# puzzlepaint/camera_calibration

Hardware: NVIDIA H100
Metric: LM iterations/sec (higher is better)
Workload: dtype f64

## Files before the change

### camera_calibration_b200/cabi.py

```python
from __future__ import annotations

import ctypes as C
import os
from dataclasses import dataclass, field
from typing import List, Optional, Sequence

import numpy as np

MODEL_CENTRAL_GENERIC = 0
MODEL_NONCENTRAL_GENERIC = 1
MODEL_CENTRAL_THIN_PRISM_FISHEYE = 2
MODEL_CENTRAL_OPENCV = 3
MODEL_CENTRAL_RADIAL = 4

SCHUR_DENSE = 0
SCHUR_DENSE_CUDA = 1
SCHUR_DENSE_ONTHEFLY = 2
SCHUR_SPARSE = 3
SCHUR_SPARSE_ONTHEFLY = 4

JACOBIAN_NUMERIC = 0
JACOBIAN_ANALYTIC = 1

MAX_TRACE = 128
# ... 347 lines not shown
            p = Problem()
            p.n_cameras = len(self.cameras)
            p.cameras = C.cast(self._cam_array, C.POINTER(Camera))
            p.n_imagesets = self.n_imagesets
            p.n_points = self.n_points
            p.n_obs = self.n_obs
            p.obs_imageset = _ptr(self.obs_imageset, C.c_uint32)
            p.obs_camera = _ptr(self.obs_camera, C.c_uint32)
            p.obs_point = _ptr(self.obs_point, C.c_uint32)
            p.obs_xy = _ptr(self.obs_xy, C.c_float)
            self._c = p
        return self._c

    def shard(self, rank: int, world: int) -> "FlatProblem":
        keep = (self.obs_imageset % np.uint32(world)) == np.uint32(rank)
        return FlatProblem(self.cameras, self.n_imagesets, self.n_points, self.obs_imageset[keep],
                           self.obs_camera[keep], self.obs_point[keep], self.obs_xy[keep])

    def shard_indices(self, rank: int, world: int) -> np.ndarray:
        return np.nonzero((self.obs_imageset % np.uint32(world)) == np.uint32(rank))[0]


@dataclass
class FlatState:

    points: np.ndarray
    rig_tr_global: np.ndarray
    camera_tr_rig: np.ndarray
    intrinsics: List[np.ndarray]
    last_projection: Optional[np.ndarray] = None
    _iptr: object = field(default=None, repr=False)

    def __post_init__(self):
        self.points = np.ascontiguousarray(self.points, dtype=np.float64).reshape(-1, 3)
        self.rig_tr_global = np.ascontiguousarray(self.rig_tr_global, dtype=np.float64).reshape(-1, 7)
        self.camera_tr_rig = np.ascontiguousarray(self.camera_tr_rig, dtype=np.float64).reshape(-1, 7)
        self.intrinsics = [np.ascontiguousarray(a, dtype=np.float64).reshape(-1) for a in self.intrinsics]
        if self.last_projection is not None:
            self.last_projection = np.ascontiguousarray(self.last_projection, dtype=np.float64).reshape(-1, 2)

    def copy(self) -> "FlatState":
        return FlatState(self.points.copy(), self.rig_tr_global.copy(), self.camera_tr_rig.copy(),
                         [a.copy() for a in self.intrinsics],
                         None if self.last_projection is None else self.last_projection.copy())

    def c_struct(self) -> State:
        s = State()
        s.points = _ptr(self.points, C.c_double)
        s.rig_tr_global = _ptr(self.rig_tr_global, C.c_double)
        s.camera_tr_rig = _ptr(self.camera_tr_rig, C.c_double)
        arr = (C.POINTER(C.c_double) * len(self.intrinsics))(*[_ptr(a, C.c_double) for a in self.intrinsics])
        self._iptr = arr
        s.intrinsics = C.cast(arr, C.POINTER(C.POINTER(C.c_double)))
        if self.last_projection is not None:
            s.last_projection = _ptr(self.last_projection, C.c_double)
        else:
            s.last_projection = None
        return s

    def check(self, problem: FlatProblem):
        if self.points.shape != (problem.n_points, 3):
            raise ValueError("points shape")
        if self.rig_tr_global.shape != (problem.n_imagesets, 7):
            raise ValueError("rig_tr_global shape")
        if self.camera_tr_rig.shape != (problem.n_cameras, 7):
            raise ValueError("camera_tr_rig shape")
        for cam, a in zip(problem.cameras, self.intrinsics):
            if a.size != cam.intrinsics_size():
                raise ValueError("intrinsics size")
        if self.last_projection is not None and self.last_projection.shape != (problem.n_obs, 2):
            raise ValueError("last_projection shape")


_LIB = None
LIB_PATH = os.path.join(os.path.dirname(os.path.abspath(__file__)), "csrc", "libb200ba.so")

_D = C.POINTER(C.c_double)
_I32 = C.POINTER(C.c_int32)

SYMBOLS = {
    "b200ba_intrinsics_size": (C.c_int64, [C.POINTER(Camera)]),
    "b200ba_update_parameter_count": (C.c_int32, [C.POINTER(Camera)]),
    "b200ba_default_options": (None, [C.POINTER(Options)]),
    "b200ba_create": (C.c_int, [C.POINTER(Problem), C.c_int, C.POINTER(C.c_void_p)]),
    "b200ba_destroy": (None, [C.c_void_p]),
    "b200ba_last_error": (C.c_char_p, [C.c_void_p]),
    "b200ba_set_state": (C.c_int, [C.c_void_p, C.POINTER(State)]),
    "b200ba_get_state": (C.c_int, [C.c_void_p, C.POINTER(State)]),
    "b200ba_optimize": (C.c_int, [C.c_void_p, C.POINTER(Options), C.POINTER(Report)]),
    "b200ba_optimize_host": (C.c_int, [C.c_void_p, C.POINTER(State), C.POINTER(Options), C.POINTER(Report)]),
    "b200ba_evaluate": (C.c_int, [C.c_void_p, C.POINTER(Options), C.c_int, _D, _D, _D]),
    "b200ba_get_jacobians": (C.c_int, [C.c_void_p, _D, _D, _D, _D, _I32, C.c_int32]),
    "b200ba_build_system": (C.c_int, [C.c_void_p, C.POINTER(Options), C.c_int32, _D, _D, _D]),
    "b200ba_degrees_of_freedom": (C.c_int32, [C.c_void_p, C.POINTER(Options)]),
    "b200ba_schur_solve": (C.c_int, [C.c_int, C.c_int32, C.c_int32, C.c_int32, _D, _D, _D, _D, _D, _D]),
    "b200ba_project": (C.c_int, [C.c_int, C.POINTER(Camera), _D, C.c_int64, _D, _D, _I32]),
    "b200ba_unproject": (C.c_int, [C.c_int, C.POINTER(Camera), _D, C.c_int64, _D, _D, _D, _I32]),
    "b200ba_fit_directions": (C.c_int, [C.c_int, C.c_int32, C.c_int32, _D, C.c_int64, _D, _D, C.c_int32,
                                        C.POINTER(FitReport)]),
    "b200ba_compare_models": (C.c_int, [C.c_int, C.POINTER(Camera), _D, C.POINTER(Camera), _D, C.POINTER(FittingReport),
                                        _D, _D, _D]),
    "b200ba_fitting_images": (C.c_int, [C.c_int, C.POINTER(Camera), _D, C.POINTER(Camera), _D, C.POINTER(FittingReport),
                                        C.POINTER(C.c_uint8), C.POINTER(C.c_uint8), C.POINTER(C.c_uint8),
                                        C.POINTER(C.c_uint8), C.POINTER(C.c_uint8), _D]),
    "b200ba_line_offsets": (C.c_int, [C.c_int, C.POINTER(Camera), _D, C.POINTER(LineOffsetsReport), C.POINTER(C.c_uint8),
                                      _D, C.c_int32, _D, C.POINTER(C.c_int64), _D]),
    "b200ba_localization_accuracy": (C.c_int, [C.c_int, C.POINTER(Camera), _D, C.POINTER(Camera), _D, C.c_int64,
                                               C.c_uint64, C.POINTER(LocalizationReport), C.POINTER(C.c_float), _D,
                                               C.POINTER(C.c_float), _D]),
    "b200ba_compare_reconstructions": (C.c_int, [C.c_int, C.POINTER(Camera), _D, C.POINTER(Camera), _D, C.c_int32, _D,
                                                 _D, _D, _D, C.c_int32, C.POINTER(ReconstructionComparison), _D]),
    "b200ba_reconstruction_directions": (C.c_int, [C.c_int, C.POINTER(Camera), _D, C.POINTER(Camera), _D, C.c_int32,
                                                   C.POINTER(C.c_int32), _D]),
    "b200ba_reconstruction_alignment": (C.c_int, [C.c_int64, _D, C.c_int32, _D, _D, _D, _D,
                                                  C.POINTER(ReconstructionComparison)]),
    "b200ba_nccl_unique_id": (C.c_int, [C.POINTER(C.c_uint8)]),
    "b200ba_comm_init": (C.c_int, [C.c_void_p, C.POINTER(C.c_uint8), C.c_int, C.c_int]),
    "b200ba_get_timings": (C.c_int, [C.c_void_p, C.POINTER(Timings)]),
    "b200ba_dense_cholesky_solve": (C.c_int, [C.c_int, C.c_int32, C.c_int32, C.POINTER(C.c_double), C.POINTER(C.c_double),
                                             C.POINTER(C.c_double), C.POINTER(C.c_double), C.POINTER(C.c_double)]),
    "b200ba_run_bundle_adjustment": (C.c_int, [C.c_void_p, C.POINTER(Options), C.c_int32, C.c_double, C.POINTER(BAReport),
                                              ON_ITERATION, C.c_void_p]),
    "b200ba_calibration_report": (C.c_int, [C.c_void_p, C.POINTER(CameraReport), _D, _D]),
    "b200ba_report_images": (C.c_int, [C.c_void_p, C.c_int32, C.POINTER(C.c_uint8), C.POINTER(C.c_uint8),
                                       C.POINTER(C.c_uint8), C.POINTER(C.c_int64), _D]),
    "b200ba_delete_outliers": (C.c_int, [C.c_void_p, C.c_int32, C.c_float, C.POINTER(C.c_uint8), C.POINTER(C.c_uint8),
                                         C.POINTER(C.c_uint8), C.POINTER(OutlierReport), _D]),
    "b200ba_render_voronoi": (C.c_int, [C.c_int, C.c_int32, C.c_int32, C.c_int64, _I32, C.POINTER(C.c_float),
                                        C.POINTER(C.c_uint8), _D]),
    "b200ba_visualize_camera": (C.c_int, [C.c_int, C.c_int32, C.c_int32, _D, C.POINTER(C.c_uint8), _D, _D, _D]),
    "b200ba_intersect_features": (C.c_int, [C.c_int, C.c_int32, C.c_int64, C.POINTER(C.c_int64), C.POINTER(C.c_float),
                                            C.c_double, C.POINTER(C.c_uint8), C.POINTER(IntersectionReport), _D]),
    "b200ba_synthetic_poses": (C.c_int, [C.POINTER(Pattern), C.c_int32, C.c_int32, C.c_int32, C.c_int32,
                                         C.POINTER(C.c_float), C.c_int64, C.c_uint64, _D, C.POINTER(C.c_int64)]),
    "b200ba_render_pattern_images": (C.c_int, [C.c_int, C.POINTER(Pattern), C.POINTER(C.c_uint8), C.c_int32,
                                               C.c_int32, C.c_int32, C.c_int32, C.POINTER(C.c_float), C.c_int64, _D,
                                               C.POINTER(C.c_uint8), _D]),
    "b200ba_feature_samples": (C.c_int, [C.c_int32, C.c_int32, C.POINTER(C.c_float)]),
    "b200ba_refine_features": (C.c_int, [C.c_int, C.POINTER(Pattern), C.POINTER(C.c_uint8), C.c_int32, C.c_int32,
                                         C.c_int64, C.POINTER(C.c_float), C.c_int32, C.c_int32, C.c_int32, C.c_int64,
                                         C.POINTER(FeaturePrediction), C.POINTER(C.c_float), C.POINTER(C.c_float),
                                         C.POINTER(C.c_int32), _D]),
    "b200ba_snapshot_state": (C.c_int, [C.c_void_p]),
    "b200ba_restore_state": (C.c_int, [C.c_void_p]),
    "b200ba_version": (C.c_char_p, []),
    "b200ba_debug_set_eval_budget": (None, [C.c_int]),
    "b200ba_debug_eval_counts": (C.c_int, [C.c_void_p, C.POINTER(C.c_uint16)]),
    "b200ba_debug_solve_step": (C.c_int, [C.c_void_p, C.POINTER(Options), C.c_double, C.c_int32, _D, _D, _D, _D, _D, _D,
                                          _I32]),
    "b200ba_debug_apply_update": (C.c_int, [C.c_void_p, C.POINTER(Options), _D, C.c_int32, C.POINTER(State)]),
    "b200ba_debug_cost_compare": (C.c_int, [C.c_int, C.c_int64, _D, _D, _D, _D]),
    "b200ba_debug_nice_orientation": (C.c_int, [C.c_void_p, _D]),
    "b200ba_debug_lm_events": (C.c_int32, [C.c_void_p, _I32, C.c_int32]),
}

LM_ACCEPTED, LM_REJECTED_COST, LM_REFUSED_PIVOT = 1, 2, 3


class LibraryMissing(RuntimeError):
    pass


def load_library(path: Optional[str] = None):
    global _LIB
    if _LIB is not None and path is None:
        return _LIB
    p = path or LIB_PATH
    if not os.path.exists(p):
        raise LibraryMissing(
            f"{p} not found: build the CUDA extension first (python -c 'import __graft_entry__ as g; g.build()'). "
            "There is no CPU fallback for this path.")
    lib = C.CDLL(p, mode=C.RTLD_GLOBAL)
    for name, (res, args) in SYMBOLS.items():
        fn = getattr(lib, name)
        fn.restype = res
        fn.argtypes = args
    if path is None:
        _LIB = lib
    return lib
```

### camera_calibration_b200/csrc/ba_common.h

```cpp
#pragma once

#include <cuda_runtime.h>
#include <stdint.h>
#include <string.h>

#include "../../include/b200ba.h"

namespace b200ba {

constexpr int kMaxCameras = 8;
constexpr int kMaxK = 80;

struct CamDev {
  int model_type;
  int width, height;
  int min_x, min_y, max_x, max_y;
  int gw, gh;
  double gmul_x, gmul_y;
  double sx, sy;
  double center_x, center_y;
  int K;
  int dof_per_point;
  int64_t intr_off;
  int64_t tan_off;
  int upd_off;
  int upd_count;
};

struct Layout {
  int n_points, n_imagesets, n_cameras;
  int rig_in_state;
  int localize_only;
  int eliminate_points;
  int dof;
  int bs;
  int nblocks;
  int dsz;
  int nbd;
  int nd;
  int g_point, g_pose, g_rig, g_intr;
  int n_jcols;
  int Kmax;
  int jc_point, jc_pose, jc_rig, jc_intr;
};

struct ProblemDev {
  int64_t n_obs;
  const uint32_t* obs_imageset;
  const uint32_t* obs_camera;
  const uint32_t* obs_point;
  const float2* obs_xy;
  CamDev cams[kMaxCameras];
};

struct StateDev {
  double* points;
  double* rig_tr_global;
  double* camera_tr_rig;
  double* intrinsics;
  double* image_tr_global;
  double* tangents;
};

struct ObsOut {
  double* residual;
  double* cost;
  double* jac;
  double* cjac;
  int compact;
  int32_t* cell;
  uint8_t* has_jac;
  uint16_t* evals;
};

struct SystemDev {
  double* base;
  int64_t total;
  double* Dblk;
  double* bp;
  double* B;
  double* C;
  double* bd;
  double* scalars;
};

constexpr int kReportBiasCells = 50;
struct ReportCam {
  long long count;
  double sum, max, median;
  double biasedness;
  int biasedness_cells;
  double hfov, vfov;
  unsigned long long select_prefix;
  long long select_rank;
};
struct ReportDev {
  double2* err;
  double* mag;
  int64_t* cam_off;
  int* cell_off;
  uint32_t* cell_order;
  double* Q;
  double* partial;
  unsigned int* select_hist;
  int* hist;
  double* kl;
  ReportCam* cams;
};

struct OutlierDev {
  int64_t* range;
  double* mag;
  double* partial;
  unsigned int* select_hist;
  ReportCam* stats;
  uint8_t* used;
  int* kept;
  unsigned long long* counts;
  uint8_t* remove;
  uint32_t* owner;
  uint8_t* image;
};

struct CompareDev {
  double* mag;
  double* dir_err;
  double* rep_err;
  unsigned long long* dir_max;
  int64_t* range;
  double* partial;
  unsigned int* select_hist;
  ReportCam* stats;
  uint8_t* angles;
  uint8_t* magnitudes;
  uint8_t* directions;
  uint8_t* rep_magnitudes;
  uint8_t* reprojections;
};

constexpr int kLocPoints = 15;
constexpr int kLocMaxDraws = 4096;
struct LocalizationDev {
  double* p;
  double* f;
  float* samples;
  double* poses;
  double* mag;
  unsigned long long* counts;
  int* capped;
  int64_t* range;
  double* partial;
  unsigned int* select_hist;
  ReportCam* stats;
};

constexpr int kSweepSums = 10;

constexpr int kLineSums = 10;
struct LineOffsetsDev {
  double* lines;
  double* partial;
  double* sums;
  double* mag;
  unsigned long long* extent;
  int64_t* range;
  double* stat_partial;
  unsigned int* select_hist;
  ReportCam* stats;
  double* offsets;
  uint8_t* image;
  double* obj;
};

constexpr int kVoronoiNoSite = INT32_MIN;
struct VoronoiGrid {
  int x0, y0;
  int bs;
  int nx, ny;
  int* off;
  int* count;
  int* idx;
  int* scan_sums;
};
constexpr int kVoronoiScanChunk = 4096;
constexpr int kVoronoiScanMax = 4096;
constexpr int64_t kVoronoiMaxBuckets = int64_t(kVoronoiScanChunk) * kVoronoiScanMax - 1;

struct FixedRanges {
  int n;
  int lo[4], hi[4];
  __host__ __device__ bool has(int g) const {
    for (int i = 0; i < n; ++i)
      if (g >= lo[i] && g < hi[i]) return true;
    return false;
  }
};

__host__ __device__ __forceinline__ uint64_t loc_splitmix64(uint64_t z) {
  z += 0x9E3779B97F4A7C15ull;
  z = (z ^ (z >> 30)) * 0xBF58476D1CE4E5B9ull;
  z = (z ^ (z >> 27)) * 0x94D049BB133111EBull;
  return z ^ (z >> 31);
}

__host__ __device__ __forceinline__ float rf_add(float a, float b) {
#ifdef __CUDA_ARCH__
  return __fadd_rn(a, b);
#else
  return a + b;
#endif
}
__host__ __device__ __forceinline__ float rf_sub(float a, float b) {
#ifdef __CUDA_ARCH__
  return __fsub_rn(a, b);
#else
  return a - b;
#endif
}
__host__ __device__ __forceinline__ float rf_mul(float a, float b) {
#ifdef __CUDA_ARCH__
  return __fmul_rn(a, b);
#else
  return a * b;
#endif
}
// ... 141 lines not shown
```

### camera_calibration_b200/csrc/ba_host.cu

```cuda

#include <cublas_v2.h>
#include <cusolverDn.h>
#include <dlfcn.h>

#include <algorithm>
#include <cmath>
#include <cstdarg>
#include <cstdio>
#include <cstring>
#include <limits>
#include <string>
#include <vector>

#include "ba_kernels.h"

using namespace b200ba;

namespace {

std::string g_create_error;

struct NcclUniqueId {
  char internal[128];
};
struct NcclApi {
  void* lib = nullptr;
  int (*GetUniqueId)(void*) = nullptr;
  int (*CommInitRank)(void**, int, NcclUniqueId, int) = nullptr;
  int (*AllReduce)(const void*, void*, size_t, int, int, void*, cudaStream_t) = nullptr;
  int (*Broadcast)(const void*, void*, size_t, int, int, void*, cudaStream_t) = nullptr;
  int (*ReduceScatter)(const void*, void*, size_t, int, int, void*, cudaStream_t) = nullptr;
  int (*CommDestroy)(void*) = nullptr;
  const char* (*GetErrorString)(int) = nullptr;
};
constexpr int kNcclDouble = 8;
constexpr int kNcclInt32 = 2;
constexpr int kNcclSum = 0;
constexpr int kNcclMax = 2;

NcclApi g_nccl;
bool load_nccl(std::string* err) {
  if (g_nccl.lib) return true;
  const char* names[] = {"libnccl.so.2", "libnccl.so"};
  void* lib = nullptr;
  for (const char* n : names) {
    lib = dlopen(n, RTLD_NOW | RTLD_GLOBAL);
    if (lib) break;
  }
  if (!lib) {
    *err = std::string("cannot load libnccl: ") + dlerror();
    return false;
  }
  g_nccl.lib = lib;
  *reinterpret_cast<void**>(&g_nccl.GetUniqueId) = dlsym(lib, "ncclGetUniqueId");
  *reinterpret_cast<void**>(&g_nccl.CommInitRank) = dlsym(lib, "ncclCommInitRank");
  *reinterpret_cast<void**>(&g_nccl.AllReduce) = dlsym(lib, "ncclAllReduce");
  *reinterpret_cast<void**>(&g_nccl.Broadcast) = dlsym(lib, "ncclBroadcast");
  *reinterpret_cast<void**>(&g_nccl.ReduceScatter) = dlsym(lib, "ncclReduceScatter");
  *reinterpret_cast<void**>(&g_nccl.CommDestroy) = dlsym(lib, "ncclCommDestroy");
  *reinterpret_cast<void**>(&g_nccl.GetErrorString) = dlsym(lib, "ncclGetErrorString");
  if (!g_nccl.GetUniqueId || !g_nccl.CommInitRank || !g_nccl.AllReduce || !g_nccl.Broadcast || !g_nccl.ReduceScatter ||
      !g_nccl.CommDestroy) {
    *err = "libnccl lacks a required symbol";
    g_nccl.lib = nullptr;
    return false;
  }
  return true;
}

enum Phase { PH_JAC = 0, PH_ACC, PH_SCHUR, PH_FACTOR, PH_TRIAL, PH_UPDATE, PH_ALLREDUCE, PH_STRAGGLER, PH_SOLVE, PH_COUNT };

}

struct b200ba_handle {
  int device = 0;
  cudaStream_t stream = nullptr;
  cudaStream_t side_stream = nullptr;
  cudaEvent_t straggler_done = nullptr;
  cublasHandle_t cublas = nullptr;
  cusolverDnHandle_t cusolver = nullptr;
  std::string error;

  std::vector<b200ba_camera> cams_host;
  ProblemDev pb{};
  int n_cameras = 0, n_imagesets = 0, n_points = 0;
  int64_t n_obs = 0;
  int uniform_model = -1;
  int64_t n_control_total = 0, n_param_total = 0, intr_total = 0, tan_total = 0;
  uint32_t *d_obs_imageset = nullptr, *d_obs_camera = nullptr, *d_obs_point = nullptr;
  float2* d_obs_xy = nullptr;

  StateDev st[2]{};
  int cur = 0;
  double2* d_last_projection = nullptr;
  bool have_state = false;
  StateDev snap{};
  double2* d_snap_lp = nullptr;
  bool have_snapshot = false;

  Layout L{};
  bool have_layout = false;
  ObsOut out{};
  ObsOut out_trial{};
  SystemDev sys{};
  double *d_W = nullptr, *d_S = nullptr, *d_Linv = nullptr, *d_v = nullptr, *d_y = nullptr, *d_x = nullptr;
  double trace_H = 0;
  int64_t reduce_count = 0;
  double* d_potrf_work = nullptr;
  int potrf_lwork = 0;
  int *d_info = nullptr, *d_fail = nullptr;
  std::vector<uint32_t> perm;
  uint32_t* d_perm = nullptr;
  double2* d_lp_stage = nullptr;
  uint32_t* d_straggler_list = nullptr;
  int* d_straggler_count = nullptr;
  double *d_partial = nullptr, *d_scal = nullptr;
  double* d_rot = nullptr;
  double* h_scal = nullptr;
  int* h_flags = nullptr;

  std::vector<uint32_t> h_obs_imageset, h_obs_camera, h_obs_point;
  std::vector<float> h_obs_xy;
  int group_blocks_n = 0;
  int n_groups = 0;
  std::vector<int> group_start;
  std::vector<int> group_count;
  int* d_group_of_block = nullptr;
  int* d_group_blocks = nullptr;
  uint8_t* d_flags = nullptr;
  int* d_cols = nullptr;
  int* d_count = nullptr;
  int* h_count = nullptr;
  double* d_Wc = nullptr;
  double* d_P = nullptr;
  size_t wc_stride = 0, p_stride = 0;
  cudaEvent_t ev_syrk[2] = {nullptr, nullptr}, ev_scatter[2] = {nullptr, nullptr}, ev_s_ready = nullptr;
  double* d_u = nullptr;
  bool use_grouped = false;
  double* capture_S = nullptr;
  double* capture_rhs = nullptr;
  std::vector<int32_t> lm_events;
  std::vector<double> grp_sums;
  int force_grouped = -1;

  ReportDev rep{};
  double2* d_rep_stage = nullptr;
  bool have_report = false;
  std::vector<int64_t> img_cam_groups;
  int* d_img_group_off = nullptr;
  uint32_t* d_img_group_obs = nullptr;
  bool have_images = false;

  void* comm = nullptr;
  int rank = 0, n_ranks = 1;

  bool own_dense = true;
  DenseCtx dn;
  int dense_planned_ranks = 0, dense_planned_n = -1;
  int dense_nb = 0;
  cudaStream_t panel_stream = nullptr;
  cudaStream_t aux_stream = nullptr;
  int* d_ident_cols = nullptr;
  double* d_gemv_partial = nullptr;

  b200ba_timings timings{};
  struct Pending {
    int phase;
    cudaEvent_t a, b;
    bool own_a = true;
  };
  std::vector<Pending> pending;
  std::vector<cudaEvent_t> event_pool;
};

namespace {

#define CUDA_TRY(h, expr)                                                                      \
  do {                                                                                         \
    cudaError_t _e = (expr);                                                                   \
    if (_e != cudaSuccess) {                                                                   \
      (h)->error = std::string(#expr) + ": " + cudaGetErrorString(_e);                         \
      return 1;                                                                                \
    }                                                                                          \
  } while (0)
#define CUBLAS_TRY(h, expr)                                                                    \
  do {                                                                                         \
    cublasStatus_t _s = (expr);                                                                \
    if (_s != CUBLAS_STATUS_SUCCESS) {                                                         \
      (h)->error = std::string(#expr) + ": cuBLAS status " + std::to_string(static_cast<int>(_s)); \
      return 1;                                                                                \
    }                                                                                          \
  } while (0)
#define CUSOLVER_TRY(h, expr)                                                                  \
  do {                                                                                         \
    cusolverStatus_t _s = (expr);                                                              \
    if (_s != CUSOLVER_STATUS_SUCCESS) {                                                       \
      (h)->error = std::string(#expr) + ": cuSOLVER status " + std::to_string(static_cast<int>(_s)); \
      return 1;                                                                                \
    }                                                                                          \
  } while (0)

template <class T>
int dev_alloc(b200ba_handle* h, T** p, size_t count) {
  if (*p) {
    cudaFree(*p);
    *p = nullptr;
  }
  if (count == 0) count = 1;
  CUDA_TRY(h, cudaMalloc(reinterpret_cast<void**>(p), count * sizeof(T)));
  return 0;
}

int64_t intrinsics_size(const b200ba_camera& c) {
  const int64_t G = static_cast<int64_t>(c.grid_width) * c.grid_height;
  switch (c.model_type) {
    case B200BA_MODEL_CENTRAL_GENERIC: return 3 * G;
    case B200BA_MODEL_NONCENTRAL_GENERIC: return 6 * G;
    default: return 12;
  }
}
int update_parameter_count(const b200ba_camera& c) {
  const int G = c.grid_width * c.grid_height;
  switch (c.model_type) {
    case B200BA_MODEL_CENTRAL_GENERIC: return 2 * G;
    case B200BA_MODEL_NONCENTRAL_GENERIC: return 5 * G;
    default: return 12;
  }
}
int jacobian_size(const b200ba_camera& c) {
  switch (c.model_type) {
    case B200BA_MODEL_CENTRAL_GENERIC: return 32;
    case B200BA_MODEL_NONCENTRAL_GENERIC: return 80;
    default: return 12;
  }
}

void fill_camdev(const b200ba_camera& c, CamDev* d) {
  d->model_type = c.model_type;
  d->width = c.width;
  d->height = c.height;
  d->min_x = c.calibration_min_x;
  d->min_y = c.calibration_min_y;
  d->max_x = c.calibration_max_x;
  d->max_y = c.calibration_max_y;
  d->gw = c.grid_width;
  d->gh = c.grid_height;
  const int aw = c.calibration_max_x + 1 - c.calibration_min_x;
  const int ah = c.calibration_max_y + 1 - c.calibration_min_y;
  d->gmul_x = (c.grid_width > 0) ? static_cast<double>(c.grid_width - 3) / aw : 0.0;
  d->gmul_y = (c.grid_height > 0) ? static_cast<double>(c.grid_height - 3) / ah : 0.0;
  d->sx = (c.grid_width > 0) ? static_cast<double>((c.grid_width - 3.f) / aw) : 0.0;
  d->sy = (c.grid_height > 0) ? static_cast<double>((c.grid_height - 3.f) / ah) : 0.0;
  d->center_x = 0.5f * static_cast<float>(c.calibration_min_x + c.calibration_max_x + 1);
  d->center_y = 0.5f * static_cast<float>(c.calibration_min_y + c.calibration_max_y + 1);
  d->K = jacobian_size(c);
  d->dof_per_point = c.model_type == B200BA_MODEL_CENTRAL_GENERIC ? 2 : (c.model_type == B200BA_MODEL_NONCENTRAL_GENERIC ? 5 : 0);
  d->upd_count = update_parameter_count(c);
}

int64_t align32(int64_t n) { return (n + 31) / 32 * 32; }

cudaEvent_t get_event(b200ba_handle* h) {
  if (!h->event_pool.empty()) {
    cudaEvent_t e = h->event_pool.back();
    h->event_pool.pop_back();
    return e;
  }
  cudaEvent_t e;
  cudaEventCreate(&e);
  return e;
}
struct ScopedPhase {
  b200ba_handle* h;
  int phase;
  cudaEvent_t a;
  ScopedPhase(b200ba_handle* h_, int p) : h(h_), phase(p) {
    a = get_event(h);
    cudaEventRecord(a, h->stream);
  }
  ~ScopedPhase() {
    cudaEvent_t b = get_event(h);
    cudaEventRecord(b, h->stream);
    h->pending.push_back({phase, a, b, true});
  }
};
void resolve_timings(b200ba_handle* h) {
  for (auto& p : h->pending) {
    float ms = 0;
    if (cudaEventElapsedTime(&ms, p.a, p.b) == cudaSuccess) {
      switch (p.phase) {
        case PH_JAC: h->timings.jacobian_kernel_ms += ms; h->timings.jacobian_kernel_launches++; break;
        case PH_ACC: h->timings.accumulate_ms += ms; break;
        case PH_SCHUR: h->timings.schur_ms += ms; break;
        case PH_FACTOR: h->timings.factor_ms += ms; break;
        case PH_TRIAL: h->timings.trial_cost_ms += ms; break;
        case PH_UPDATE: h->timings.update_ms += ms; break;
        case PH_ALLREDUCE: h->timings.allreduce_ms += ms; break;
        case PH_STRAGGLER: h->timings.straggler_ms += ms; break;
        case PH_SOLVE: h->timings.solve_ms += ms; h->timings.factor_ms += ms; break;
      }
    }
    if (p.own_a) h->event_pool.push_back(p.a);
    h->event_pool.push_back(p.b);
  }
  h->pending.clear();
}
int reduce_group_sums(b200ba_handle* h) {
  if (h->n_ranks <= 1 || !h->comm || h->grp_sums.empty()) return 0;
  const size_t n = h->grp_sums.size();
  double* d = nullptr;
  CUDA_TRY(h, cudaMalloc(reinterpret_cast<void**>(&d), n * sizeof(double)));
  cudaMemcpy(d, h->grp_sums.data(), n * sizeof(double), cudaMemcpyHostToDevice);
  const int rc = g_nccl.AllReduce(d, d, n, kNcclDouble, kNcclSum, h->comm, h->stream);
  const cudaError_t ce = cudaStreamSynchronize(h->stream);
  if (rc == 0 && ce == cudaSuccess) cudaMemcpy(h->grp_sums.data(), d, n * sizeof(double), cudaMemcpyDeviceToHost);
  cudaFree(d);
  if (rc != 0 || ce != cudaSuccess) {
    h->error = "all-reduce of the group centroids failed";
    return 1;
  }
  return 0;
}

int build_groups(b200ba_handle* h, bool allocate) {
  const Layout& L = h->L;
  const int nb = L.nblocks;
  int gb = (L.bs == 3) ? 96 : 48;
  if (const char* e = getenv("B200BA_GROUP_BLOCKS")) gb = std::max(1, atoi(e));
  h->group_blocks_n = gb;
  std::vector<int> order(nb);
  for (int i = 0; i < nb; ++i) order[i] = i;
  if (L.eliminate_points && nb > 0) {
    const double* sx = h->grp_sums.data();
    const double* sy = sx + nb;
    const double* cnt = sy + nb;
    const double qx = std::max(1.0, h->cams_host[0].width / 64.0), qy = std::max(1.0, h->cams_host[0].height / 64.0);
    std::vector<uint32_t> zkey(nb, 0);
    for (int p = 0; p < nb; ++p) {
      if (cnt[p] <= 0) continue;
      uint32_t ux = static_cast<uint32_t>(std::min(1023.0, std::max(0.0, sx[p] / cnt[p] / qx)));
      uint32_t uy = static_cast<uint32_t>(std::min(1023.0, std::max(0.0, sy[p] / cnt[p] / qy)));
      uint32_t z = 0;
      for (int b = 0; b < 10; ++b) z |= ((ux >> b) & 1u) << (2 * b) | ((uy >> b) & 1u) << (2 * b + 1);
      zkey[p] = z;
    }
    std::stable_sort(order.begin(), order.end(), [&](int a, int b) { return zkey[a] < zkey[b]; });
  }
  h->n_groups = (nb + gb - 1) / gb;
  h->group_start.assign(h->n_groups + 1, 0);
  std::vector<int> gob(std::max(1, nb), 0);
  for (int g = 0; g < h->n_groups; ++g) {
    h->group_start[g] = g * gb;
    for (int i = g * gb; i < std::min(nb, (g + 1) * gb); ++i) gob[order[i]] = g;
  }
  h->group_start[h->n_groups] = nb;
  h->group_count.assign(std::max(1, h->n_groups), 0);
  if (allocate) {
    if (dev_alloc(h, &h->d_group_of_block, std::max(1, nb))) return 1;
    if (dev_alloc(h, &h->d_group_blocks, std::max(1, nb))) return 1;
    if (dev_alloc(h, &h->d_flags, static_cast<size_t>(std::max(1, h->n_groups)) * std::max(1, L.nd))) return 1;
    if (dev_alloc(h, &h->d_cols, static_cast<size_t>(std::max(1, h->n_groups)) * std::max(1, L.nd))) return 1;
    if (dev_alloc(h, &h->d_count, std::max(1, h->n_groups))) return 1;
    if (h->h_count) cudaFreeHost(h->h_count);
    CUDA_TRY(h, cudaMallocHost(reinterpret_cast<void**>(&h->h_count), std::max(1, h->n_groups) * sizeof(int)));
    h->wc_stride = static_cast<size_t>(gb) * L.bs * (std::max(1, L.nd) + 1);
    h->p_stride = static_cast<size_t>(std::max(1, L.nd)) * std::max(1, L.nd);
    if (dev_alloc(h, &h->d_Wc, 2 * h->wc_stride)) return 1;
    if (!h->own_dense && dev_alloc(h, &h->d_P, 2 * h->p_stride)) return 1;
    for (int i = 0; i < 2; ++i) {
      if (!h->ev_syrk[i]) CUDA_TRY(h, cudaEventCreateWithFlags(&h->ev_syrk[i], cudaEventDisableTiming));
      if (!h->ev_scatter[i]) CUDA_TRY(h, cudaEventCreateWithFlags(&h->ev_scatter[i], cudaEventDisableTiming));
    }
    if (!h->ev_s_ready) CUDA_TRY(h, cudaEventCreateWithFlags(&h->ev_s_ready, cudaEventDisableTiming));
    if (dev_alloc(h, &h->d_u, std::max(1, L.nbd))) return 1;
  }
  CUDA_TRY(h, cudaMemcpy(h->d_group_of_block, gob.data(), std::max(1, nb) * sizeof(int), cudaMemcpyHostToDevice));
  if (nb > 0) CUDA_TRY(h, cudaMemcpy(h->d_group_blocks, order.data(), nb * sizeof(int), cudaMemcpyHostToDevice));
  return 0;
}

int nccl_bcast_cb(double* buf, size_t count, int root, cudaStream_t s, void* user) {
  b200ba_handle* h = static_cast<b200ba_handle*>(user);
  const int rc = g_nccl.Broadcast(buf, buf, count, kNcclDouble, root, h->comm, s);
  if (rc != 0) {
    h->error = std::string("ncclBroadcast: ") + (g_nccl.GetErrorString ? g_nccl.GetErrorString(rc) : "error");
    return 1;
  }
  return 0;
}

cudaError_t dense_create(DenseCtx* d, bool own_streams) {
  cudaError_t e = cudaSuccess;
  if (own_streams) {
    int lo = 0, hi = 0;
    cudaDeviceGetStreamPriorityRange(&lo, &hi);
    e = cudaStreamCreateWithFlags(&d->s_main, cudaStreamNonBlocking);
    if (e == cudaSuccess) e = cudaStreamCreateWithPriority(&d->s_panel, cudaStreamNonBlocking, hi);
    if (e == cudaSuccess) e = cudaStreamCreateWithPriority(&d->s_aux, cudaStreamNonBlocking, hi);
  }
  for (cudaEvent_t* ev : {&d->ev_ready[0], &d->ev_ready[1], &d->ev_main[0], &d->ev_main[1], &d->ev_half2[0],
                          &d->ev_half2[1], &d->ev_misc})
    if (e == cudaSuccess && !*ev) e = cudaEventCreateWithFlags(ev, cudaEventDisableTiming);
  return e;
}
void dense_release(DenseCtx* d, bool own_streams) {
  for (cudaEvent_t ev : {d->ev_ready[0], d->ev_ready[1], d->ev_main[0], d->ev_main[1], d->ev_half2[0], d->ev_half2[1],
                         d->ev_misc})
    if (ev) cudaEventDestroy(ev);
  if (own_streams)
    for (cudaStream_t s : {d->s_main, d->s_panel, d->s_aux})
      if (s) cudaStreamDestroy(s);
}

int plan_dense(b200ba_handle* h) {
// ... 56 lines not shown
  }
  const int rig_dof = L.rig_in_state ? 6 * h->n_cameras : 0;
  if (L.eliminate_points) {
    L.bs = 3;
    L.nblocks = h->n_points;
    L.g_point = 0;
    L.g_pose = 3 * h->n_points;
    L.g_rig = L.g_pose + 6 * h->n_imagesets;
    L.g_intr = L.g_rig + rig_dof;
  } else {
    L.bs = 6;
    L.nblocks = h->n_imagesets;
    L.g_pose = 0;
    L.g_rig = 6 * h->n_imagesets;
    L.g_point = L.g_rig + rig_dof;
    L.g_intr = L.g_point + 3 * h->n_points;
  }
  L.dsz = L.bs * (L.bs + 1) / 2;
  L.nbd = L.bs * L.nblocks;
  L.dof = 3 * h->n_points + 6 * h->n_imagesets + rig_dof + n_intr;
  L.nd = L.dof - L.nbd;
  L.Kmax = kmax;
  L.jc_point = 0;
  L.jc_pose = 3;
  L.jc_rig = 9;
  L.jc_intr = 9 + (L.rig_in_state ? 6 : 0);
  L.n_jcols = L.jc_intr + kmax;
  const bool same = h->have_layout && memcmp(&L, &h->L, sizeof(Layout)) == 0;
  if (same) return plan_dense(h);
  h->L = L;
  h->have_layout = true;
  h->dense_planned_n = -1;

  const int64_t n = h->n_obs;
  if (dev_alloc(h, &h->out.residual, 2 * n)) return 1;
  if (dev_alloc(h, &h->out.cost, n)) return 1;
  h->out.compact = (h->uniform_model == B200BA_MODEL_CENTRAL_GENERIC) ? 1 : 0;
  if (h->out.compact) {
    if (h->out.jac) cudaFree(h->out.jac);
    h->out.jac = nullptr;
    if (dev_alloc(h, &h->out.cjac, 14 * static_cast<size_t>(n))) return 1;
  } else {
    if (dev_alloc(h, &h->out.jac, 2 * static_cast<size_t>(L.n_jcols) * n)) return 1;
  }
  if (dev_alloc(h, &h->out.cell, n)) return 1;
  if (dev_alloc(h, &h->out.has_jac, n)) return 1;
  if (dev_alloc(h, &h->out.evals, n)) return 1;
  h->out_trial.evals = nullptr;
  if (dev_alloc(h, &h->out_trial.residual, 2 * n)) return 1;
  if (dev_alloc(h, &h->out_trial.cost, n)) return 1;
  h->out_trial.jac = nullptr;
  h->out_trial.cjac = nullptr;
  h->out_trial.compact = 0;
  h->out_trial.cell = nullptr;
  h->out_trial.has_jac = nullptr;

  SystemDev& s = h->sys;
  const int64_t oD = 0;
  const int64_t obp = oD + align32(static_cast<int64_t>(L.dsz) * L.nblocks);
  const int64_t oB = obp + align32(L.nbd);
  const int64_t obd = oB + align32(static_cast<int64_t>(L.nbd) * L.nd);
  const int64_t osc = obd + align32(L.nd);
  const int64_t oC = osc + 32;
  s.total = oC + align32(static_cast<int64_t>(L.nd) * L.nd);
  h->reduce_count = oC;
  if (dev_alloc(h, &s.base, s.total)) return 1;
  s.Dblk = s.base + oD;
  s.bp = s.base + obp;
  s.B = s.base + oB;
  s.C = s.base + oC;
  s.bd = s.base + obd;
  s.scalars = s.base + osc;
  if (dev_alloc(h, &h->d_W, static_cast<size_t>(L.nbd) * L.nd)) return 1;
  if (!h->own_dense) {
    if (dev_alloc(h, &h->d_S, static_cast<size_t>(L.nd) * L.nd + L.nd)) return 1;
  } else if (plan_dense(h)) {
    return 1;
  }
  if (dev_alloc(h, &h->d_Linv, static_cast<size_t>(L.dsz) * L.nblocks)) return 1;
  if (dev_alloc(h, &h->d_v, L.nbd)) return 1;
  if (dev_alloc(h, &h->d_y, L.nbd)) return 1;
  if (dev_alloc(h, &h->d_x, L.dof)) return 1;
  int lwork = 0;
  CUSOLVER_TRY(h, cusolverDnDpotrf_bufferSize(h->cusolver, CUBLAS_FILL_MODE_LOWER, L.nd, h->d_S, std::max(1, L.nd), &lwork));
  h->potrf_lwork = lwork;
  if (dev_alloc(h, &h->d_potrf_work, std::max(1, lwork))) return 1;

  {
    const int nb = L.nblocks;
    h->grp_sums.assign(3 * static_cast<size_t>(std::max(1, nb)), 0.0);
    if (L.eliminate_points) {
      for (int64_t o = 0; o < h->n_obs; ++o) {
        const int p = static_cast<int>(h->h_obs_point[o]);
        h->grp_sums[p] += h->h_obs_xy[2 * o];
        h->grp_sums[nb + p] += h->h_obs_xy[2 * o + 1];
        h->grp_sums[2 * nb + p] += 1.0;
      }
    }
    if (reduce_group_sums(h)) return 1;
    if (build_groups(h, true)) return 1;
  }
  return 0;
}

int sync_stream(b200ba_handle* h) {
  CUDA_TRY(h, cudaStreamSynchronize(h->stream));
  resolve_timings(h);
  return 0;
}

int all_reduce(b200ba_handle* h, double* buf, size_t count) {
  if (h->n_ranks <= 1 || !h->comm) return 0;
  ScopedPhase ph(h, PH_ALLREDUCE);
  int rc = g_nccl.AllReduce(buf, buf, count, kNcclDouble, kNcclSum, h->comm, h->stream);
  if (rc != 0) {
    h->error = std::string("ncclAllReduce: ") + (g_nccl.GetErrorString ? g_nccl.GetErrorString(rc) : "error");
    return 1;
  }
  return 0;
}

int evaluate_state(b200ba_handle* h, int which, bool jac, const ObsOut& out, double huber, int phase,
                   bool overlap_stragglers = false) {
  launch_prepare_state(h->pb, h->L, h->st[which], h->n_control_total, h->stream);
  h->timings.kernel_launches += 1;
  {
    cudaEvent_t a = get_event(h), mid = get_event(h);
    cudaEventRecord(a, h->stream);
    launch_residual_jacobian(h->uniform_model, jac, h->pb, h->L, h->st[which], h->d_last_projection, out, huber,
                             h->d_straggler_list, h->d_straggler_count, h->stream, mid);
    if (h->n_obs == 0) cudaEventRecord(mid, h->stream);
    h->pending.push_back({phase, a, mid, true});
    cudaStream_t ss = overlap_stragglers ? h->side_stream : h->stream;
    if (overlap_stragglers) CUDA_TRY(h, cudaStreamWaitEvent(h->side_stream, mid, 0));
    cudaEvent_t s0 = get_event(h), s1 = get_event(h);
    cudaEventRecord(s0, ss);
    launch_straggler_pass(h->uniform_model, jac, h->pb, h->L, h->st[which], h->d_last_projection, out, huber,
                          h->d_straggler_list, h->d_straggler_count, ss);
    cudaEventRecord(s1, ss);
    h->pending.push_back({PH_STRAGGLER, s0, s1, true});
    h->straggler_done = s1;
    h->timings.kernel_launches += 2 * (h->n_obs > 0);
  }
  CUDA_TRY(h, cudaGetLastError());
  return 0;
}

int build_system(b200ba_handle* h, double huber, double* cost, double* n_valid, const b200ba_options* fix = nullptr) {
  if (evaluate_state(h, h->cur, true, h->out, huber, PH_JAC, true)) return 1;
  {
    ScopedPhase ph(h, PH_ACC);
    CUDA_TRY(h, cudaMemsetAsync(h->sys.base, 0, h->sys.total * sizeof(double), h->stream));
    launch_accumulate_scatter(h->pb, h->L, h->st[h->cur], h->out, h->sys, huber, h->stream);
    if (!h->L.localize_only || h->L.rig_in_state) {
      launch_accumulate_cells(h->pb, h->L, h->st[h->cur], h->out, h->sys, huber, h->stream);
      h->timings.kernel_launches += 1;
    }
    CUDA_TRY(h, cudaStreamWaitEvent(h->stream, h->straggler_done, 0));
    launch_accumulate_list(h->pb, h->L, h->st[h->cur], h->out, h->sys, huber, h->d_straggler_list, h->d_straggler_count, h->stream);
    h->timings.kernel_launches += 2;
    launch_cost_reduce(h->n_obs, h->out.cost, nullptr, h->out.residual, h->d_partial, h->sys.scalars, h->stream);
    launch_trace(h->L.nblocks, h->L.bs, h->sys.Dblk, h->L.nd, h->sys.C, h->sys.scalars + 8, h->stream);
    h->timings.kernel_launches += 3;
  }
  CUDA_TRY(h, cudaGetLastError());
  if (all_reduce(h, h->sys.base, static_cast<size_t>(h->reduce_count))) return 1;
  if (fix) {
    const Layout& L = h->L;
    FixedRanges fr{};
    auto add = [&](int g0, int count) {
      if (count > 0 && fr.n < 4) {
        fr.lo[fr.n] = g0;
        fr.hi[fr.n] = g0 + count;
        fr.n++;
      }
    };
    int n_intr = 0;
    for (int c = 0; c < h->n_cameras; ++c) n_intr += update_parameter_count(h->cams_host[c]);
    if (fix->debug_fix_points) add(L.g_point, 3 * L.n_points);
    if (fix->debug_fix_poses) add(L.g_pose, 6 * L.n_imagesets);
    if (fix->debug_fix_rig_poses && L.rig_in_state) add(L.g_rig, 6 * L.n_cameras);
    if (fix->debug_fix_intrinsics && !L.localize_only) add(L.g_intr, n_intr);
    launch_mask_fixed(L, h->sys, fr, h->rank == 0 ? 1.0 : 0.0, h->stream);
    h->timings.kernel_launches += 3;
  }
  CUDA_TRY(h, cudaMemcpyAsync(h->h_scal, h->sys.scalars, 9 * sizeof(double), cudaMemcpyDeviceToHost, h->stream));
  if (h->n_groups > 0 && h->L.nd > 0 && h->force_grouped != 0) {
    ScopedPhase ph(h, PH_SCHUR);
    CUDA_TRY(h, cudaMemsetAsync(h->d_flags, 0, static_cast<size_t>(h->n_groups) * h->L.nd, h->stream));
    launch_group_support(h->L.bs, h->L.nblocks, h->L.nd, h->sys.B, h->d_group_of_block, h->d_flags, h->stream);
    launch_compact_columns(h->n_groups, h->L.nd, h->d_flags, h->d_cols, h->d_count, h->stream);
    CUDA_TRY(h, cudaMemcpyAsync(h->h_count, h->d_count, h->n_groups * sizeof(int), cudaMemcpyDeviceToHost, h->stream));
    h->timings.kernel_launches += 2;
  }
  if (sync_stream(h)) return 1;
  *cost = h->h_scal[3];
  *n_valid = h->h_scal[4];
  h->trace_H = h->h_scal[8];
  h->use_grouped = false;
  if (h->n_groups > 0 && h->L.nd > 0 && h->force_grouped != 0) {
    double grouped = 0;
    for (int g = 0; g < h->n_groups; ++g) {
      const double kg = static_cast<double>(h->group_start[g + 1] - h->group_start[g]) * h->L.bs;
      const double mg = h->h_count[g];
      h->group_count[g] = h->h_count[g];
      grouped += mg * mg * (kg + 24.0);
    }
    const double dense = static_cast<double>(h->L.nd) * h->L.nd * h->L.nbd;
    h->use_grouped = (h->force_grouped == 1) || grouped < 0.6 * dense;
  }
  return 0;
}

int factor_dense(b200ba_handle* h) {
  const int nd = h->L.nd;
  CUSOLVER_TRY(h, cusolverDnDpotrf(h->cusolver, CUBLAS_FILL_MODE_LOWER, nd, h->d_S, nd, h->d_potrf_work, h->potrf_lwork,
                                   h->d_info));
  return 0;
}

int capture_reduced_system(b200ba_handle* h) {
  const Layout& L = h->L;
  const int nd = L.nd;
  if (nd > 0) {
    if (h->own_dense) {
      const DenseCtx& d = h->dn;
      for (int j = 0; j < d.nblk; ++j) {
        const int c0 = j * d.NB, w = std::min(d.NB, nd - c0);
        CUDA_TRY(h, cudaMemcpy2DAsync(h->capture_S + static_cast<size_t>(c0) * nd, static_cast<size_t>(nd) * sizeof(double),
                                      h->d_S + d.map.col_offset(c0), d.map.ld * sizeof(double),
                                      static_cast<size_t>(nd) * sizeof(double), w, cudaMemcpyDeviceToHost, h->stream));
      }
    } else {
      CUDA_TRY(h, cudaMemcpyAsync(h->capture_S, h->d_S, static_cast<size_t>(nd) * nd * sizeof(double), cudaMemcpyDeviceToHost,
                                  h->stream));
    }
    CUDA_TRY(h, cudaMemcpyAsync(h->capture_rhs, h->d_x + L.nbd, static_cast<size_t>(nd) * sizeof(double),
                                cudaMemcpyDeviceToHost, h->stream));
  }
  return sync_stream(h);
}

int solve_system_own(b200ba_handle* h, double lambda, int* spd);

int solve_system(b200ba_handle* h, double lambda, int* spd) {
  if (h->own_dense) return solve_system_own(h, lambda, spd);
  const Layout& L = h->L;
  const double one = 1.0, minus_one = -1.0;
  bool grouped_done = false;
  if (h->use_grouped) {
    ScopedPhase ph(h, PH_SCHUR);
    const double zero = 0.0;
    CUDA_TRY(h, cudaMemsetAsync(h->d_fail, 0, sizeof(int), h->stream));
    launch_schur_blocks(L.bs, L.nblocks, h->sys.Dblk, h->sys.bp, lambda, h->d_Linv, h->d_v, h->d_fail, h->stream);
    CUDA_TRY(h, cudaEventRecord(h->ev_s_ready, h->stream));
    CUDA_TRY(h, cudaStreamWaitEvent(h->side_stream, h->ev_s_ready, 0));
    CUDA_TRY(h, cudaMemcpyAsync(h->d_S, h->sys.C, static_cast<size_t>(L.nd) * L.nd * sizeof(double),
                                cudaMemcpyDeviceToDevice, h->side_stream));
    CUDA_TRY(h, cudaEventRecord(h->ev_s_ready, h->side_stream));
    launch_block_solve_t(L.bs, L.nblocks, h->d_Linv, h->d_v, h->d_u, h->stream);
    h->timings.kernel_launches += 2;
    int it = 0;
    for (int g = h->rank; g < h->n_groups; g += h->n_ranks) {
      const int nblk = h->group_start[g + 1] - h->group_start[g];
      const int kg = nblk * L.bs, mg = h->group_count[g];
      if (mg == 0 || kg == 0) continue;
      h->timings.contraction_flops += static_cast<double>(mg) * mg * kg;
      const int b = it & 1;
      double* Wc = h->d_Wc + b * h->wc_stride;
      double* P = h->d_P + b * h->p_stride;
      const int* cols = h->d_cols + static_cast<size_t>(g) * L.nd;
      if (it >= 2) CUDA_TRY(h, cudaStreamWaitEvent(h->stream, h->ev_scatter[b], 0));
      launch_gather_scale(L.bs, nblk, L.nd, mg, mg, h->sys.B, h->d_Linv, h->d_group_blocks + h->group_start[g], cols, Wc,
                          h->stream);
      CUBLAS_TRY(h, cublasDsyrk(h->cublas, CUBLAS_FILL_MODE_LOWER, CUBLAS_OP_N, mg, kg, &one, Wc, mg, &zero, P, mg));
      CUDA_TRY(h, cudaEventRecord(h->ev_syrk[b], h->stream));
      CUDA_TRY(h, cudaStreamWaitEvent(h->side_stream, h->ev_syrk[b], 0));
      launch_scatter_sub(L.nd, mg, cols, P, h->d_S, h->side_stream);
      CUDA_TRY(h, cudaEventRecord(h->ev_scatter[b], h->side_stream));
      h->timings.kernel_launches += 2;
      ++it;
    }
    CUDA_TRY(h, cudaStreamWaitEvent(h->stream, h->ev_s_ready, 0));
    for (int b = 0; b < 2 && b < it; ++b) CUDA_TRY(h, cudaStreamWaitEvent(h->stream, h->ev_scatter[b], 0));
    grouped_done = true;
  }
  if (grouped_done) {
    if (h->n_ranks > 1) {
      if (all_reduce(h, h->d_S, static_cast<size_t>(L.nd) * L.nd)) return 1;
    }
    ScopedPhase ph(h, PH_SCHUR);
    launch_add_diagonal(L.nd, h->d_S, L.nd, lambda, h->stream);
    CUDA_TRY(h, cudaMemcpyAsync(h->d_x + L.nbd, h->sys.bd, L.nd * sizeof(double), cudaMemcpyDeviceToDevice, h->stream));
    if (L.nbd > 0 && L.nd > 0)
      CUBLAS_TRY(h, cublasDgemv(h->cublas, CUBLAS_OP_N, L.nd, L.nbd, &minus_one, h->sys.B, L.nd, h->d_u, 1, &one,
                                h->d_x + L.nbd, 1));
    h->timings.kernel_launches += 1;
  } else {
    const int p0 = static_cast<int>(static_cast<int64_t>(L.nblocks) * h->rank / h->n_ranks);
    const int p1 = static_cast<int>(static_cast<int64_t>(L.nblocks) * (h->rank + 1) / h->n_ranks);
    const int k_rows = L.bs * (p1 - p0);
    double* rhs_tail = h->d_S + static_cast<size_t>(L.nd) * L.nd;
    {
      ScopedPhase ph(h, PH_SCHUR);
      CUDA_TRY(h, cudaMemsetAsync(h->d_fail, 0, sizeof(int), h->stream));
      launch_schur_blocks(L.bs, L.nblocks, h->sys.Dblk, h->sys.bp, lambda, h->d_Linv, h->d_v, h->d_fail, h->stream);
// ... 86 lines not shown
    launch_block_solve_t(L.bs, L.nblocks, h->d_Linv, h->d_v, h->d_u, h->stream);
    h->timings.kernel_launches += 2;
    bool joined = false;
    auto join_copy = [&]() {
      if (!joined) cudaStreamWaitEvent(h->stream, h->ev_s_ready, 0);
      joined = true;
    };
    if (h->use_grouped) {
      int it = 0;
      for (int g = h->rank; g < h->n_groups; g += R) {
        const int nblk = h->group_start[g + 1] - h->group_start[g];
        const int kg = nblk * L.bs, mg = h->group_count[g];
        if (mg == 0 || kg == 0) continue;
        const int ldw = (mg + 1) / 2 * 2;
        double* Wc = h->d_Wc + (it & 1) * h->wc_stride;
        const int* cols = h->d_cols + static_cast<size_t>(g) * nd;
        launch_gather_scale(L.bs, nblk, nd, mg, ldw, h->sys.B, h->d_Linv, h->d_group_blocks + h->group_start[g], cols, Wc,
                            h->stream);
        join_copy();
        GemmArgs ga{};
        ga.M = ga.N = mg;
        ga.K = kg;
        ga.A = ga.B = Wc;
        ga.lda = ga.ldb = ldw;
        ga.C = h->d_S;
        ga.alpha = -1.0;
        ga.beta = 1.0;
        ga.a_aligned = ga.b_aligned = gemm_operand_aligned(Wc, ldw);
        ga.cols = cols;
        ga.map = d.map;
        if (launch_dgemm_nt(ga, true, true, h->stream)) {
          h->error = "dgemm_nt (contraction) launch failed";
          return 1;
        }
        h->timings.contraction_flops += static_cast<double>(mg) * mg * kg;
        h->timings.kernel_launches += 2;
        ++it;
      }
    } else if (L.nbd > 0 && nd > 0) {
      const int p0 = static_cast<int>(static_cast<int64_t>(L.nblocks) * h->rank / R);
      const int p1 = static_cast<int>(static_cast<int64_t>(L.nblocks) * (h->rank + 1) / R);
      const int k_rows = L.bs * (p1 - p0);
      launch_schur_scale_rows(L.bs, L.nblocks, nd, h->sys.B, h->d_Linv, h->d_W, h->stream);
      h->timings.kernel_launches += 1;
      if (k_rows > 0) {
        const double* Wr = h->d_W + static_cast<size_t>(L.bs) * p0 * nd;
        join_copy();
        GemmArgs ga{};
        ga.M = ga.N = nd;
        ga.K = k_rows;
        ga.A = ga.B = Wr;
        ga.lda = ga.ldb = nd;
        ga.C = h->d_S;
        ga.ldc = d.map.ld;
        ga.alpha = -1.0;
        ga.beta = 1.0;
        ga.a_aligned = ga.b_aligned = gemm_operand_aligned(Wr, nd);
        ga.cols = h->d_ident_cols;
        ga.map = d.map;
        if (launch_dgemm_nt(ga, true, R > 1, h->stream)) {
          h->error = "dgemm_nt (contraction) launch failed";
          return 1;
        }
        h->timings.contraction_flops += static_cast<double>(nd) * nd * k_rows;
        h->timings.kernel_launches += 1;
      }
    }
    join_copy();
    if (h->rank == 0) launch_add_diagonal_map(nd, h->d_S, d.map, lambda, h->stream);
    CUDA_TRY(h, cudaMemcpyAsync(h->d_x + L.nbd, h->sys.bd, nd * sizeof(double), cudaMemcpyDeviceToDevice, h->stream));
    if (L.nbd > 0 && nd > 0) launch_gemv_t(L.nbd, nd, nd, h->sys.B, h->d_u, -1.0, h->d_x + L.nbd, h->d_gemv_partial, h->stream);
    h->timings.kernel_launches += 4;
  }
  if (h->capture_S && capture_reduced_system(h)) return 1;
  if (R > 1 && nd > 0) {
    ScopedPhase ph(h, PH_ALLREDUCE);
    const int rc = g_nccl.ReduceScatter(h->d_S, h->d_S + static_cast<size_t>(h->rank) * d.chunk, static_cast<size_t>(d.chunk),
                                        kNcclDouble, kNcclSum, h->comm, h->stream);
    if (rc != 0) {
      h->error = std::string("ncclReduceScatter: ") + (g_nccl.GetErrorString ? g_nccl.GetErrorString(rc) : "error");
      return 1;
    }
  }
  {
    ScopedPhase ph(h, PH_FACTOR);
    if (dense_factor(&d)) {
      if (h->error.empty()) h->error = "dense_factor: launch failed";
      return 1;
    }
    h->timings.factor_flops += static_cast<double>(nd) * nd * nd / 3.0;
    if (R > 1) {
      const int rc = g_nccl.AllReduce(h->d_info, h->d_info, 1, kNcclInt32, kNcclMax, h->comm, h->stream);
      if (rc != 0) {
        h->error = "ncclAllReduce (factorisation status) failed";
        return 1;
      }
    }
  }
  {
    ScopedPhase ph(h, PH_SOLVE);
    if (dense_solve(&d, h->d_x + L.nbd)) {
      h->error = "dense_solve: launch failed";
      return 1;
    }
    h->timings.kernel_launches += 4 * d.ntiles;
  }
  {
    ScopedPhase ph(h, PH_SCHUR);
    if (L.nbd > 0 && nd > 0)
      launch_gemv_n(L.nbd, nd, nd, h->sys.B, h->d_x + L.nbd, h->d_y, h->stream);
    else if (L.nbd > 0)
      CUDA_TRY(h, cudaMemsetAsync(h->d_y, 0, L.nbd * sizeof(double), h->stream));
    launch_block_backsub2(L.bs, L.nblocks, h->d_Linv, h->d_u, h->d_y, h->d_x, h->stream);
    h->timings.kernel_launches += 1;
  }
  CUDA_TRY(h, cudaMemcpyAsync(h->h_flags, h->d_info, sizeof(int), cudaMemcpyDeviceToHost, h->stream));
  CUDA_TRY(h, cudaMemcpyAsync(h->h_flags + 1, h->d_fail, sizeof(int), cudaMemcpyDeviceToHost, h->stream));
  if (sync_stream(h)) return 1;
  *spd = (h->h_flags[0] == 0 && h->h_flags[1] == 0) ? 1 : 0;
  return 0;
}

int check_ready(b200ba_handle* h, const b200ba_options* opt) {
  if (!h) return 1;
  if (!opt) {
    h->error = "options are NULL";
    return 2;
  }
  if (!h->have_state) {
    h->error = "no state: call b200ba_set_state first";
    return 2;
  }
  CUDA_TRY(h, cudaSetDevice(h->device));
  return make_layout(h, opt);
}

void free_handle_buffers(b200ba_handle* h) {
  auto F = [](auto*& p) {
    if (p) cudaFree(p);
    p = nullptr;
  };
  F(h->d_obs_imageset); F(h->d_obs_camera); F(h->d_obs_point); F(h->d_obs_xy);
  for (int i = 0; i < 2; ++i) {
    F(h->st[i].points); F(h->st[i].rig_tr_global); F(h->st[i].camera_tr_rig); F(h->st[i].intrinsics);
    F(h->st[i].image_tr_global); F(h->st[i].tangents);
  }
  F(h->d_last_projection);
  F(h->snap.points); F(h->snap.rig_tr_global); F(h->snap.camera_tr_rig); F(h->snap.intrinsics); F(h->d_snap_lp);
  h->have_snapshot = false;
  F(h->out.residual); F(h->out.cost); F(h->out.jac); F(h->out.cjac); F(h->out.cell); F(h->out.has_jac); F(h->out.evals);
  F(h->out_trial.residual); F(h->out_trial.cost);
  F(h->sys.base); F(h->d_W); F(h->d_S); F(h->d_Linv); F(h->d_v); F(h->d_y); F(h->d_x); F(h->d_potrf_work);
  F(h->d_info); F(h->d_fail); F(h->d_straggler_list); F(h->d_straggler_count); F(h->d_perm); F(h->d_lp_stage);
  F(h->d_group_of_block); F(h->d_group_blocks); F(h->d_flags); F(h->d_cols); F(h->d_count); F(h->d_Wc); F(h->d_P); F(h->d_u);
  if (h->h_count) cudaFreeHost(h->h_count);
  h->h_count = nullptr;
  F(h->d_partial); F(h->d_scal); F(h->d_rot);
  F(h->rep.err); F(h->rep.mag); F(h->rep.cam_off); F(h->rep.cell_off); F(h->rep.cell_order); F(h->rep.Q);
  F(h->rep.partial); F(h->rep.select_hist); F(h->rep.hist); F(h->rep.kl); F(h->rep.cams); F(h->d_rep_stage);
  h->have_report = false;
  F(h->d_img_group_off); F(h->d_img_group_obs);
  h->have_images = false;
  F(h->dn.Lpack); F(h->dn.tmp); F(h->dn.d_panel_off); F(h->dn.d_panel_h); F(h->d_ident_cols); F(h->d_gemv_partial);
  h->dn.S = nullptr;
  h->dense_planned_n = -1;
  if (h->h_scal) cudaFreeHost(h->h_scal);
  if (h->h_flags) cudaFreeHost(h->h_flags);
  h->h_scal = nullptr;
  h->h_flags = nullptr;
}

int setup_report(b200ba_handle* h) {
  if (h->have_report) return 0;
  const int64_t n = h->n_obs;
  const int nc = h->n_cameras;
  constexpr int kCells = kReportBiasCells * kReportBiasCells;
  std::vector<int64_t> cam_off(nc + 1, 0);
  for (int64_t o = 0; o < n; ++o) ++cam_off[h->h_obs_camera[o] + 1];
  for (int c = 0; c < nc; ++c) cam_off[c + 1] += cam_off[c];
  std::vector<uint32_t> key(n);
  std::vector<int> cell_off(static_cast<size_t>(nc) * kCells + 1, 0);
  for (int64_t o = 0; o < n; ++o) {
    const uint32_t cam = h->h_obs_camera[o];
    const b200ba_camera& c = h->cams_host[cam];
    const double step_u = static_cast<double>(c.calibration_max_x - c.calibration_min_x) / kReportBiasCells + 1e-7;
    const double step_v = static_cast<double>(c.calibration_max_y - c.calibration_min_y) / kReportBiasCells + 1e-7;
    const float dx = h->h_obs_xy[2 * o] - static_cast<float>(c.calibration_min_x);
    const float dy = h->h_obs_xy[2 * o + 1] - static_cast<float>(c.calibration_min_y);
    const int cx = std::min(kReportBiasCells - 1, std::max(0, static_cast<int>(dx / step_u)));
    const int cy = std::min(kReportBiasCells - 1, std::max(0, static_cast<int>(dy / step_v)));
    key[o] = cam * kCells + cy * kReportBiasCells + cx;
    ++cell_off[key[o] + 1];
  }
  for (size_t k = 0; k + 1 < cell_off.size(); ++k) cell_off[k + 1] += cell_off[k];
  std::vector<uint32_t> pos(n), order(n);
  for (int64_t i = 0; i < n; ++i) pos[h->perm[i]] = static_cast<uint32_t>(i);
  {
    std::vector<int> fill(cell_off.begin(), cell_off.end() - 1);
    for (int64_t o = 0; o < n; ++o) order[fill[key[o]]++] = pos[o];
  }
  double Q[64], q_sum = 0;
  for (int y = 0; y < 8; ++y)
    for (int x = 0; x < 8; ++x) {
      const double dx = (2.5 / (0.5 * 8)) * (0.5 * 8 - (x + 0.5));
      const double dy = (2.5 / (0.5 * 8)) * (0.5 * 8 - (y + 0.5));
      const double p = std::exp(-0.5 * (dx * dx + dy * dy));
      Q[y * 8 + x] = p;
      q_sum += p;
    }
  for (double& q : Q) q /= q_sum;
  ReportDev& r = h->rep;
  if (dev_alloc(h, &r.err, n) || dev_alloc(h, &r.mag, n) || dev_alloc(h, &r.cam_off, nc + 1) ||
      dev_alloc(h, &r.cell_off, cell_off.size()) || dev_alloc(h, &r.cell_order, n) || dev_alloc(h, &r.Q, 64) ||
      dev_alloc(h, &r.partial, report_partial_size(nc)) || dev_alloc(h, &r.select_hist, 256 * nc) ||
      dev_alloc(h, &r.hist, static_cast<size_t>(nc) * B200BA_REPORT_HIST * B200BA_REPORT_HIST) ||
      dev_alloc(h, &r.kl, static_cast<size_t>(nc) * kCells) || dev_alloc(h, &r.cams, nc) || dev_alloc(h, &h->d_rep_stage, n))
    return 1;
  CUDA_TRY(h, cudaMemcpy(r.cam_off, cam_off.data(), cam_off.size() * sizeof(int64_t), cudaMemcpyHostToDevice));
  CUDA_TRY(h, cudaMemcpy(r.cell_off, cell_off.data(), cell_off.size() * sizeof(int), cudaMemcpyHostToDevice));
  if (n > 0) CUDA_TRY(h, cudaMemcpy(r.cell_order, order.data(), n * sizeof(uint32_t), cudaMemcpyHostToDevice));
  CUDA_TRY(h, cudaMemcpy(r.Q, Q, sizeof(Q), cudaMemcpyHostToDevice));
  h->have_report = true;
  return 0;
}

int setup_images(b200ba_handle* h) {
  if (h->have_images) return 0;
  const int64_t n = h->n_obs;
  const int nc = h->n_cameras;
  std::vector<uint32_t> pos(n);
  for (int64_t i = 0; i < n; ++i) pos[h->perm[i]] = static_cast<uint32_t>(i);
  std::vector<std::pair<int64_t, uint32_t>> keyed;
  keyed.reserve(n);
  for (int64_t o = 0; o < n; ++o) {
    const b200ba_camera& c = h->cams_host[h->h_obs_camera[o]];
    const float x = h->h_obs_xy[2 * o], y = h->h_obs_xy[2 * o + 1];
    if (!(x > -1.f && y > -1.f && x < 4.f * c.width && y < 4.f * c.height)) continue;
    const int64_t ix = static_cast<int>(x), iy = static_cast<int>(y);
    if (ix >= 4 * static_cast<int64_t>(c.width) || iy >= 4 * static_cast<int64_t>(c.height)) continue;
    const int64_t key = (static_cast<int64_t>(h->h_obs_camera[o]) << 40) | (iy * 4 * c.width + ix);
    keyed.emplace_back(key, static_cast<uint32_t>(o));
  }
  std::stable_sort(keyed.begin(), keyed.end(),
                   [](const std::pair<int64_t, uint32_t>& a, const std::pair<int64_t, uint32_t>& b) { return a.first < b.first; });
  std::vector<int> group_off;
  std::vector<uint32_t> group_obs(keyed.size());
  h->img_cam_groups.assign(nc + 1, 0);
  for (size_t k = 0; k < keyed.size(); ++k) {
    if (k == 0 || keyed[k].first != keyed[k - 1].first) {
      group_off.push_back(static_cast<int>(k));
      ++h->img_cam_groups[(keyed[k].first >> 40) + 1];
    }
    group_obs[k] = pos[keyed[k].second];
  }
  group_off.push_back(static_cast<int>(keyed.size()));
  for (int c = 0; c < nc; ++c) h->img_cam_groups[c + 1] += h->img_cam_groups[c];
  if (dev_alloc(h, &h->d_img_group_off, group_off.size()) || dev_alloc(h, &h->d_img_group_obs, group_obs.size())) return 1;
  CUDA_TRY(h, cudaMemcpy(h->d_img_group_off, group_off.data(), group_off.size() * sizeof(int), cudaMemcpyHostToDevice));
  if (!group_obs.empty())
    CUDA_TRY(h, cudaMemcpy(h->d_img_group_obs, group_obs.data(), group_obs.size() * sizeof(uint32_t), cudaMemcpyHostToDevice));
  h->have_images = true;
  return 0;
}

struct CallScope {
  std::string* error;
  int rc = 0;
  std::vector<void*> buffers;
  cudaEvent_t events[3] = {};
  cublasHandle_t cublas = nullptr;
  cusolverDnHandle_t cusolver = nullptr;

  explicit CallScope(std::string* error_sink) : error(error_sink) {}
  CallScope(const CallScope&) = delete;
  CallScope& operator=(const CallScope&) = delete;
  ~CallScope() {
    for (void* p : buffers) cudaFree(p);
    for (cudaEvent_t e : events)
      if (e) cudaEventDestroy(e);
    if (cublas) cublasDestroy(cublas);
    if (cusolver) cusolverDnDestroy(cusolver);
  }
  int use_device(int device) {
    int ndev = 0;
    if (cudaGetDeviceCount(&ndev) != cudaSuccess || ndev == 0) {
      g_create_error = "no CUDA device available (this library has no CPU fallback)";
      return 3;
    }
    if (device >= 0) cudaSetDevice(device);
    return 0;
  }
  void fail(const char* message) {
    if (rc == 0) {
      *error = message;
      rc = 1;
    }
  }
  bool ok(cudaError_t e) {
    if (e != cudaSuccess) fail(cudaGetErrorString(e));
    return e == cudaSuccess;
  }
  template <class T>
  void alloc(T** p, size_t count) {
    if (ok(cudaMalloc(p, sizeof(T) * count))) buffers.push_back(*p);
  }
  void record(int k, cudaStream_t s) {
    for (cudaEvent_t& e : events)
      if (!e) ok(cudaEventCreate(&e));
    cudaEventRecord(events[k], s);
  }
  float elapsed_ms(int from, int to) {
    float ms = 0;
    ok(cudaEventElapsedTime(&ms, events[from], events[to]));
    return ms;
  }
  bool create_solvers() {
    if (rc == 0 && (cublasCreate(&cublas) != CUBLAS_STATUS_SUCCESS || cusolverDnCreate(&cusolver) != CUSOLVER_STATUS_SUCCESS))
      fail("cuBLAS / cuSOLVER initialisation failed");
    return rc == 0;
  }
};

struct VoronoiRun {
  VoronoiGrid g{};
  int64_t nb = 0;
  void alloc(CallScope& cs, int64_t n, int64_t lo_x, int64_t lo_y, int64_t hi_x, int64_t hi_y) {
    g = voronoi_grid_geometry(lo_x, lo_y, hi_x, hi_y);
    nb = static_cast<int64_t>(g.nx) * g.ny;
    cs.alloc(&g.off, nb + 1);
    cs.alloc(&g.count, nb);
    cs.alloc(&g.idx, std::max<int64_t>(1, n));
    cs.alloc(&g.scan_sums, kVoronoiScanMax);
  }
  cudaError_t n_valid(int64_t* out) {
    int v = 0;
    const cudaError_t e = cudaMemcpy(&v, g.off + nb, sizeof(int), cudaMemcpyDeviceToHost);
    *out = v;
    return e;
  }
};

void alloc_range_statistics(CallScope& cs, int64_t n, int64_t** range, double** partial, unsigned int** select_hist,
                            ReportCam** stats) {
  cs.alloc(range, 2);
  cs.alloc(partial, report_partial_size(1));
  cs.alloc(select_hist, 256);
  cs.alloc(stats, 1);
  const int64_t r[2] = {0, n};
  if (cs.rc == 0) cs.ok(cudaMemcpy(*range, r, sizeof(r), cudaMemcpyHostToDevice));
}

struct LmResult {
  int iterations = 0, attempts = 0;
  double initial_cost = 0, final_cost = 0, lambda = 0;
};
template <class System, class InitLambda, class Solve, class TrialCost, class Accept>
LmResult small_lm(const int& rc, int max_iterations, System system, InitLambda init_lambda, Solve solve,
                  TrialCost trial_cost, Accept accept) {
  LmResult r;
  for (int iteration = 0; rc == 0 && iteration < max_iterations; ++iteration) {
    r.final_cost = system(iteration);
    if (rc) break;
    if (iteration == 0) r.initial_cost = r.final_cost;
    if (r.final_cost == 0) break;
    if (iteration == 0) {
      r.lambda = init_lambda(static_cast<double>(0.001f));
      if (rc) break;
    }
    bool applied = false;
    for (int attempt = 0; rc == 0 && attempt < 10; ++attempt) {
      r.attempts++;
      const bool solved = solve(r.lambda);
      if (rc) break;
      if (!solved) {
        r.lambda = 2.f * r.lambda;
        continue;
      }
      const double test_cost = trial_cost();
      if (rc) break;
      if (test_cost < r.final_cost) {
        accept();
        r.lambda = 0.5f * r.lambda;
        applied = true;
        r.iterations += 1;
        r.final_cost = test_cost;
        break;
      }
      r.lambda = 2.f * r.lambda;
    }
    if (!applied || r.final_cost == 0) break;
  }
  return r;
}

int download_system(b200ba_handle* h, double* H, double* b) {
  const Layout& L = h->L;
  const int n = L.dof;
  std::vector<double> D(static_cast<size_t>(L.dsz) * L.nblocks), bp(L.nbd), B(static_cast<size_t>(L.nbd) * L.nd),
      C(static_cast<size_t>(L.nd) * L.nd), bd(L.nd);
  CUDA_TRY(h, cudaMemcpy(D.data(), h->sys.Dblk, D.size() * sizeof(double), cudaMemcpyDeviceToHost));
  CUDA_TRY(h, cudaMemcpy(bp.data(), h->sys.bp, bp.size() * sizeof(double), cudaMemcpyDeviceToHost));
  CUDA_TRY(h, cudaMemcpy(B.data(), h->sys.B, B.size() * sizeof(double), cudaMemcpyDeviceToHost));
  CUDA_TRY(h, cudaMemcpy(C.data(), h->sys.C, C.size() * sizeof(double), cudaMemcpyDeviceToHost));
  CUDA_TRY(h, cudaMemcpy(bd.data(), h->sys.bd, bd.size() * sizeof(double), cudaMemcpyDeviceToHost));
  std::fill(H, H + static_cast<size_t>(n) * n, 0.0);
  for (int p = 0; p < L.nblocks; ++p) {
    const double* d = &D[static_cast<size_t>(L.dsz) * p];
    const int o = L.bs * p;
    for (int a2 = 0; a2 < L.bs; ++a2)
      for (int b2 = a2; b2 < L.bs; ++b2)
        H[static_cast<size_t>(o + a2) * n + o + b2] = d[a2 * L.bs - (a2 * (a2 - 1)) / 2 + (b2 - a2)];
  }
  for (int i = 0; i < L.nbd; ++i)
    for (int k = 0; k < L.nd; ++k) H[static_cast<size_t>(i) * n + L.nbd + k] = B[static_cast<size_t>(i) * L.nd + k];
  for (int i = 0; i < L.nd; ++i)
    for (int k = i; k < L.nd; ++k) H[static_cast<size_t>(L.nbd + i) * n + L.nbd + k] = C[static_cast<size_t>(i) * L.nd + k];
  for (int i = 0; i < L.nbd; ++i) b[i] = bp[i];
  for (int i = 0; i < L.nd; ++i) b[L.nbd + i] = bd[i];
  return 0;
}

}

extern "C" {

const char* b200ba_version(void) { return "b200ba 0.1.0 (sm_90a, FP64)"; }

int64_t b200ba_intrinsics_size(const b200ba_camera* cam) { return cam ? intrinsics_size(*cam) : 0; }
int32_t b200ba_update_parameter_count(const b200ba_camera* cam) { return cam ? update_parameter_count(*cam) : 0; }

void b200ba_default_options(b200ba_options* o) {
  if (!o) return;
  o->max_iteration_count = 1;
  o->init_lambda = -1.0;
  o->numerical_diff_delta = 1e-4;
  o->regularization_weight = 0.0;
  o->localize_only = 0;
  o->eliminate_points = 1;
  o->schur_mode = B200BA_SCHUR_DENSE;
  o->max_lm_attempts = 50;
  o->init_lambda_factor = 1e-5;
  o->huber_parameter = 1.0;
  o->jacobian_mode = B200BA_JACOBIAN_ANALYTIC;
  o->print_progress = 0;
  o->debug_verify_cost = 0;
  o->debug_fix_points = o->debug_fix_poses = o->debug_fix_rig_poses = o->debug_fix_intrinsics = 0;
}

const char* b200ba_last_error(const b200ba_handle* h) { return h ? h->error.c_str() : g_create_error.c_str(); }

int b200ba_create(const b200ba_problem* p, int device, b200ba_handle** out) {
  if (!p || !out) {
    g_create_error = "NULL argument";
    return 2;
  }
  *out = nullptr;
  int ndev = 0;
  if (cudaGetDeviceCount(&ndev) != cudaSuccess || ndev == 0) {
    g_create_error = "no CUDA device available (this library has no CPU fallback)";
    return 3;
  }
  if (p->n_cameras < 1 || p->n_cameras > kMaxCameras) {
    g_create_error = "n_cameras out of range (1..8)";
    return 2;
  }
  for (int c = 0; c < p->n_cameras; ++c) {
    const int t = p->cameras[c].model_type;
    if (t != B200BA_MODEL_CENTRAL_GENERIC && t != B200BA_MODEL_NONCENTRAL_GENERIC && t != B200BA_MODEL_CENTRAL_OPENCV) {
      g_create_error = "camera model not on the accelerated path (central-generic, noncentral-generic, central-opencv)";
      return 2;
    }
    if (t != B200BA_MODEL_CENTRAL_OPENCV && (p->cameras[c].grid_width < 4 || p->cameras[c].grid_height < 4)) {
      g_create_error = "generic models need a grid of at least 4x4 control points";
      return 2;
    }
  }
  if (p->n_obs >= (1LL << 31)) {
    g_create_error = "n_obs must be < 2^31";
    return 2;
  }
  for (int64_t o = 0; o < p->n_obs; ++o) {
    if (p->obs_imageset[o] >= static_cast<uint32_t>(p->n_imagesets) || p->obs_point[o] >= static_cast<uint32_t>(p->n_points) ||
        p->obs_camera[o] >= static_cast<uint32_t>(p->n_cameras)) {
      g_create_error = "observation index out of range";
      return 2;
    }
  }
  b200ba_handle* h = new b200ba_handle();
  auto fail = [&](int rc) {
    g_create_error = h->error;
    free_handle_buffers(h);
    if (h->cublas) cublasDestroy(h->cublas);
    if (h->cusolver) cusolverDnDestroy(h->cusolver);
    if (h->stream) cudaStreamDestroy(h->stream);
    if (h->side_stream) cudaStreamDestroy(h->side_stream);
    delete h;
    return rc;
  };
  if (device < 0) {
    if (cudaGetDevice(&device) != cudaSuccess) device = 0;
  }
  h->device = device;
#define TRYC(expr) \
  if ((expr) != 0) return fail(1)
  auto cuda_ok = [&](cudaError_t e, const char* what) {
    if (e != cudaSuccess) {
      h->error = std::string(what) + ": " + cudaGetErrorString(e);
      return 1;
    }
    return 0;
  };
  TRYC(cuda_ok(cudaSetDevice(device), "cudaSetDevice"));
  TRYC(cuda_ok(cudaStreamCreateWithFlags(&h->stream, cudaStreamNonBlocking), "cudaStreamCreate"));
  TRYC(cuda_ok(cudaStreamCreateWithFlags(&h->side_stream, cudaStreamNonBlocking), "cudaStreamCreate"));
  if (cublasCreate(&h->cublas) != CUBLAS_STATUS_SUCCESS) {
    h->error = "cublasCreate failed";
    return fail(1);
  }
  cublasSetStream(h->cublas, h->stream);
  if (cusolverDnCreate(&h->cusolver) != CUSOLVER_STATUS_SUCCESS) {
    h->error = "cusolverDnCreate failed";
    return fail(1);
  }
  cusolverDnSetStream(h->cusolver, h->stream);

  h->n_cameras = p->n_cameras;
  h->n_imagesets = p->n_imagesets;
  h->n_points = p->n_points;
  h->n_obs = p->n_obs;
  h->cams_host.assign(p->cameras, p->cameras + p->n_cameras);
  h->uniform_model = h->cams_host[0].model_type;
  int upd = 0;
  for (int c = 0; c < p->n_cameras; ++c) {
    CamDev& d = h->pb.cams[c];
    fill_camdev(h->cams_host[c], &d);
    d.intr_off = h->intr_total;
    d.tan_off = h->tan_total;
    d.upd_off = upd;
    upd += d.upd_count;
    h->intr_total += intrinsics_size(h->cams_host[c]);
    const int64_t G = static_cast<int64_t>(d.gw) * d.gh;
    h->tan_total += 6 * G;
    h->n_control_total += G;
    if (d.gw == 0) h->n_param_total += 12;
    if (h->cams_host[c].model_type != h->uniform_model) h->uniform_model = -1;
  }
  const int64_t n = p->n_obs;
  TRYC(dev_alloc(h, &h->d_obs_imageset, n));
  TRYC(dev_alloc(h, &h->d_obs_camera, n));
  TRYC(dev_alloc(h, &h->d_obs_point, n));
  TRYC(dev_alloc(h, &h->d_obs_xy, n));
  if (n > 0) {
    std::vector<uint32_t> key(n);
    for (int64_t o = 0; o < n; ++o) {
      const uint32_t cam = p->obs_camera[o];
      const CamDev& cd = h->pb.cams[cam];
      uint32_t cell = 0;
      if (cd.gw > 0) {
        const double gx = 1.0 + cd.gmul_x * (static_cast<double>(p->obs_xy[2 * o]) - cd.min_x);
        const double gy = 1.0 + cd.gmul_y * (static_cast<double>(p->obs_xy[2 * o + 1]) - cd.min_y);
        const int x0 = std::min(std::max(static_cast<int>(std::floor(gx)) - 1, 0), cd.gw - 4);
        const int y0 = std::min(std::max(static_cast<int>(std::floor(gy)) - 1, 0), cd.gh - 4);
        cell = static_cast<uint32_t>(x0 + y0 * cd.gw);
      }
      key[o] = (cam << 24) | cell;
    }
    h->perm.resize(n);
    for (int64_t o = 0; o < n; ++o) h->perm[o] = static_cast<uint32_t>(o);
    std::stable_sort(h->perm.begin(), h->perm.end(), [&](uint32_t a, uint32_t b) { return key[a] < key[b]; });
    std::vector<uint32_t> t32(n);
    std::vector<float> txy(2 * n);
    for (int64_t i = 0; i < n; ++i) t32[i] = p->obs_imageset[h->perm[i]];
    TRYC(cuda_ok(cudaMemcpy(h->d_obs_imageset, t32.data(), n * sizeof(uint32_t), cudaMemcpyHostToDevice), "H2D"));
    for (int64_t i = 0; i < n; ++i) t32[i] = p->obs_camera[h->perm[i]];
    TRYC(cuda_ok(cudaMemcpy(h->d_obs_camera, t32.data(), n * sizeof(uint32_t), cudaMemcpyHostToDevice), "H2D"));
    for (int64_t i = 0; i < n; ++i) t32[i] = p->obs_point[h->perm[i]];
    TRYC(cuda_ok(cudaMemcpy(h->d_obs_point, t32.data(), n * sizeof(uint32_t), cudaMemcpyHostToDevice), "H2D"));
    for (int64_t i = 0; i < n; ++i) {
      txy[2 * i] = p->obs_xy[2 * h->perm[i]];
      txy[2 * i + 1] = p->obs_xy[2 * h->perm[i] + 1];
    }
    TRYC(cuda_ok(cudaMemcpy(h->d_obs_xy, txy.data(), n * sizeof(float2), cudaMemcpyHostToDevice), "H2D"));
    TRYC(dev_alloc(h, &h->d_perm, n));
    TRYC(cuda_ok(cudaMemcpy(h->d_perm, h->perm.data(), n * sizeof(uint32_t), cudaMemcpyHostToDevice), "H2D"));
  }
  TRYC(dev_alloc(h, &h->d_lp_stage, n));
  if (n > 0) {
    h->h_obs_imageset.assign(p->obs_imageset, p->obs_imageset + n);
    h->h_obs_camera.assign(p->obs_camera, p->obs_camera + n);
    h->h_obs_point.assign(p->obs_point, p->obs_point + n);
    h->h_obs_xy.assign(p->obs_xy, p->obs_xy + 2 * n);
  }
  if (const char* e = getenv("B200BA_DENSE")) h->own_dense = !(strcmp(e, "lib") == 0 || strcmp(e, "0") == 0);
  if (const char* e = getenv("B200BA_DENSE_NB")) h->dense_nb = std::max(128, atoi(e) / 128 * 128);
  {
    int lo = 0, hi = 0;
    cudaDeviceGetStreamPriorityRange(&lo, &hi);
    TRYC(cuda_ok(cudaStreamCreateWithPriority(&h->panel_stream, cudaStreamNonBlocking, hi), "cudaStreamCreate"));
    TRYC(cuda_ok(cudaStreamCreateWithPriority(&h->aux_stream, cudaStreamNonBlocking, hi), "cudaStreamCreate"));
  }
  if (const char* e = getenv("B200BA_GROUPED")) h->force_grouped = atoi(e);
  h->pb.n_obs = n;
  h->pb.obs_imageset = h->d_obs_imageset;
  h->pb.obs_camera = h->d_obs_camera;
  h->pb.obs_point = h->d_obs_point;
  h->pb.obs_xy = h->d_obs_xy;
  for (int i = 0; i < 2; ++i) {
    TRYC(dev_alloc(h, &h->st[i].points, 3 * static_cast<size_t>(h->n_points)));
    TRYC(dev_alloc(h, &h->st[i].rig_tr_global, 7 * static_cast<size_t>(h->n_imagesets)));
    TRYC(dev_alloc(h, &h->st[i].camera_tr_rig, 7 * static_cast<size_t>(h->n_cameras)));
    TRYC(dev_alloc(h, &h->st[i].intrinsics, h->intr_total));
    TRYC(dev_alloc(h, &h->st[i].image_tr_global, 12 * static_cast<size_t>(h->n_imagesets) * h->n_cameras));
    TRYC(dev_alloc(h, &h->st[i].tangents, h->tan_total));
  }
  TRYC(dev_alloc(h, &h->d_last_projection, n));
  TRYC(cuda_ok(cudaMemset(h->d_last_projection, 0, std::max<int64_t>(1, n) * sizeof(double2)), "memset"));
  TRYC(dev_alloc(h, &h->d_straggler_list, n));
  TRYC(dev_alloc(h, &h->d_straggler_count, 1));
  TRYC(dev_alloc(h, &h->d_info, 2));
  TRYC(dev_alloc(h, &h->d_fail, 1));
  TRYC(dev_alloc(h, &h->d_partial, cost_reduce_partial_size()));
  TRYC(dev_alloc(h, &h->d_scal, 16));
  TRYC(cuda_ok(cudaMallocHost(reinterpret_cast<void**>(&h->h_scal), 16 * sizeof(double)), "cudaMallocHost"));
  TRYC(cuda_ok(cudaMallocHost(reinterpret_cast<void**>(&h->h_flags), 4 * sizeof(int)), "cudaMallocHost"));
#undef TRYC
  *out = h;
  return 0;
}

void b200ba_destroy(b200ba_handle* h) {
  if (!h) return;
  cudaSetDevice(h->device);
  if (h->stream) cudaStreamSynchronize(h->stream);
  if (h->comm && g_nccl.CommDestroy) g_nccl.CommDestroy(h->comm);
  resolve_timings(h);
  for (auto e : h->event_pool) cudaEventDestroy(e);
  for (int i = 0; i < 2; ++i) {
    if (h->ev_syrk[i]) cudaEventDestroy(h->ev_syrk[i]);
    if (h->ev_scatter[i]) cudaEventDestroy(h->ev_scatter[i]);
  }
  if (h->ev_s_ready) cudaEventDestroy(h->ev_s_ready);
  free_handle_buffers(h);
  if (h->cublas) cublasDestroy(h->cublas);
  if (h->cusolver) cusolverDnDestroy(h->cusolver);
  if (h->stream) cudaStreamDestroy(h->stream);
  if (h->side_stream) cudaStreamDestroy(h->side_stream);
  if (h->panel_stream) cudaStreamDestroy(h->panel_stream);
  if (h->aux_stream) cudaStreamDestroy(h->aux_stream);
  dense_release(&h->dn, false);
  delete h;
}

int b200ba_set_state(b200ba_handle* h, const b200ba_state* s) {
  if (!h) return 1;
  if (!s || !s->points || !s->rig_tr_global || !s->camera_tr_rig || !s->intrinsics) {
    h->error = "NULL state array";
    return 2;
  }
  CUDA_TRY(h, cudaSetDevice(h->device));
  StateDev& d = h->st[h->cur];
  CUDA_TRY(h, cudaMemcpyAsync(d.points, s->points, 3 * sizeof(double) * h->n_points, cudaMemcpyHostToDevice, h->stream));
  CUDA_TRY(h, cudaMemcpyAsync(d.rig_tr_global, s->rig_tr_global, 7 * sizeof(double) * h->n_imagesets, cudaMemcpyHostToDevice, h->stream));
  CUDA_TRY(h, cudaMemcpyAsync(d.camera_tr_rig, s->camera_tr_rig, 7 * sizeof(double) * h->n_cameras, cudaMemcpyHostToDevice, h->stream));
  for (int c = 0; c < h->n_cameras; ++c)
    CUDA_TRY(h, cudaMemcpyAsync(d.intrinsics + h->pb.cams[c].intr_off, s->intrinsics[c],
                                sizeof(double) * intrinsics_size(h->cams_host[c]), cudaMemcpyHostToDevice, h->stream));
  if (s->last_projection) {
    CUDA_TRY(h, cudaMemcpyAsync(h->d_lp_stage, s->last_projection, 2 * sizeof(double) * h->n_obs, cudaMemcpyHostToDevice, h->stream));
    launch_permute_double2(h->n_obs, h->d_perm, h->d_lp_stage, h->d_last_projection, false, h->stream);
  } else
    CUDA_TRY(h, cudaMemsetAsync(h->d_last_projection, 0, std::max<int64_t>(1, h->n_obs) * sizeof(double2), h->stream));
  CUDA_TRY(h, cudaStreamSynchronize(h->stream));
  h->have_state = true;
  return 0;
}

int b200ba_get_state(b200ba_handle* h, b200ba_state* s) {
  if (!h) return 1;
  if (!s || !h->have_state) {
    h->error = "no state";
    return 2;
  }
  CUDA_TRY(h, cudaSetDevice(h->device));
  const StateDev& d = h->st[h->cur];
  if (s->points) CUDA_TRY(h, cudaMemcpyAsync(s->points, d.points, 3 * sizeof(double) * h->n_points, cudaMemcpyDeviceToHost, h->stream));
  if (s->rig_tr_global) CUDA_TRY(h, cudaMemcpyAsync(s->rig_tr_global, d.rig_tr_global, 7 * sizeof(double) * h->n_imagesets, cudaMemcpyDeviceToHost, h->stream));
  if (s->camera_tr_rig) CUDA_TRY(h, cudaMemcpyAsync(s->camera_tr_rig, d.camera_tr_rig, 7 * sizeof(double) * h->n_cameras, cudaMemcpyDeviceToHost, h->stream));
  if (s->intrinsics)
    for (int c = 0; c < h->n_cameras; ++c)
      CUDA_TRY(h, cudaMemcpyAsync(s->intrinsics[c], d.intrinsics + h->pb.cams[c].intr_off,
                                  sizeof(double) * intrinsics_size(h->cams_host[c]), cudaMemcpyDeviceToHost, h->stream));
  if (s->last_projection) {
    launch_permute_double2(h->n_obs, h->d_perm, h->d_last_projection, h->d_lp_stage, true, h->stream);
    CUDA_TRY(h, cudaMemcpyAsync(s->last_projection, h->d_lp_stage, 2 * sizeof(double) * h->n_obs, cudaMemcpyDeviceToHost, h->stream));
  }
  CUDA_TRY(h, cudaStreamSynchronize(h->stream));
  return 0;
}

static int copy_state_dev(b200ba_handle* h, const StateDev& src, const double2* src_lp, StateDev& dst, double2* dst_lp) {
  CUDA_TRY(h, cudaMemcpyAsync(dst.points, src.points, 3 * sizeof(double) * h->n_points, cudaMemcpyDeviceToDevice, h->stream));
  CUDA_TRY(h, cudaMemcpyAsync(dst.rig_tr_global, src.rig_tr_global, 7 * sizeof(double) * h->n_imagesets, cudaMemcpyDeviceToDevice, h->stream));
  CUDA_TRY(h, cudaMemcpyAsync(dst.camera_tr_rig, src.camera_tr_rig, 7 * sizeof(double) * h->n_cameras, cudaMemcpyDeviceToDevice, h->stream));
  CUDA_TRY(h, cudaMemcpyAsync(dst.intrinsics, src.intrinsics, sizeof(double) * h->intr_total, cudaMemcpyDeviceToDevice, h->stream));
  CUDA_TRY(h, cudaMemcpyAsync(dst_lp, src_lp, sizeof(double2) * std::max<int64_t>(1, h->n_obs), cudaMemcpyDeviceToDevice, h->stream));
  CUDA_TRY(h, cudaStreamSynchronize(h->stream));
  return 0;
}

int b200ba_snapshot_state(b200ba_handle* h) {
  if (!h) return 1;
  if (!h->have_state) {
    h->error = "no state";
    return 2;
  }
  CUDA_TRY(h, cudaSetDevice(h->device));
  if (!h->snap.points) {
    if (dev_alloc(h, &h->snap.points, 3 * static_cast<size_t>(h->n_points))) return 1;
    if (dev_alloc(h, &h->snap.rig_tr_global, 7 * static_cast<size_t>(h->n_imagesets))) return 1;
    if (dev_alloc(h, &h->snap.camera_tr_rig, 7 * static_cast<size_t>(h->n_cameras))) return 1;
    if (dev_alloc(h, &h->snap.intrinsics, h->intr_total)) return 1;
    if (dev_alloc(h, &h->d_snap_lp, h->n_obs)) return 1;
  }
  if (copy_state_dev(h, h->st[h->cur], h->d_last_projection, h->snap, h->d_snap_lp)) return 1;
  h->have_snapshot = true;
  return 0;
}

int b200ba_restore_state(b200ba_handle* h) {
  if (!h) return 1;
// ... 470 lines not shown
    if (e == cudaSuccess) e = cudaMemcpy(jac.data(), tmp, jac.size() * sizeof(double), cudaMemcpyDeviceToHost);
    cudaFree(tmp);
    CUDA_TRY(h, e);
  } else
    CUDA_TRY(h, cudaMemcpy(jac.data(), h->out.jac, jac.size() * sizeof(double), cudaMemcpyDeviceToHost));
  CUDA_TRY(h, cudaMemcpy(cell.data(), h->out.cell, n * sizeof(int32_t), cudaMemcpyDeviceToHost));
  CUDA_TRY(h, cudaMemcpy(has.data(), h->out.has_jac, n, cudaMemcpyDeviceToHost));
  std::vector<uint32_t> cams(n);
  CUDA_TRY(h, cudaMemcpy(cams.data(), h->d_obs_camera, n * sizeof(uint32_t), cudaMemcpyDeviceToHost));
  auto J = [&](int col, int r, int64_t i) { return jac[(2 * static_cast<size_t>(col) + r) * n + i]; };
  for (int64_t i = 0; i < n; ++i) {
    const int64_t o = h->perm[i];
    const bool v = has[i] == 1 || has[i] == 3;
    for (int r = 0; r < 2; ++r) {
      if (j_point) for (int j = 0; j < 3; ++j) j_point[(o * 2 + r) * 3 + j] = v ? J(L.jc_point + j, r, i) : 0.0;
      if (j_pose) for (int j = 0; j < 6; ++j) j_pose[(o * 2 + r) * 6 + j] = v ? J(L.jc_pose + j, r, i) : 0.0;
      if (j_rig) for (int j = 0; j < 6; ++j) j_rig[(o * 2 + r) * 6 + j] = (v && L.rig_in_state) ? J(L.jc_rig + j, r, i) : 0.0;
    }
    const CamDev& c = h->pb.cams[cams[i]];
    for (int k = 0; k < K; ++k) {
      const bool vk = v && !L.localize_only && k < c.K;
      if (j_intr) {
        j_intr[(o * 2 + 0) * K + k] = vk ? J(L.jc_intr + k, 0, i) : 0.0;
        j_intr[(o * 2 + 1) * K + k] = vk ? J(L.jc_intr + k, 1, i) : 0.0;
      }
      if (intr_index) {
        int idx = -1;
        if (vk) {
          int local;
          if (c.model_type == B200BA_MODEL_CENTRAL_GENERIC) {
            const int cp = k >> 1;
            local = 2 * (cell[i] + (cp & 3) + (cp >> 2) * c.gw) + (k & 1);
          } else if (c.model_type == B200BA_MODEL_NONCENTRAL_GENERIC) {
            const int cp = k / 5;
            local = 5 * (cell[i] + (cp & 3) + (cp >> 2) * c.gw) + (k - 5 * cp);
          } else {
            local = k;
          }
          idx = L.g_intr + c.upd_off + local;
        }
        intr_index[o * K + k] = idx;
      }
    }
  }
  return 0;
}

int b200ba_build_system(b200ba_handle* h, const b200ba_options* opt, int32_t n, double* H, double* b, double* cost) {
  if (int rc = check_ready(h, opt)) return rc;
  const Layout& L = h->L;
  if (n != L.dof) {
    h->error = "n does not equal the number of unknowns";
    return 2;
  }
  double c = 0, nv = 0;
  if (build_system(h, opt->huber_parameter, &c, &nv)) return 1;
  if (cost) *cost = c;
  return download_system(h, H, b);
}

int b200ba_debug_solve_step(b200ba_handle* h, const b200ba_options* opt, double lambda, int32_t n, double* H, double* b,
                            double* S, double* rhs, double* x, double* lambda_used, int32_t info[8]) {
  if (int rc = check_ready(h, opt)) return rc;
  const Layout& L = h->L;
  if (h->n_ranks > 1) {
    h->error = "b200ba_debug_solve_step: the handle is joined to a communicator";
    return 2;
  }
  if (n != L.dof || !S || !rhs || !x || !info) {
    h->error = "b200ba_debug_solve_step: n does not equal the number of unknowns, or a required output is NULL";
    return 2;
  }
  const bool any_fixed = opt->debug_fix_points || opt->debug_fix_poses || opt->debug_fix_rig_poses || opt->debug_fix_intrinsics;
  double cost = 0, n_valid = 0;
  if (build_system(h, opt->huber_parameter, &cost, &n_valid, any_fixed ? opt : nullptr)) return 1;
  if (H && b && download_system(h, H, b)) return 1;
  if (lambda < 0) lambda = opt->init_lambda_factor * h->trace_H / L.dof;
  int spd = 1;
  h->capture_S = S;
  h->capture_rhs = rhs;
  const int rc = solve_system(h, lambda, &spd);
  h->capture_S = h->capture_rhs = nullptr;
  if (rc) return rc;
  CUDA_TRY(h, cudaMemcpy(x, h->d_x, static_cast<size_t>(L.dof) * sizeof(double), cudaMemcpyDeviceToHost));
  if (lambda_used) *lambda_used = lambda;
  info[0] = spd;
  info[1] = h->use_grouped ? 1 : 0;
  info[2] = h->n_groups;
  info[3] = info[4] = info[5] = info[6] = 0;
  info[7] = h->own_dense ? h->dn.NB : 0;
  return 0;
}

int b200ba_debug_apply_update(b200ba_handle* h, const b200ba_options* opt, const double* x, int32_t n,
                              b200ba_state* out) {
  if (int rc = check_ready(h, opt)) return rc;
  const Layout& L = h->L;
  if (n != L.dof || !x || !out) {
    h->error = "b200ba_debug_apply_update: n does not equal the number of unknowns, or an argument is NULL";
    return 2;
  }
  CUDA_TRY(h, cudaMemcpyAsync(h->d_x, x, static_cast<size_t>(n) * sizeof(double), cudaMemcpyHostToDevice, h->stream));
  launch_update_state(h->pb, L, h->st[h->cur], h->st[1 - h->cur], h->d_x, h->n_control_total, h->n_param_total,
                      h->stream);
  CUDA_TRY(h, cudaGetLastError());
  b200ba_state o = *out;
  o.last_projection = nullptr;
  h->cur = 1 - h->cur;
  const int rc = b200ba_get_state(h, &o);
  h->cur = 1 - h->cur;
  return rc;
}

int b200ba_debug_cost_compare(int device, int64_t n, const double* trial, const double* base, const double* residual,
                              double out[6]) {
  if (n < 0 || (n > 0 && !trial) || !out) {
    g_create_error = "b200ba_debug_cost_compare: bad argument";
    return 2;
  }
  CallScope cs(&g_create_error);
  if (int rc = cs.use_device(device)) return rc;
  const size_t m = static_cast<size_t>(std::max<int64_t>(1, n));
  double *d_t = nullptr, *d_b = nullptr, *d_r = nullptr, *d_partial = nullptr, *d_out = nullptr;
  cs.alloc(&d_t, m);
  if (base) cs.alloc(&d_b, m);
  if (residual) cs.alloc(&d_r, 2 * m);
  cs.alloc(&d_partial, cost_reduce_partial_size());
  cs.alloc(&d_out, 6);
  if (cs.rc == 0 && n > 0) {
    cs.ok(cudaMemcpy(d_t, trial, n * sizeof(double), cudaMemcpyHostToDevice));
    if (base) cs.ok(cudaMemcpy(d_b, base, n * sizeof(double), cudaMemcpyHostToDevice));
    if (residual) cs.ok(cudaMemcpy(d_r, residual, 2 * n * sizeof(double), cudaMemcpyHostToDevice));
  }
  if (cs.rc == 0) {
    launch_cost_reduce(n, d_t, d_b, d_r, d_partial, d_out, 0);
    cs.ok(cudaGetLastError());
    cs.ok(cudaMemcpy(out, d_out, 6 * sizeof(double), cudaMemcpyDeviceToHost));
  }
  return cs.rc;
}

int b200ba_debug_nice_orientation(b200ba_handle* h, double* rot) {
  if (!h) return 1;
  if (!rot || !h->have_state) {
    h->error = "b200ba_debug_nice_orientation: rot is NULL, or no state";
    return 2;
  }
  CUDA_TRY(h, cudaSetDevice(h->device));
  if (!h->d_rot && dev_alloc(h, &h->d_rot, 9 * static_cast<size_t>(h->n_cameras))) return 1;
  launch_nice_orientation(h->pb, h->st[h->cur], h->n_cameras, h->d_rot, h->stream);
  CUDA_TRY(h, cudaGetLastError());
  CUDA_TRY(h, cudaMemcpyAsync(rot, h->d_rot, 9 * sizeof(double) * h->n_cameras, cudaMemcpyDeviceToHost, h->stream));
  CUDA_TRY(h, cudaStreamSynchronize(h->stream));
  return 0;
}

int32_t b200ba_debug_lm_events(const b200ba_handle* h, int32_t* codes, int32_t cap) {
  if (!h) return -1;
  const int32_t n = static_cast<int32_t>(h->lm_events.size());
  for (int32_t i = 0; i < n && i < cap && codes; ++i) codes[i] = h->lm_events[i];
  return n;
}

B200BA_API void b200ba_debug_set_eval_budget(int budget) { set_main_eval_budget(budget); }

B200BA_API int b200ba_debug_eval_counts(b200ba_handle* h, uint16_t* counts) {
  if (!h || !counts || !h->have_layout) return 1;
  std::vector<uint16_t> tmp(h->n_obs);
  CUDA_TRY(h, cudaMemcpy(tmp.data(), h->out.evals, h->n_obs * sizeof(uint16_t), cudaMemcpyDeviceToHost));
  for (int64_t i = 0; i < h->n_obs; ++i) counts[h->perm[i]] = tmp[i];
  return 0;
}

int b200ba_get_timings(const b200ba_handle* h, b200ba_timings* t) {
  if (!h || !t) return 1;
  *t = h->timings;
  return 0;
}

int b200ba_dense_cholesky_solve(int device, int32_t n, int32_t nb, const double* A, const double* b, double* x,
                                double* factor_ms, double* solve_ms) {
  if (n < 1 || nb < 128 || nb % 128 != 0 || !A || !b || !x) {
    g_create_error = "b200ba_dense_cholesky_solve: bad argument";
    return 2;
  }
  CallScope cs(&g_create_error);
  if (int rc = cs.use_device(device)) return rc;
  DenseCtx d;
  dense_plan(&d, n, nb, 0, 1);
  double* dA = nullptr;
  double* db = nullptr;
  cs.ok(dense_create(&d, true));
  cs.alloc(&dA, static_cast<size_t>(n) * n);
  cs.alloc(&d.S, static_cast<size_t>(d.chunk));
  cs.alloc(&d.Lpack, static_cast<size_t>(d.panel_off[d.nblk]));
  cs.alloc(&d.tmp, static_cast<size_t>(n));
  cs.alloc(&d.d_panel_off, d.panel_off.size());
  cs.alloc(&d.d_panel_h, d.panel_h.size());
  cs.alloc(&db, static_cast<size_t>(n));
  cs.alloc(&d.info, 1);
  if (cs.rc == 0) {
    cs.ok(cudaMemcpy(dA, A, static_cast<size_t>(n) * n * sizeof(double), cudaMemcpyHostToDevice));
    cs.ok(cudaMemcpy(db, b, static_cast<size_t>(n) * sizeof(double), cudaMemcpyHostToDevice));
    cs.ok(cudaMemcpy(d.d_panel_off, d.panel_off.data(), d.panel_off.size() * sizeof(int64_t), cudaMemcpyHostToDevice));
    cs.ok(cudaMemcpy(d.d_panel_h, d.panel_h.data(), d.panel_h.size() * sizeof(int), cudaMemcpyHostToDevice));
    cs.ok(cudaMemset(d.S, 0, static_cast<size_t>(d.chunk) * sizeof(double)));
    cs.ok(cudaMemset(d.info, 0, sizeof(int)));
    cs.ok(cudaMemcpy2D(d.S, d.map.ld * sizeof(double), dA, static_cast<size_t>(n) * sizeof(double),
                       static_cast<size_t>(n) * sizeof(double), n, cudaMemcpyDeviceToDevice));
    cs.ok(cudaDeviceSynchronize());
  }
  if (cs.rc == 0) {
    cs.record(0, d.s_main);
    if (dense_factor(&d)) cs.fail("b200ba_dense_cholesky_solve: kernel launch failed");
    cs.record(1, d.s_main);
    if (cs.rc == 0 && dense_solve(&d, db)) cs.fail("b200ba_dense_cholesky_solve: kernel launch failed");
    cs.record(2, d.s_main);
    cs.ok(cudaStreamSynchronize(d.s_main));
    cs.ok(cudaStreamSynchronize(d.s_panel));
  }
  if (cs.rc == 0) {
    if (factor_ms) *factor_ms = cs.elapsed_ms(0, 1);
    if (solve_ms) *solve_ms = cs.elapsed_ms(1, 2);
    int info = 0;
    cs.ok(cudaMemcpy(&info, d.info, sizeof(int), cudaMemcpyDeviceToHost));
    cs.ok(cudaMemcpy(x, db, static_cast<size_t>(n) * sizeof(double), cudaMemcpyDeviceToHost));
    if (cs.rc == 0 && info != 0) {
      g_create_error = "b200ba_dense_cholesky_solve: the matrix is not positive definite";
      cs.rc = 4;
    }
  }
  dense_release(&d, true);
  return cs.rc;
}

int b200ba_schur_solve(int device, int32_t bs, int32_t nb, int32_t nd, const double* D, const double* B,
                       const double* C, const double* b1, const double* b2, double* x) {
  if (bs < 1 || bs > 6 || nb < 0 || nd < 1 || !D || !B || !C || !b1 || !b2 || !x) {
    g_create_error = "b200ba_schur_solve: bad argument";
    return 2;
  }
  CallScope cs(&g_create_error);
  if (int rc = cs.use_device(device)) return rc;
  const int nbd = bs * nb;
  double *dD = nullptr, *dB = nullptr, *dC = nullptr, *db1 = nullptr, *db2 = nullptr, *dDinvB = nullptr, *dDinvb = nullptr,
         *dwork = nullptr;
  int *dipiv = nullptr, *dinfo = nullptr;
  cs.alloc(&dD, std::max(1, nb * bs * bs));
  cs.alloc(&dB, std::max<size_t>(1, static_cast<size_t>(nbd) * nd));
  cs.alloc(&dC, static_cast<size_t>(nd) * nd);
  cs.alloc(&db1, std::max(1, nbd));
  cs.alloc(&db2, nd);
  cs.alloc(&dDinvB, std::max<size_t>(1, static_cast<size_t>(nbd) * nd));
  cs.alloc(&dDinvb, std::max(1, nbd));
  cs.alloc(&dipiv, nd);
  cs.alloc(&dinfo, 1);
  if (cs.rc == 0) {
    cs.ok(cudaMemcpy(dD, D, sizeof(double) * nb * bs * bs, cudaMemcpyHostToDevice));
    cs.ok(cudaMemcpy(dB, B, sizeof(double) * static_cast<size_t>(nbd) * nd, cudaMemcpyHostToDevice));
    cs.ok(cudaMemcpy(dC, C, sizeof(double) * static_cast<size_t>(nd) * nd, cudaMemcpyHostToDevice));
    cs.ok(cudaMemcpy(db1, b1, sizeof(double) * nbd, cudaMemcpyHostToDevice));
    cs.ok(cudaMemcpy(db2, b2, sizeof(double) * nd, cudaMemcpyHostToDevice));
  }
  if (cs.create_solvers()) {
    const double one = 1.0, m1 = -1.0;
    launch_symmetrize(nd, dC, 0);
    launch_generic_block_inverse(bs, nb, nd, dD, dB, db1, dDinvB, dDinvb, 0);
    if (nbd > 0) {
      cublasDgemm(cs.cublas, CUBLAS_OP_N, CUBLAS_OP_T, nd, nd, nbd, &m1, dB, nd, dDinvB, nd, &one, dC, nd);
      cublasDgemv(cs.cublas, CUBLAS_OP_N, nd, nbd, &m1, dB, nd, dDinvb, 1, &one, db2, 1);
    }
    int lwork = 0;
    cusolverDnDgetrf_bufferSize(cs.cusolver, nd, nd, dC, nd, &lwork);
    cs.alloc(&dwork, std::max(1, lwork));
    cusolverDnDgetrf(cs.cusolver, nd, nd, dC, nd, dwork, dipiv, dinfo);
    cusolverDnDgetrs(cs.cusolver, CUBLAS_OP_N, nd, 1, dC, nd, dipiv, db2, nd, dinfo);
    if (nbd > 0) cublasDgemv(cs.cublas, CUBLAS_OP_T, nd, nbd, &m1, dDinvB, nd, db2, 1, &one, dDinvb, 1);
    cs.ok(cudaDeviceSynchronize());
    if (nbd > 0) cs.ok(cudaMemcpy(x, dDinvb, sizeof(double) * nbd, cudaMemcpyDeviceToHost));
    cs.ok(cudaMemcpy(x + nbd, db2, sizeof(double) * nd, cudaMemcpyDeviceToHost));
  }
  return cs.rc;
}

static int model_io(int device, const b200ba_camera* cam, const double* intrinsics, int64_t n, const double* in,
                    int in_w, double* io_pixels, double* dirs, double* origins, int32_t* ok_out, bool project) {
  if (!cam || !intrinsics || n < 0) {
    g_create_error = "bad argument";
    return 2;
  }
  CallScope cs(&g_create_error);
  if (int rc = cs.use_device(device)) return rc;
  CamDev c{};
  fill_camdev(*cam, &c);
  const int64_t ni = intrinsics_size(*cam);
  double *dintr = nullptr, *din = nullptr, *dpx = nullptr, *ddir = nullptr, *dorg = nullptr;
  int32_t* dok = nullptr;
  const size_t nn = std::max<int64_t>(1, n);
  cs.alloc(&dintr, ni);
  cs.alloc(&din, in_w * nn);
  cs.alloc(&dpx, 2 * nn);
  cs.alloc(&ddir, 3 * nn);
  cs.alloc(&dorg, 3 * nn);
  cs.alloc(&dok, nn);
  if (cs.rc == 0) {
    cs.ok(cudaMemcpy(dintr, intrinsics, sizeof(double) * ni, cudaMemcpyHostToDevice));
// ... 1507 lines not shown
```

### camera_calibration_b200/csrc/ba_kernels.cu

```cuda

#include <algorithm>
#include <cstdlib>

#include "ba_device.cuh"
#include "ba_kernels.h"

namespace b200ba {

__device__ __forceinline__ int intr_col(const CamDev& c, int cell, int k);

__device__ __forceinline__ void add_H(const Layout& L, const SystemDev& sys, int gi, int gj, double v) {
  if (gi > gj) {
    const int t = gi;
    gi = gj;
    gj = t;
  }
  if (gj < L.nbd) {
    const int blk = gi / L.bs;
    const int a = gi - blk * L.bs, b = gj - blk * L.bs;
    atomicAdd(&sys.Dblk[static_cast<int64_t>(blk) * L.dsz + a * L.bs - (a * (a - 1)) / 2 + (b - a)], v);
  } else if (gi < L.nbd) {
    atomicAdd(&sys.B[static_cast<int64_t>(gi) * L.nd + (gj - L.nbd)], v);
  } else {
    atomicAdd(&sys.C[static_cast<int64_t>(gi - L.nbd) * L.nd + (gj - L.nbd)], v);
// ... 534 lines not shown
                              uint32_t* straggler_list, int* straggler_count, cudaStream_t s,
                              cudaEvent_t main_done) {
  if (jac)
    launch_rj<true>(uniform_model, pb, L, st, last_projection, out, huber, straggler_list, straggler_count, s, main_done);
  else
    launch_rj<false>(uniform_model, pb, L, st, last_projection, out, huber, straggler_list, straggler_count, s, main_done);
}

void launch_straggler_pass(int uniform_model, bool jac, const ProblemDev& pb, const Layout& L, const StateDev& st,
                           double2* last_projection, const ObsOut& out, double huber, uint32_t* straggler_list,
                           int* straggler_count, cudaStream_t s) {
  if (jac)
    launch_stragglers<true>(uniform_model, pb, L, st, last_projection, out, huber, straggler_list, straggler_count, s);
  else
    launch_stragglers<false>(uniform_model, pb, L, st, last_projection, out, huber, straggler_list, straggler_count, s);
}

__global__ void expand_jacobian_kernel(ProblemDev pb, Layout L, StateDev st, ObsOut out, double* __restrict__ jac) {
  const int64_t o = blockIdx.x * static_cast<int64_t>(blockDim.x) + threadIdx.x;
  const int col = blockIdx.y;
  if (o >= pb.n_obs) return;
  double jx = 0.0, jy = 0.0;
  if (out.has_jac[o] == kJacValid || out.has_jac[o] == kJacLate) load_jcol(pb, L, st, out, o, col, jx, jy);
  jac[(2 * static_cast<int64_t>(col)) * pb.n_obs + o] = jx;
  jac[(2 * static_cast<int64_t>(col) + 1) * pb.n_obs + o] = jy;
}
void launch_expand_jacobian(const ProblemDev& pb, const Layout& L, const StateDev& st, const ObsOut& out, double* jac,
                            cudaStream_t s) {
  if (pb.n_obs == 0 || L.n_jcols == 0) return;
  dim3 grid(static_cast<unsigned>((pb.n_obs + 127) / 128), L.n_jcols);
  expand_jacobian_kernel<<<grid, 128, 0, s>>>(pb, L, st, out, jac);
}

__global__ void accumulate_list_kernel(ProblemDev pb, Layout L, StateDev st, ObsOut out, SystemDev sys, double huber,
                                       const uint32_t* __restrict__ list, const int* __restrict__ count) {
  const int lane = threadIdx.x & 31;
  const int64_t warp = (blockIdx.x * static_cast<int64_t>(blockDim.x) + threadIdx.x) >> 5;
  const int64_t n_warps = (static_cast<int64_t>(gridDim.x) * blockDim.x) >> 5;
  const int64_t n = pb.n_obs;
  for (int64_t li = warp; li < *count; li += n_warps) {
    const int64_t o = list[li];
    if (out.has_jac[o] != kJacLate) continue;
    const int cam = static_cast<int>(pb.obs_camera[o]);
    const int iset = static_cast<int>(pb.obs_imageset[o]);
    const int pidx = static_cast<int>(pb.obs_point[o]);
    const CamDev& c = pb.cams[cam];
    const int cell = out.cell[o];
    const double rx = out.residual[o], ry = out.residual[n + o];
    const double w = huber_weight_sq(huber, rx * rx + ry * ry);
    const int K = L.localize_only ? 0 : c.K;
    const int nc = 9 + (L.rig_in_state ? 6 : 0) + K;
    auto jcol = [&](int e) -> int {
      if (e < 9) return e;
      if (L.rig_in_state && e < 15) return L.jc_rig + (e - 9);
      return L.jc_intr + (e - (L.rig_in_state ? 15 : 9));
    };
    auto gidx = [&](int e) -> int {
      if (e < 3) return L.g_point + 3 * pidx + e;
      if (e < 9) return L.g_pose + 6 * iset + (e - 3);
      if (L.rig_in_state && e < 15) return L.g_rig + 6 * cam + (e - 9);
      return L.g_intr + intr_col(c, cell, e - (L.rig_in_state ? 15 : 9));
    };
    for (int p = lane; p < nc * nc; p += 32) {
      const int i = p / nc, j = p - i * nc;
      if (j < i) continue;
      const int ci = jcol(i), cj = jcol(j);
      double ax, ay, bx, by;
      load_jcol(pb, L, st, out, o, ci, ax, ay);
      load_jcol(pb, L, st, out, o, cj, bx, by);
      const double v = w * (ax * bx + ay * by);
      add_H(L, sys, gidx(i), gidx(j), v);
    }
    for (int i = lane; i < nc; i += 32) {
      const int ci = jcol(i);
      double ax, ay;
      load_jcol(pb, L, st, out, o, ci, ax, ay);
      const double v = w * (ax * rx + ay * ry);
      add_b(L, sys, gidx(i), v);
    }
    __syncwarp();
    if (lane == 0) out.has_jac[o] = kJacValid;
  }
}
void launch_accumulate_list(const ProblemDev& pb, const Layout& L, const StateDev& st, const ObsOut& out,
                            const SystemDev& sys, double huber, const uint32_t* list, const int* count, cudaStream_t s) {
  if (pb.n_obs == 0) return;
  accumulate_list_kernel<<<296, 128, 0, s>>>(pb, L, st, out, sys, huber, list, count);
}

__device__ __forceinline__ int intr_col(const CamDev& c, int cell, int k) {
  if (c.model_type == B200BA_MODEL_CENTRAL_GENERIC) {
    const int cp = k >> 1;
    return c.upd_off + 2 * (cell + (cp & 3) + (cp >> 2) * c.gw) + (k & 1);
  } else if (c.model_type == B200BA_MODEL_NONCENTRAL_GENERIC) {
    const int cp = k / 5;
    return c.upd_off + 5 * (cell + (cp & 3) + (cp >> 2) * c.gw) + (k - 5 * cp);
  }
  return c.upd_off + k;
}

__device__ __forceinline__ double warp_sum(double v) {
#pragma unroll
  for (int off = 16; off > 0; off >>= 1) v += __shfl_xor_sync(0xffffffffu, v, off);
  return v;
}

__global__ void __launch_bounds__(128)
    accumulate_scatter_kernel(ProblemDev pb, Layout L, StateDev st, ObsOut out, SystemDev sys, double huber) {
  const int64_t o = blockIdx.x * static_cast<int64_t>(blockDim.x) + threadIdx.x;
  const int64_t n = pb.n_obs;
  if (o >= n || out.has_jac[o] != kJacValid) return;
  const int iset = static_cast<int>(pb.obs_imageset[o]);
  const int cam = static_cast<int>(pb.obs_camera[o]);
  const int pidx = static_cast<int>(pb.obs_point[o]);
  const double rx = out.residual[o], ry = out.residual[n + o];
  const double w = huber_weight_sq(huber, rx * rx + ry * ry);
  double jpx[3], jpy[3], jox[6], joy[6], jrx6[6], jry6[6];
  if (out.compact) {
    double jp[2][3], jo[2][6], jr[2][6];
    compact_small_blocks(pb, L, st, out, o, jp, jo, jr);
#pragma unroll
    for (int a = 0; a < 3; ++a) {
      jpx[a] = jp[0][a];
      jpy[a] = jp[1][a];
    }
#pragma unroll
    for (int a = 0; a < 6; ++a) {
      jox[a] = jo[0][a];
      joy[a] = jo[1][a];
      jrx6[a] = jr[0][a];
      jry6[a] = jr[1][a];
    }
  } else {
#pragma unroll
    for (int a = 0; a < 3; ++a) {
      jpx[a] = out.jac[(2 * static_cast<int64_t>(L.jc_point + a)) * n + o];
      jpy[a] = out.jac[(2 * static_cast<int64_t>(L.jc_point + a) + 1) * n + o];
    }
#pragma unroll
    for (int a = 0; a < 6; ++a) {
      jox[a] = out.jac[(2 * static_cast<int64_t>(L.jc_pose + a)) * n + o];
      joy[a] = out.jac[(2 * static_cast<int64_t>(L.jc_pose + a) + 1) * n + o];
      if (L.rig_in_state) {
        jrx6[a] = out.jac[(2 * static_cast<int64_t>(L.jc_rig + a)) * n + o];
        jry6[a] = out.jac[(2 * static_cast<int64_t>(L.jc_rig + a) + 1) * n + o];
      }
    }
  }
  const int gp = L.g_point + 3 * pidx, go = L.g_pose + 6 * iset;
#pragma unroll
  for (int a = 0; a < 3; ++a) {
    const double wx_ = w * jpx[a], wy_ = w * jpy[a];
#pragma unroll
    for (int b = a; b < 3; ++b) add_H(L, sys, gp + a, gp + b, wx_ * jpx[b] + wy_ * jpy[b]);
#pragma unroll
    for (int b = 0; b < 6; ++b) add_H(L, sys, gp + a, go + b, wx_ * jox[b] + wy_ * joy[b]);
    add_b(L, sys, gp + a, wx_ * rx + wy_ * ry);
  }
#pragma unroll
  for (int a = 0; a < 6; ++a) {
    const double wx_ = w * jox[a], wy_ = w * joy[a];
#pragma unroll
    for (int b = a; b < 6; ++b) add_H(L, sys, go + a, go + b, wx_ * jox[b] + wy_ * joy[b]);
    add_b(L, sys, go + a, wx_ * rx + wy_ * ry);
  }
  if (L.rig_in_state) {
    const int gr = L.g_rig + 6 * cam;
#pragma unroll
    for (int b = 0; b < 6; ++b) {
      const double wx_ = w * jrx6[b], wy_ = w * jry6[b];
#pragma unroll
      for (int a = 0; a < 3; ++a) add_H(L, sys, gp + a, gr + b, wx_ * jpx[a] + wy_ * jpy[a]);
#pragma unroll
      for (int a = 0; a < 6; ++a) add_H(L, sys, go + a, gr + b, wx_ * jox[a] + wy_ * joy[a]);
    }
  }
}

void launch_accumulate_scatter(const ProblemDev& pb, const Layout& L, const StateDev& st, const ObsOut& out,
                               const SystemDev& sys, double huber, cudaStream_t s) {
  const int threads = 128;
  const unsigned blocks = static_cast<unsigned>((pb.n_obs + threads - 1) / threads);
  if (blocks == 0) return;
  accumulate_scatter_kernel<<<blocks, threads, 0, s>>>(pb, L, st, out, sys, huber);
}

constexpr int kCellChunk = 128;
constexpr int kCellTile = 32;
constexpr int kCellThreads = 256;
constexpr uint32_t kInvalidKey = 0xffffffffu;

__device__ __forceinline__ uint32_t cell_key(const ProblemDev& pb, const ObsOut& out, int64_t pos) {
  if (out.has_jac[pos] != kJacValid) return kInvalidKey;
  return (pb.obs_camera[pos] << 24) | static_cast<uint32_t>(out.cell[pos]);
}

template <int MAXPAIRS>
__global__ void __launch_bounds__(kCellThreads)
    accumulate_cells_kernel(ProblemDev pb, Layout L, StateDev st, ObsOut out, SystemDev sys, double huber) {
  extern __shared__ double smem[];
  static_assert(kCellTile == 32, "one lane per observation of a tile");
  const int64_t n = pb.n_obs;
  const int64_t begin = static_cast<int64_t>(blockIdx.x) * kCellChunk;
  const int64_t end = min(n, begin + kCellChunk);
  const int rigE = L.rig_in_state ? 6 : 0;
  const int Emax = rigE + L.Kmax;
  const int S = Emax | 1;
  double* sJx = smem;
  double* sJy = sJx + kCellTile * S;
  double* sR = sJy + kCellTile * S;
  double* sPx = sR + 2 * kCellTile;
  double* sPy = sPx + 9 * kCellTile;
  __shared__ double sObs[kCellTile * 16];
  __shared__ double sTan[96];
  __shared__ uint32_t sKey[kCellTile];
  __shared__ int sPoint[kCellTile];
  __shared__ int sIset[kCellTile];
  const int warp = threadIdx.x >> 5, lane = threadIdx.x & 31;
  constexpr int kWarps = kCellThreads / 32;
  constexpr int kSlots = (kMaxK + 31) / 32;

  double acc[MAXPAIRS];
  double accb = 0;
  int pi[MAXPAIRS], pj[MAXPAIRS];

  int64_t pos = begin;
  while (pos < end) {
    const uint32_t key = cell_key(pb, out, pos);
    if (key == kInvalidKey) {
      ++pos;
      continue;
    }
    const int cam = static_cast<int>(key >> 24);
    const int cell = static_cast<int>(key & 0xffffffu);
    const CamDev& c = pb.cams[cam];
    const int K = L.localize_only ? 0 : c.K;
    const int E = rigE + K;
    const int npairs = E * (E + 1) / 2;
#pragma unroll
    for (int q = 0; q < MAXPAIRS; ++q) {
      acc[q] = 0;
      const int p = threadIdx.x + q * kCellThreads;
      int i = 0, j = 0;
      if (p < npairs) {
        int lo = 0, hi = E - 1;
        while (lo < hi) {
          const int mid = (lo + hi + 1) >> 1;
          if (mid * E - mid * (mid - 1) / 2 <= p) lo = mid; else hi = mid - 1;
        }
        i = lo;
        j = i + (p - (i * E - i * (i - 1) / 2));
      }
      pi[q] = i;
      pj[q] = j;
    }
    accb = 0;
    int gck[kSlots];
#pragma unroll
    for (int s = 0; s < kSlots; ++s) {
      const int kk = lane + 32 * s;
      gck[s] = (kk < K) ? (L.g_intr + intr_col(c, cell, kk) - L.nbd) : -1;
    }
    bool run_done = false;
    while (!run_done && pos < end) {
      const int tile_n = static_cast<int>(min(static_cast<int64_t>(kCellTile), end - pos));
      __syncthreads();
      if (threadIdx.x < tile_n) sKey[threadIdx.x] = cell_key(pb, out, pos + threadIdx.x);
      __syncthreads();
      int run_n = 0;
      while (run_n < tile_n && sKey[run_n] == key) ++run_n;
      if (run_n < tile_n) run_done = true;
      if (out.compact) {
        if (warp == 0 && lane < run_n) {
          const int64_t o = pos + lane;
          const double rx = out.residual[o], ry = out.residual[n + o];
          const double sw = sqrt(huber_weight_sq(huber, rx * rx + ry * ry));
          double wx[4], dwx[4], wy[4], dwy[4];
          bspline_basis(out.cjac[12 * n + o], wx, dwx);
          bspline_basis(out.cjac[13 * n + o], wy, dwy);
          double* so = sObs + lane * 16;
          so[0] = sw;
#pragma unroll
          for (int q = 0; q < 4; ++q) {
            so[1 + q] = wx[q];
            so[5 + q] = wy[q];
          }
#pragma unroll
          for (int q = 0; q < 6; ++q) so[9 + q] = out.cjac[static_cast<int64_t>(6 + q) * n + o];
          sR[2 * lane] = sw * rx;
          sR[2 * lane + 1] = sw * ry;
          sPoint[lane] = static_cast<int>(pb.obs_point[o]);
          sIset[lane] = static_cast<int>(pb.obs_imageset[o]);
        }
        if (warp == 1 && lane < run_n) {
          const int64_t o = pos + lane;
          const double rx = out.residual[o], ry = out.residual[n + o];
          const double sw = sqrt(huber_weight_sq(huber, rx * rx + ry * ry));
          double jp[2][3], jo[2][6], jr[2][6];
          compact_small_blocks(pb, L, st, out, o, jp, jo, jr);
#pragma unroll
          for (int q = 0; q < 3; ++q) {
            sPx[lane * 9 + q] = sw * jp[0][q];
            sPy[lane * 9 + q] = sw * jp[1][q];
          }
#pragma unroll
          for (int q = 0; q < 6; ++q) {
            sPx[lane * 9 + 3 + q] = sw * jo[0][q];
            sPy[lane * 9 + 3 + q] = sw * jo[1][q];
            if (rigE) {
              sJx[lane * S + q] = sw * jr[0][q];
              sJy[lane * S + q] = sw * jr[1][q];
            }
          }
        }
        if (threadIdx.x >= 64 && threadIdx.x < 64 + 96 && K > 0) {
          const int q = threadIdx.x - 64, cp = q / 6;
          sTan[q] = st.tangents[c.tan_off + 6 * (static_cast<int64_t>(cell) + (cp & 3) + static_cast<int64_t>(cp >> 2) * c.gw) + (q - 6 * cp)];
        }
        __syncthreads();
        if (lane < run_n) {
          const double* so = sObs + lane * 16;
          for (int k = warp; k < K; k += kWarps) {
            const int cp = k >> 1;
            const double wk = so[0] * so[1 + (cp & 3)] * so[5 + (cp >> 2)];
            const double* t = sTan + 6 * cp + 3 * (k & 1);
            sJx[lane * S + rigE + k] = wk * (so[9] * t[0] + so[10] * t[1] + so[11] * t[2]);
            sJy[lane * S + rigE + k] = wk * (so[12] * t[0] + so[13] * t[1] + so[14] * t[2]);
          }
        }
      } else if (lane < run_n) {
        const int64_t o = pos + lane;
        const double rx = out.residual[o], ry = out.residual[n + o];
        const double sw = sqrt(huber_weight_sq(huber, rx * rx + ry * ry));
        for (int e = warp; e < E; e += kWarps) {
          const int col = (e < rigE) ? (L.jc_rig + e) : (L.jc_intr + (e - rigE));
          sJx[lane * S + e] = sw * out.jac[(2 * static_cast<int64_t>(col)) * n + o];
          sJy[lane * S + e] = sw * out.jac[(2 * static_cast<int64_t>(col) + 1) * n + o];
        }
        for (int r9 = warp; r9 < 9; r9 += kWarps) {
          const int col = (r9 < 3) ? (L.jc_point + r9) : (L.jc_pose + (r9 - 3));
          sPx[lane * 9 + r9] = sw * out.jac[(2 * static_cast<int64_t>(col)) * n + o];
          sPy[lane * 9 + r9] = sw * out.jac[(2 * static_cast<int64_t>(col) + 1) * n + o];
        }
        if (warp == 0) {
          sR[2 * lane] = sw * rx;
          sR[2 * lane + 1] = sw * ry;
          sPoint[lane] = static_cast<int>(pb.obs_point[o]);
          sIset[lane] = static_cast<int>(pb.obs_imageset[o]);
        }
      }
      __syncthreads();
      if (K > 0) {
        for (int q = warp; q < run_n * 9; q += kWarps) {
          const int t = q / 9, r9 = q - 9 * t;
          const double px = sPx[t * 9 + r9], py = sPy[t * 9 + r9];
          const int grow = (r9 < 3) ? (L.g_point + 3 * sPoint[t] + r9) : (L.g_pose + 6 * sIset[t] + (r9 - 3));
          double* rowp = (grow < L.nbd) ? (sys.B + static_cast<int64_t>(grow) * L.nd)
                                        : (sys.C + static_cast<int64_t>(grow - L.nbd) * L.nd);
          const double* jx = sJx + t * S + rigE;
          const double* jy = sJy + t * S + rigE;
#pragma unroll
          for (int s = 0; s < kSlots; ++s) {
            const int kk = lane + 32 * s;
            if (kk < K) atomicAdd(rowp + gck[s], fma(px, jx[kk], py * jy[kk]));
          }
        }
      }
#pragma unroll
      for (int q = 0; q < MAXPAIRS; ++q) {
        if (threadIdx.x + q * kCellThreads < npairs) {
          double a = acc[q];
          const double* xi = sJx + pi[q];
          const double* xj = sJx + pj[q];
          const double* yi = sJy + pi[q];
          const double* yj = sJy + pj[q];
          for (int t = 0; t < run_n; ++t) a = fma(xi[t * S], xj[t * S], fma(yi[t * S], yj[t * S], a));
          acc[q] = a;
        }
      }
      if (threadIdx.x < E) {
        double a = accb;
        for (int t = 0; t < run_n; ++t)
          a = fma(sJx[t * S + threadIdx.x], sR[2 * t], fma(sJy[t * S + threadIdx.x], sR[2 * t + 1], a));
        accb = a;
      }
      pos += run_n;
    }
    auto gcol = [&](int e) -> int {
      return (e < rigE) ? (L.g_rig + 6 * cam + e) : (L.g_intr + intr_col(c, cell, e - rigE));
    };
#pragma unroll
    for (int q = 0; q < MAXPAIRS; ++q) {
      if (threadIdx.x + q * kCellThreads < npairs) {
        const int gi = gcol(pi[q]) - L.nbd, gj = gcol(pj[q]) - L.nbd;
        atomicAdd(&sys.C[static_cast<int64_t>(gi) * L.nd + gj], acc[q]);
      }
    }
    if (threadIdx.x < E) atomicAdd(&sys.bd[gcol(threadIdx.x) - L.nbd], accb);
  }
}

void launch_accumulate_cells(const ProblemDev& pb, const Layout& L, const StateDev& st, const ObsOut& out,
                             const SystemDev& sys, double huber, cudaStream_t s) {
  if (pb.n_obs == 0) return;
  const int rigE = L.rig_in_state ? 6 : 0;
  const int Emax = rigE + L.Kmax;
  if (Emax == 0) return;
  const int npairs = Emax * (Emax + 1) / 2;
  const int per_thread = (npairs + kCellThreads - 1) / kCellThreads;
  const size_t smem = (2 * static_cast<size_t>(kCellTile) * (Emax | 1) + 2 * kCellTile + 18 * kCellTile) * sizeof(double);
  const unsigned blocks = static_cast<unsigned>((pb.n_obs + kCellChunk - 1) / kCellChunk);
#define B200BA_LAUNCH_CELLS(MP)                                                                              \
  do {                                                                                                       \
    cudaFuncSetAttribute(accumulate_cells_kernel<MP>, cudaFuncAttributeMaxDynamicSharedMemorySize,           \
                         static_cast<int>(smem));                                                            \
    accumulate_cells_kernel<MP><<<blocks, kCellThreads, smem, s>>>(pb, L, st, out, sys, huber);              \
  } while (0)
  if (per_thread <= 1)
    B200BA_LAUNCH_CELLS(1);
  else if (per_thread <= 3)
    B200BA_LAUNCH_CELLS(3);
  else if (per_thread <= 4)
    B200BA_LAUNCH_CELLS(4);
  else if (per_thread <= 13)
    B200BA_LAUNCH_CELLS(13);
  else
    B200BA_LAUNCH_CELLS(15);
#undef B200BA_LAUNCH_CELLS
}

template <int BS>
__global__ void schur_blocks_kernel(int n_blocks, const double* __restrict__ Dblk, const double* __restrict__ bp,
                                    double lambda, double* __restrict__ Linv, double* __restrict__ v, int* fail) {
  constexpr int DSZ = BS * (BS + 1) / 2;
  const int p = blockIdx.x * blockDim.x + threadIdx.x;
  if (p >= n_blocks) return;
  const double* D = Dblk + static_cast<int64_t>(DSZ) * p;
  double A[BS][BS], Lm[BS][BS], Li[BS][BS];
#pragma unroll
  for (int a = 0; a < BS; ++a)
#pragma unroll
    for (int b = a; b < BS; ++b) {
      const double d = D[a * BS - (a * (a - 1)) / 2 + (b - a)] + (a == b ? lambda : 0.0);
      A[a][b] = d;
      A[b][a] = d;
    }
  bool bad = false;
#pragma unroll
  for (int j = 0; j < BS; ++j) {
    double s = A[j][j];
#pragma unroll
    for (int k2 = 0; k2 < j; ++k2) s -= Lm[j][k2] * Lm[j][k2];
    if (!(s > 0)) bad = true;
    const double ljj = sqrt(s);
    Lm[j][j] = ljj;
#pragma unroll
    for (int i = j + 1; i < BS; ++i) {
      double t = A[i][j];
#pragma unroll
      for (int k2 = 0; k2 < j; ++k2) t -= Lm[i][k2] * Lm[j][k2];
      Lm[i][j] = t / ljj;
    }
  }
  if (bad) *fail = 1;
#pragma unroll
  for (int c2 = 0; c2 < BS; ++c2) {
#pragma unroll
    for (int i = 0; i < BS; ++i) {
      if (i < c2) {
        Li[i][c2] = 0;
      } else {
        double t = (i == c2) ? 1.0 : 0.0;
#pragma unroll
        for (int k2 = c2; k2 < i; ++k2) t -= Lm[i][k2] * Li[k2][c2];
        Li[i][c2] = t / Lm[i][i];
      }
    }
  }
  double* out = Linv + static_cast<int64_t>(DSZ) * p;
#pragma unroll
  for (int i = 0; i < BS; ++i)
#pragma unroll
    for (int j = 0; j <= i; ++j) out[(i * (i + 1)) / 2 + j] = Li[i][j];
#pragma unroll
  for (int i = 0; i < BS; ++i) {
    double t = 0;
#pragma unroll
    for (int j = 0; j <= i; ++j) t += Li[i][j] * bp[BS * p + j];
    v[BS * p + i] = t;
  }
}
void launch_schur_blocks(int bs, int n_blocks, const double* Dblk, const double* bp, double lambda, double* Linv,
                         double* v, int* fail, cudaStream_t s) {
  if (n_blocks == 0) return;
  if (bs == 3)
    schur_blocks_kernel<3><<<(n_blocks + 127) / 128, 128, 0, s>>>(n_blocks, Dblk, bp, lambda, Linv, v, fail);
  else
    schur_blocks_kernel<6><<<(n_blocks + 127) / 128, 128, 0, s>>>(n_blocks, Dblk, bp, lambda, Linv, v, fail);
}

template <int BS>
__global__ void schur_scale_rows_kernel(int nd, const double* __restrict__ B, const double* __restrict__ Linv,
                                        double* __restrict__ W) {
  constexpr int DSZ = BS * (BS + 1) / 2;
  const int p = blockIdx.y;
  const int col = blockIdx.x * blockDim.x + threadIdx.x;
  if (col >= nd) return;
  const double* Li = Linv + static_cast<int64_t>(DSZ) * p;
  const int64_t r0 = static_cast<int64_t>(BS) * p * nd + col;
  double b[BS];
#pragma unroll
  for (int i = 0; i < BS; ++i) b[i] = B[r0 + static_cast<int64_t>(i) * nd];
#pragma unroll
  for (int i = 0; i < BS; ++i) {
    double t = 0;
#pragma unroll
    for (int j = 0; j <= i; ++j) t = fma(Li[(i * (i + 1)) / 2 + j], b[j], t);
    W[r0 + static_cast<int64_t>(i) * nd] = t;
  }
}
void launch_schur_scale_rows(int bs, int n_blocks, int nd, const double* B, const double* Linv, double* W,
                             cudaStream_t s) {
  if (n_blocks == 0 || nd == 0) return;
  dim3 grid((nd + 255) / 256, n_blocks);
  if (bs == 3)
    schur_scale_rows_kernel<3><<<grid, 256, 0, s>>>(nd, B, Linv, W);
  else
    schur_scale_rows_kernel<6><<<grid, 256, 0, s>>>(nd, B, Linv, W);
}

template <int BS>
__global__ void schur_backsub_kernel(int n_blocks, const double* __restrict__ Linv, const double* __restrict__ y,
                                     double* __restrict__ xp) {
  constexpr int DSZ = BS * (BS + 1) / 2;
  const int p = blockIdx.x * blockDim.x + threadIdx.x;
  if (p >= n_blocks) return;
  const double* Li = Linv + static_cast<int64_t>(DSZ) * p;
#pragma unroll
  for (int j = 0; j < BS; ++j) {
    double t = 0;
#pragma unroll
    for (int i = j; i < BS; ++i) t += Li[(i * (i + 1)) / 2 + j] * y[BS * p + i];
    xp[BS * p + j] = t;
  }
}
void launch_schur_backsub(int bs, int n_blocks, const double* Linv, const double* y, double* xp, cudaStream_t s) {
  if (n_blocks == 0) return;
  if (bs == 3)
    schur_backsub_kernel<3><<<(n_blocks + 127) / 128, 128, 0, s>>>(n_blocks, Linv, y, xp);
  else
    schur_backsub_kernel<6><<<(n_blocks + 127) / 128, 128, 0, s>>>(n_blocks, Linv, y, xp);
}


__global__ void group_support_kernel(int bs, int nblocks, int nd, const double* __restrict__ B,
                                     const int* __restrict__ group_of_block, uint8_t* __restrict__ flags) {
  const int c = blockIdx.x * blockDim.x + threadIdx.x;
  const int blk0 = blockIdx.y * 8;
  if (c >= nd) return;
  for (int blk = blk0; blk < min(blk0 + 8, nblocks); ++blk) {
    bool nz = false;
    for (int r = 0; r < bs; ++r) nz |= (B[(static_cast<int64_t>(blk) * bs + r) * nd + c] != 0.0);
    if (nz) flags[static_cast<int64_t>(group_of_block[blk]) * nd + c] = 1;
  }
}
void launch_group_support(int bs, int nblocks, int nd, const double* B, const int* group_of_block, uint8_t* flags,
                          cudaStream_t s) {
  if (nblocks == 0 || nd == 0) return;
  dim3 grid((nd + 255) / 256, (nblocks + 7) / 8);
  group_support_kernel<<<grid, 256, 0, s>>>(bs, nblocks, nd, B, group_of_block, flags);
}

__global__ void compact_columns_kernel(int nd, const uint8_t* __restrict__ flags, int* __restrict__ cols,
                                       int* __restrict__ count) {
  const int g = blockIdx.x;
  const uint8_t* f = flags + static_cast<int64_t>(g) * nd;
  int* out = cols + static_cast<int64_t>(g) * nd;
  __shared__ int warp_sums[32];
  __shared__ int base;
  if (threadIdx.x == 0) base = 0;
  __syncthreads();
// ... 3328 lines not shown
```

### camera_calibration_b200/csrc/ba_kernels.h

```cpp
#pragma once
#include <vector>

#include "ba_common.h"

namespace b200ba {

void launch_prepare_state(const ProblemDev& pb, const Layout& L, const StateDev& st, int64_t n_control_total,
                          cudaStream_t s);
void launch_residual_jacobian(int uniform_model, bool jac, const ProblemDev& pb, const Layout& L,
                              const StateDev& st, double2* last_projection, const ObsOut& out, double huber,
                              uint32_t* straggler_list, int* straggler_count, cudaStream_t s,
                              cudaEvent_t main_done = nullptr);
void launch_straggler_pass(int uniform_model, bool jac, const ProblemDev& pb, const Layout& L, const StateDev& st,
                           double2* last_projection, const ObsOut& out, double huber, uint32_t* straggler_list,
                           int* straggler_count, cudaStream_t s);
void launch_accumulate_list(const ProblemDev& pb, const Layout& L, const StateDev& st, const ObsOut& out,
                            const SystemDev& sys, double huber, const uint32_t* list, const int* count, cudaStream_t s);
void launch_expand_jacobian(const ProblemDev& pb, const Layout& L, const StateDev& st, const ObsOut& out, double* jac,
                            cudaStream_t s);
void set_main_eval_budget(int budget);
void launch_accumulate_scatter(const ProblemDev& pb, const Layout& L, const StateDev& st, const ObsOut& out,
                               const SystemDev& sys, double huber, cudaStream_t s);
void launch_accumulate_cells(const ProblemDev& pb, const Layout& L, const StateDev& st, const ObsOut& out,
                             const SystemDev& sys, double huber, cudaStream_t s);
void launch_schur_blocks(int bs, int n_blocks, const double* Dblk, const double* bp, double lambda, double* Linv,
                         double* v, int* fail, cudaStream_t s);
void launch_schur_scale_rows(int bs, int n_blocks, int nd, const double* B, const double* Linv, double* W,
                             cudaStream_t s);
void launch_schur_backsub(int bs, int n_blocks, const double* Linv, const double* y, double* xp, cudaStream_t s);
void launch_group_support(int bs, int nblocks, int nd, const double* B, const int* group_of_block, uint8_t* flags,
                          cudaStream_t s);
void launch_compact_columns(int ngroups, int nd, const uint8_t* flags, int* cols, int* count, cudaStream_t s);
void launch_gather_scale(int bs, int nblocks_in_group, int nd, int m, int ldw, const double* B, const double* Linv,
                         const int* blocks, const int* cols, double* Wc, cudaStream_t s);
void launch_scatter_sub(int nd, int m, const int* cols, const double* P, double* S, cudaStream_t s);
void launch_block_solve_t(int bs, int n_blocks, const double* Linv, const double* v, double* u, cudaStream_t s);
void launch_block_backsub2(int bs, int n_blocks, const double* Linv, const double* u, const double* t, double* xb,
                           cudaStream_t s);
void launch_add_diagonal(int n, double* M, int64_t ld, double lambda, cudaStream_t s);
void launch_trace(int n_blocks, int bs, const double* Dblk, int nd, const double* C, double* out, cudaStream_t s);
void launch_update_state(const ProblemDev& pb, const Layout& L, const StateDev& src, const StateDev& dst,
                         const double* x, int64_t n_control_total, int64_t n_param_total, cudaStream_t s);
void launch_cost_reduce(int64_t n, const double* trial, const double* base, const double* residual, double* partial,
                        double* out, cudaStream_t s);
int cost_reduce_partial_size();
void launch_project_points(const CamDev& c, const double* intr, int64_t n, const double* lp, double* px, int32_t* ok,
                           cudaStream_t s);
void launch_unproject_pixels(const CamDev& c, const double* intr, int64_t n, const double* px, double* dirs,
                             double* origins, int32_t* ok, cudaStream_t s);
void launch_calibration_report(const ProblemDev& pb, int n_cameras, const StateDev& st, const ReportDev& r,
                               cudaStream_t s);
int report_partial_size(int n_cameras);
void launch_compare_models(const CamDev& a, const double* ga, const CamDev& b, const double* gb, const CompareDev& d,
                           cudaStream_t s);
void launch_localization_sample(const CamDev& gt, const double* ggt, const CamDev& cmp, const double* gcmp,
                                int64_t trials, uint64_t seed, const LocalizationDev& d, cudaStream_t s);
void launch_localization_pose(int64_t trials, const LocalizationDev& d, cudaStream_t s);
int64_t sweep_partial_blocks(int nx, int ny);
void launch_reconstruction_sweep(const CamDev& c1, const double* intr1, const CamDev& c2, const double* intr2,
                                 int step, int nx, int ny, double* partial, double* sums, cudaStream_t s);
void launch_reconstruction_directions(const CamDev& c1, const double* intr1, const CamDev& c2, const double* intr2,
                                      int step, int nx, int ny, int32_t* ok, double* dirs, cudaStream_t s);
void launch_line_pass(const CamDev& c, const double* intr, const LineOffsetsDev& d, cudaStream_t s);
void launch_line_system(int mode, int64_t n, const double c[3], const LineOffsetsDev& d, cudaStream_t s);
int line_system_partial_size();
void launch_line_outputs(const CamDev& c, const double center[3], const LineOffsetsDev& d, int obj_step, int nx,
                         int64_t n_obj, cudaStream_t s);
void launch_report_errors(const ProblemDev& pb, int n_cameras, const StateDev& st, const ReportDev& r, cudaStream_t s);
void launch_report_select(int n_ranges, int ranks, const int64_t* off, const double* mag, unsigned int* select_hist,
                          ReportCam* rc, cudaStream_t s);
void launch_delete_outliers(const ProblemDev& pb, int n_imagesets, const ReportDev& r, const uint32_t* perm,
                            int64_t a, int64_t n, float factor, int w, int h, const OutlierDev& d, cudaStream_t s);
void launch_render_voronoi(int w, int h, int64_t n, const int2* sites, const float* colors, int nch, const VoronoiGrid& g,
                           uint8_t* img0, uint8_t* img1, cudaStream_t s);
VoronoiGrid voronoi_grid_geometry(int64_t lo_x, int64_t lo_y, int64_t hi_x, int64_t hi_y);
void launch_report_sites(const ProblemDev& pb, const ReportDev& r, int64_t n_groups, const int* group_off,
                         const uint32_t* group_obs, int2* sites, float* colors, cudaStream_t s);
void launch_observation_directions(const CamDev& c, const double* intr, uint8_t* img, cudaStream_t s);
void launch_visualize_orientation(const double* params, int w, int h, double2* win, double* rot, cudaStream_t s);
void launch_visualize_camera(const double* params, int w, int h, const double* rot, uint8_t* img, double* dirs,
                             cudaStream_t s);
void launch_intersect_features(int d, int64_t n_lists, int64_t max_list, const int64_t* off, float2* xy, float bound,
                               uint8_t* keep, float2* centres, int* n_centres, unsigned long long* counts,
                               cudaStream_t s);
constexpr int kSynthTile = 16;
constexpr int kSynthMaxVerts = 4;
struct SynthParams {
  int w, h, tiles_x, tiles_y, words, n_poly;
  float fx, fy, cx, cy;
  int pattern_w, pattern_h, squares_x, squares_y, num_tags;
  float page_w, page_h, start_x, start_y, end_x, end_y;
  int4 tags[B200BA_PATTERN_MAX_TAGS];
};
void launch_render_pattern(const SynthParams& p, int n_img, const float2* verts, const int8_t* nv, const float* poses,
                           const uint8_t* pattern, double2* proj, int4* range, uint32_t* bits, uint8_t* images,
                           cudaStream_t s);
struct RefineParams {
  int w, h;
  int half;
  int n_samples, n_match;
  int type;
  int num_star_segments, squares_x, squares_y, num_tags;
  int4 tags[B200BA_PATTERN_MAX_TAGS];
};
void launch_refine_features(const RefineParams& p, int64_t n, const b200ba_feature_prediction* pred,
                            const uint8_t* images, const float2* samples, float2* xy, float* cost, int* status,
                            cudaStream_t s);
void launch_generic_block_inverse(int bs, int nb, int nd, const double* D, const double* B, const double* b1,
                                  double* DinvB, double* Dinvb, cudaStream_t s);
void launch_symmetrize(int n, double* M, cudaStream_t s);
void launch_dirfit_tangents(int G, const double* grid, double* tan, cudaStream_t s);
void launch_dirfit(bool jac, int gw, int64_t n, const double* gp, const double* dirs, const double* grid,
                   const double* tan, double* H, double* b, int dof, double* cost, double* cost_sum, cudaStream_t s);
void launch_dirfit_update(int G, const double* grid, const double* x, double* out, cudaStream_t s);
void launch_permute_double2(int64_t n, const uint32_t* perm, const double2* src, double2* dst, bool scatter,
                            cudaStream_t s);


void launch_mask_fixed(const Layout& L, const SystemDev& sys, const FixedRanges& fr, double unit, cudaStream_t s);
void launch_nice_orientation(const ProblemDev& pb, const StateDev& st, int n_cameras, double* rot, cudaStream_t s);

struct DenseMap {
  int nb;
  int ranks;
  int blocks_per_rank;
  int64_t ld;
  __host__ __device__ __forceinline__ int slot(int block) const { return (block % ranks) * blocks_per_rank + block / ranks; }
  __host__ __device__ __forceinline__ int64_t col_offset(int c) const {
    const int b = c / nb;
    return (static_cast<int64_t>(slot(b)) * nb + (c - b * nb)) * ld;
  }
};

struct GemmArgs {
  int M, N, K;
  const double* A;
  int64_t lda;
  const double* B;
  int64_t ldb;
  double* C;
  int64_t ldc;
  double alpha, beta;
  bool a_aligned, b_aligned;
  const int* cols;
  DenseMap map;
  int64_t n_tiles_lower;
  bool owned_only;
  int rank, col_base;
};
inline bool gemm_operand_aligned(const double* p, int64_t ld) {
  return (reinterpret_cast<uintptr_t>(p) % 16 == 0) && (ld % 2 == 0);
}
int launch_dgemm_nt(const GemmArgs& g, bool lower, bool scatter, cudaStream_t s, bool one_tile_per_cta = false);

int gemv_t_partial_size(int rows, int cols);
void launch_gemv_t(int rows, int cols, int64_t ld, const double* B, const double* u, double alpha, double* y, double* partial,
                   cudaStream_t s);
void launch_gemv_n(int rows, int cols, int64_t ld, const double* B, const double* x, double* t, cudaStream_t s);
void launch_add_diagonal_map(int n, double* S, const DenseMap& map, double lambda, cudaStream_t s);

struct DenseCtx {
  int n = 0, NB = 256, nblk = 0, ntiles = 0;
  int rank = 0, ranks = 1;
  DenseMap map{};
  int64_t chunk = 0;
  std::vector<int64_t> panel_off;
  std::vector<int> panel_h;
  double* S = nullptr;
  double* Lpack = nullptr;
  double* tmp = nullptr;
  int64_t* d_panel_off = nullptr;
  int* d_panel_h = nullptr;
  int* info = nullptr;
  cudaStream_t s_main = nullptr, s_panel = nullptr, s_aux = nullptr;
  cudaEvent_t ev_ready[2] = {nullptr, nullptr}, ev_main[2] = {nullptr, nullptr}, ev_half2[2] = {nullptr, nullptr}, ev_misc = nullptr;
  int (*bcast)(double* buf, size_t count, int root, cudaStream_t s, void* user) = nullptr;
  void* user = nullptr;
// ... 7 lines not shown
```

### include/b200ba.h

```cpp
#ifndef B200BA_H_
#define B200BA_H_

#include <stdint.h>

#if defined(__GNUC__)
#define B200BA_API __attribute__((visibility("default")))
#else
#define B200BA_API
#endif

#ifdef __cplusplus
extern "C" {
#endif

enum {
  B200BA_MODEL_CENTRAL_GENERIC = 0,
  B200BA_MODEL_NONCENTRAL_GENERIC = 1,
  B200BA_MODEL_CENTRAL_THIN_PRISM_FISHEYE = 2,
  B200BA_MODEL_CENTRAL_OPENCV = 3,
  B200BA_MODEL_CENTRAL_RADIAL = 4
};

enum {
  B200BA_SCHUR_DENSE = 0,
// ... 186 lines not shown
B200BA_API int b200ba_fitting_images(int device, const b200ba_camera* cam_a, const double* intr_a,
                                     const b200ba_camera* cam_b, const double* intr_b, b200ba_fitting_report* report,
                                     uint8_t* error_magnitudes, uint8_t* error_direction_angles,
                                     uint8_t* error_directions, uint8_t* reprojection_magnitudes,
                                     uint8_t* reprojections, double* device_ms);

typedef struct b200ba_localization_report {
  int64_t trial_count;
  double average_error;
  double median_error;
  double max_error;
  int64_t total_iterations;
  int64_t redraws;
  int32_t max_iterations;
} b200ba_localization_report;
B200BA_API int b200ba_localization_accuracy(int device, const b200ba_camera* gt_cam, const double* gt_intr,
                                            const b200ba_camera* cam, const double* intr, int64_t trials,
                                            uint64_t seed, b200ba_localization_report* report, float* errors,
                                            double* poses, float* samples, double* device_ms);

typedef struct b200ba_reconstruction_comparison {
  int64_t direction_pairs;
  double direction_sums[9];
  double intrinsics1_r_intrinsics2[9];
  double rotation_cost;
  double scale;
  double firstimage1_tr_firstimage2[16];
  double endpoint_translation_difference, trajectory_length1, trajectory_length2, relative_endpoint_difference;
} b200ba_reconstruction_comparison;
B200BA_API int b200ba_compare_reconstructions(int device, const b200ba_camera* cam1, const double* intr1,
                                              const b200ba_camera* cam2, const double* intr2, int32_t n_images,
                                              const double* rig_tr_global1, const double* camera_tr_rig1,
                                              const double* rig_tr_global2, const double* camera_tr_rig2,
                                              int32_t pixel_step, b200ba_reconstruction_comparison* out,
                                              double* device_ms);
B200BA_API int b200ba_reconstruction_directions(int device, const b200ba_camera* cam1, const double* intr1,
                                                const b200ba_camera* cam2, const double* intr2, int32_t pixel_step,
                                                int32_t* ok, double* directions);
B200BA_API int b200ba_reconstruction_alignment(int64_t direction_pairs, const double* direction_sums, int32_t n_images,
                                               const double* rig_tr_global1, const double* camera_tr_rig1,
                                               const double* rig_tr_global2, const double* camera_tr_rig2,
                                               b200ba_reconstruction_comparison* out);

typedef struct b200ba_line_offsets_report {
  double center[3];
  int64_t line_count;
  double line_distance_sum, line_distance_max, line_distance_median;
  double max_line_offset_extent;
  double initial_cost, final_cost;
  int32_t num_iterations_performed, lm_attempts;
} b200ba_line_offsets_report;
B200BA_API int b200ba_line_offsets(int device, const b200ba_camera* cam, const double* intrinsics,
                                   b200ba_line_offsets_report* report, uint8_t* image, double* offsets, int32_t obj_step,
                                   double* obj_lines, int64_t* n_obj, double* device_ms);

typedef struct b200ba_intersection_report {
  int64_t intersections;
  int64_t kept;
  int64_t uncovered;
  int64_t capped;
} b200ba_intersection_report;
B200BA_API int b200ba_intersect_features(int device, int32_t n_datasets, int64_t n_lists, const int64_t* list_offsets,
                                         const float* xy, double threshold, uint8_t* keep,
                                         b200ba_intersection_report* report, double* device_ms);

#define B200BA_PATTERN_MAX_TAGS 16
typedef struct b200ba_pattern_tag {
  int32_t x, y, width, height, index;
} b200ba_pattern_tag;
typedef struct b200ba_pattern {
  int32_t squares_x, squares_y, num_star_segments, num_tags;
  float page_width_mm, page_height_mm, pattern_start_x_mm, pattern_start_y_mm, pattern_end_x_mm, pattern_end_y_mm;
  b200ba_pattern_tag tags[B200BA_PATTERN_MAX_TAGS];
} b200ba_pattern;
B200BA_API int b200ba_synthetic_poses(const b200ba_pattern* pattern, int32_t pattern_w, int32_t pattern_h,
                                      int32_t width, int32_t height, const float* fx_fy_cx_cy, int64_t n,
                                      uint64_t seed, double* camera_tr_global, int64_t* attempts);
B200BA_API int b200ba_render_pattern_images(int device, const b200ba_pattern* pattern, const uint8_t* pattern_image,
                                            int32_t pattern_w, int32_t pattern_h, int32_t width, int32_t height,
                                            const float* fx_fy_cx_cy, int64_t n, const double* camera_tr_global,
                                            uint8_t* images, double* device_ms);

#define B200BA_REFINE_MAX_HALF_EXTENT 32
B200BA_API int b200ba_feature_samples(int32_t window_half_extent, int32_t n, float* xy);

#define B200BA_REFINE_GRADIENTS_XY 0
#define B200BA_REFINE_GRADIENT_MAGNITUDE 1
#define B200BA_REFINE_INTENSITIES 2
#define B200BA_REFINE_NO_REFINEMENT 3
#define B200BA_REFINE_ACCEPTED 0
#define B200BA_REFINE_IMAGE_BORDER 1
#define B200BA_REFINE_OUTSIDE_PATTERN 2
#define B200BA_REFINE_MATCH_OUTSIDE 3
#define B200BA_REFINE_MATCH_LEFT_WINDOW 4
#define B200BA_REFINE_MATCH_NOT_CONVERGED 5
#define B200BA_REFINE_MATCH_BAD_FACTOR 6
#define B200BA_REFINE_SYM_OUTSIDE 7
#define B200BA_REFINE_SYM_LEFT_WINDOW 8
#define B200BA_REFINE_SYM_NOT_CONVERGED 9
#define B200BA_REFINE_INCONSISTENT 10
typedef struct b200ba_feature_prediction {
  int64_t image;
  float position[2];
  int32_t pattern_coordinate[2];
  float local_pixel_tr_pattern[9];
} b200ba_feature_prediction;
B200BA_API int b200ba_refine_features(int device, const b200ba_pattern* pattern, const uint8_t* images, int32_t width,
                                      int32_t height, int64_t n_images, const float* samples, int32_t n_samples,
                                      int32_t window_half_extent, int32_t refinement_type, int64_t n_features,
                                      const b200ba_feature_prediction* predictions, float* xy, float* final_cost,
                                      int32_t* status, double* device_ms);

#define B200BA_NCCL_UNIQUE_ID_BYTES 128
B200BA_API int b200ba_nccl_unique_id(uint8_t id[B200BA_NCCL_UNIQUE_ID_BYTES]);
B200BA_API int b200ba_comm_init(b200ba_handle* h, const uint8_t id[B200BA_NCCL_UNIQUE_ID_BYTES], int rank,
                     int n_ranks);

typedef struct b200ba_timings {
  double jacobian_kernel_ms;
  int32_t jacobian_kernel_launches;
  double accumulate_ms;
  double schur_ms;
  double factor_ms;
  double trial_cost_ms;
  double update_ms;
  double allreduce_ms;
  double total_ms;
  int64_t kernel_launches;
  double straggler_ms;
  double solve_ms;
  double contraction_flops;
  double factor_flops;
  int32_t lm_attempts;
  int32_t build_count;
} b200ba_timings;
B200BA_API int b200ba_get_timings(const b200ba_handle* h, b200ba_timings* t);

B200BA_API const char* b200ba_version(void);

B200BA_API void b200ba_debug_set_eval_budget(int budget);
B200BA_API int b200ba_debug_eval_counts(b200ba_handle* h, uint16_t* counts);
B200BA_API int b200ba_debug_solve_step(b200ba_handle* h, const b200ba_options* opt, double lambda, int32_t n,
                                       double* H, double* b, double* S, double* rhs, double* x,
                                       double* lambda_used, int32_t info[8]);
B200BA_API int b200ba_debug_apply_update(b200ba_handle* h, const b200ba_options* opt, const double* x, int32_t n,
                                         b200ba_state* out);
B200BA_API int b200ba_debug_cost_compare(int device, int64_t n, const double* trial, const double* base,
                                         const double* residual, double out[6]);
B200BA_API int b200ba_debug_nice_orientation(b200ba_handle* h, double* rot);
#define B200BA_LM_ACCEPTED 1
#define B200BA_LM_REJECTED_COST 2
#define B200BA_LM_REFUSED_PIVOT 3
B200BA_API int32_t b200ba_debug_lm_events(const b200ba_handle* h, int32_t* codes, int32_t cap);

#ifdef __cplusplus
}
#endif
#endif
```

Measured before the change: 23.38.

## Accumulate point/pose-intrinsic Schur blocks via window-sorted runs with shared-memory reduction

Adds host-built orderings that group observations by camera, an 8x8 grid window and a pose or point entity. Two new kernels accumulate each run's off-diagonal pose/point-by-intrinsic block in shared memory and flush it once with atomics. The per-observation global atomics in the cell kernel for these blocks are removed, and the pose/point diagonal work moves into the new kernels. This cuts atomic contention on the B/C rows in exchange for extra setup sorting, two more launches and larger shared-memory use.

```diff
diff --git a/camera_calibration_b200/cabi.py b/camera_calibration_b200/cabi.py
--- a/camera_calibration_b200/cabi.py
+++ b/camera_calibration_b200/cabi.py
@@ -523,6 +523,7 @@
     "b200ba_debug_cost_compare": (C.c_int, [C.c_int, C.c_int64, _D, _D, _D, _D]),
     "b200ba_debug_nice_orientation": (C.c_int, [C.c_void_p, _D]),
     "b200ba_debug_lm_events": (C.c_int32, [C.c_void_p, _I32, C.c_int32]),
+    "b200ba_debug_window_runs": (C.c_int, [C.POINTER(Problem), C.c_int32, C.POINTER(C.c_uint32), _I32, _I32, _I32]),
 }
 
 LM_ACCEPTED, LM_REJECTED_COST, LM_REFUSED_PIVOT = 1, 2, 3
diff --git a/camera_calibration_b200/csrc/ba_common.h b/camera_calibration_b200/csrc/ba_common.h
--- a/camera_calibration_b200/csrc/ba_common.h
+++ b/camera_calibration_b200/csrc/ba_common.h
@@ -71,6 +71,14 @@
   int32_t* cell;
   uint8_t* has_jac;
   uint16_t* evals;
+};
+
+constexpr int kRunWindow = B200BA_RUN_WINDOW;
+struct RunsDev {
+  int n_runs;
+  const uint32_t* order;
+  const int* off;
+  const int* win;
 };
 
 struct SystemDev {
diff --git a/camera_calibration_b200/csrc/ba_host.cu b/camera_calibration_b200/csrc/ba_host.cu
--- a/camera_calibration_b200/csrc/ba_host.cu
+++ b/camera_calibration_b200/csrc/ba_host.cu
@@ -111,6 +111,7 @@
   int *d_info = nullptr, *d_fail = nullptr;
   std::vector<uint32_t> perm;
   uint32_t* d_perm = nullptr;
+  RunsDev runs[2]{};
   double2* d_lp_stage = nullptr;
   uint32_t* d_straggler_list = nullptr;
   int* d_straggler_count = nullptr;
@@ -260,6 +261,57 @@
 
 int64_t align32(int64_t n) { return (n + 31) / 32 * 32; }
 
+void cell_major_order(const b200ba_problem* p, const CamDev* cams, std::vector<uint32_t>& perm,
+                      std::vector<uint32_t>& cell) {
+  const int64_t n = p->n_obs;
+  std::vector<uint32_t> key(n);
+  for (int64_t o = 0; o < n; ++o) {
+    const uint32_t cam = p->obs_camera[o];
+    const CamDev& cd = cams[cam];
+    uint32_t cl = 0;
+    if (cd.gw > 0) {
+      const double gx = 1.0 + cd.gmul_x * (static_cast<double>(p->obs_xy[2 * o]) - cd.min_x);
+      const double gy = 1.0 + cd.gmul_y * (static_cast<double>(p->obs_xy[2 * o + 1]) - cd.min_y);
+      const int x0 = std::min(std::max(static_cast<int>(std::floor(gx)) - 1, 0), cd.gw - 4);
+      const int y0 = std::min(std::max(static_cast<int>(std::floor(gy)) - 1, 0), cd.gh - 4);
+      cl = static_cast<uint32_t>(x0 + y0 * cd.gw);
+    }
+    key[o] = (cam << 24) | cl;
+  }
+  perm.resize(n);
+  for (int64_t o = 0; o < n; ++o) perm[o] = static_cast<uint32_t>(o);
+  std::stable_sort(perm.begin(), perm.end(), [&](uint32_t a, uint32_t b) { return key[a] < key[b]; });
+  cell.resize(n);
+  for (int64_t i = 0; i < n; ++i) cell[i] = key[perm[i]] & 0xffffffu;
+}
+
+void build_runs(const CamDev* cams, int64_t n, const uint32_t* cam, const uint32_t* cell, const uint32_t* ent,
+                std::vector<uint32_t>& order, std::vector<int>& off, std::vector<int>& win) {
+  std::vector<uint64_t> key(n);
+  std::vector<int> wins(n);
+  for (int64_t i = 0; i < n; ++i) {
+    const CamDev& cd = cams[cam[i]];
+    int w = 0;
+    if (cd.gw > 0) {
+      const int x0 = static_cast<int>(cell[i] % cd.gw), y0 = static_cast<int>(cell[i] / cd.gw);
+      w = x0 / kRunWindow * kRunWindow + y0 / kRunWindow * kRunWindow * cd.gw;
+    }
+    wins[i] = w;
+    key[i] = (static_cast<uint64_t>(cam[i]) << 56) | (static_cast<uint64_t>(w) << 32) | ent[i];
+  }
+  order.resize(n);
+  for (int64_t i = 0; i < n; ++i) order[i] = static_cast<uint32_t>(i);
+  std::stable_sort(order.begin(), order.end(), [&](uint32_t a, uint32_t b) { return key[a] < key[b]; });
+  off.clear();
+  win.clear();
+  for (int64_t i = 0; i < n; ++i)
+    if (i == 0 || key[order[i]] != key[order[i - 1]]) {
+      off.push_back(static_cast<int>(i));
+      win.push_back(wins[order[i]]);
+    }
+  off.push_back(static_cast<int>(n));
+}
+
 cudaEvent_t get_event(b200ba_handle* h) {
   if (!h->event_pool.empty()) {
     cudaEvent_t e = h->event_pool.back();
@@ -622,6 +674,9 @@
     ScopedPhase ph(h, PH_ACC);
     CUDA_TRY(h, cudaMemsetAsync(h->sys.base, 0, h->sys.total * sizeof(double), h->stream));
     launch_accumulate_scatter(h->pb, h->L, h->st[h->cur], h->out, h->sys, huber, h->stream);
+    for (int k = 0; k < 2; ++k)
+      launch_accumulate_runs(h->pb, h->L, h->st[h->cur], h->out, h->sys, huber, h->runs[k], k == 0, h->stream);
+    h->timings.kernel_launches += 2;
     if (!h->L.localize_only || h->L.rig_in_state) {
       launch_accumulate_cells(h->pb, h->L, h->st[h->cur], h->out, h->sys, huber, h->stream);
       h->timings.kernel_launches += 1;
@@ -1014,6 +1069,12 @@
   F(h->out_trial.residual); F(h->out_trial.cost);
   F(h->sys.base); F(h->d_W); F(h->d_S); F(h->d_Linv); F(h->d_v); F(h->d_y); F(h->d_x); F(h->d_potrf_work);
   F(h->d_info); F(h->d_fail); F(h->d_straggler_list); F(h->d_straggler_count); F(h->d_perm); F(h->d_lp_stage);
+  for (RunsDev& r : h->runs) {
+    if (r.order) cudaFree(const_cast<uint32_t*>(r.order));
+    if (r.off) cudaFree(const_cast<int*>(r.off));
+    if (r.win) cudaFree(const_cast<int*>(r.win));
+    r = RunsDev{};
+  }
   F(h->d_group_of_block); F(h->d_group_blocks); F(h->d_flags); F(h->d_cols); F(h->d_count); F(h->d_Wc); F(h->d_P); F(h->d_u);
   if (h->h_count) cudaFreeHost(h->h_count);
   h->h_count = nullptr;
@@ -1311,6 +1372,36 @@
 
 const char* b200ba_last_error(const b200ba_handle* h) { return h ? h->error.c_str() : g_create_error.c_str(); }
 
+static int check_problem(const b200ba_problem* p) {
+  if (p->n_cameras < 1 || p->n_cameras > kMaxCameras) {
+    g_create_error = "n_cameras out of range (1..8)";
+    return 2;
+  }
+  for (int c = 0; c < p->n_cameras; ++c) {
+    const int t = p->cameras[c].model_type;
+    if (t != B200BA_MODEL_CENTRAL_GENERIC && t != B200BA_MODEL_NONCENTRAL_GENERIC && t != B200BA_MODEL_CENTRAL_OPENCV) {
+      g_create_error = "camera model not on the accelerated path (central-generic, noncentral-generic, central-opencv)";
+      return 2;
+    }
+    if (t != B200BA_MODEL_CENTRAL_OPENCV && (p->cameras[c].grid_width < 4 || p->cameras[c].grid_height < 4)) {
+      g_create_error = "generic models need a grid of at least 4x4 control points";
+      return 2;
+    }
+  }
+  if (p->n_obs >= (1LL << 31)) {
+    g_create_error = "n_obs must be < 2^31";
+    return 2;
+  }
+  for (int64_t o = 0; o < p->n_obs; ++o) {
+    if (p->obs_imageset[o] >= static_cast<uint32_t>(p->n_imagesets) || p->obs_point[o] >= static_cast<uint32_t>(p->n_points) ||
+        p->obs_camera[o] >= static_cast<uint32_t>(p->n_cameras)) {
+      g_create_error = "observation index out of range";
+      return 2;
+    }
+  }
+  return 0;
+}
+
 int b200ba_create(const b200ba_problem* p, int device, b200ba_handle** out) {
   if (!p || !out) {
     g_create_error = "NULL argument";
@@ -1322,32 +1413,7 @@
     g_create_error = "no CUDA device available (this library has no CPU fallback)";
     return 3;
   }
-  if (p->n_cameras < 1 || p->n_cameras > kMaxCameras) {
-    g_create_error = "n_cameras out of range (1..8)";
-    return 2;
-  }
-  for (int c = 0; c < p->n_cameras; ++c) {
-    const int t = p->cameras[c].model_type;
-    if (t != B200BA_MODEL_CENTRAL_GENERIC && t != B200BA_MODEL_NONCENTRAL_GENERIC && t != B200BA_MODEL_CENTRAL_OPENCV) {
-      g_create_error = "camera model not on the accelerated path (central-generic, noncentral-generic, central-opencv)";
-      return 2;
-    }
-    if (t != B200BA_MODEL_CENTRAL_OPENCV && (p->cameras[c].grid_width < 4 || p->cameras[c].grid_height < 4)) {
-      g_create_error = "generic models need a grid of at least 4x4 control points";
-      return 2;
-    }
-  }
-  if (p->n_obs >= (1LL << 31)) {
-    g_create_error = "n_obs must be < 2^31";
-    return 2;
-  }
-  for (int64_t o = 0; o < p->n_obs; ++o) {
-    if (p->obs_imageset[o] >= static_cast<uint32_t>(p->n_imagesets) || p->obs_point[o] >= static_cast<uint32_t>(p->n_points) ||
-        p->obs_camera[o] >= static_cast<uint32_t>(p->n_cameras)) {
-      g_create_error = "observation index out of range";
-      return 2;
-    }
-  }
+  if (int rc = check_problem(p)) return rc;
   b200ba_handle* h = new b200ba_handle();
   auto fail = [&](int rc) {
     g_create_error = h->error;
@@ -1413,31 +1479,34 @@
   TRYC(dev_alloc(h, &h->d_obs_point, n));
   TRYC(dev_alloc(h, &h->d_obs_xy, n));
   if (n > 0) {
-    std::vector<uint32_t> key(n);
-    for (int64_t o = 0; o < n; ++o) {
-      const uint32_t cam = p->obs_camera[o];
-      const CamDev& cd = h->pb.cams[cam];
-      uint32_t cell = 0;
-      if (cd.gw > 0) {
-        const double gx = 1.0 + cd.gmul_x * (static_cast<double>(p->obs_xy[2 * o]) - cd.min_x);
-        const double gy = 1.0 + cd.gmul_y * (static_cast<double>(p->obs_xy[2 * o + 1]) - cd.min_y);
-        const int x0 = std::min(std::max(static_cast<int>(std::floor(gx)) - 1, 0), cd.gw - 4);
-        const int y0 = std::min(std::max(static_cast<int>(std::floor(gy)) - 1, 0), cd.gh - 4);
-        cell = static_cast<uint32_t>(x0 + y0 * cd.gw);
-      }
-      key[o] = (cam << 24) | cell;
-    }
-    h->perm.resize(n);
-    for (int64_t o = 0; o < n; ++o) h->perm[o] = static_cast<uint32_t>(o);
-    std::stable_sort(h->perm.begin(), h->perm.end(), [&](uint32_t a, uint32_t b) { return key[a] < key[b]; });
-    std::vector<uint32_t> t32(n);
+    std::vector<uint32_t> cell;
+    cell_major_order(p, h->pb.cams, h->perm, cell);
+    std::vector<uint32_t> t32(n), c32(n), p32(n);
     std::vector<float> txy(2 * n);
     for (int64_t i = 0; i < n; ++i) t32[i] = p->obs_imageset[h->perm[i]];
     TRYC(cuda_ok(cudaMemcpy(h->d_obs_imageset, t32.data(), n * sizeof(uint32_t), cudaMemcpyHostToDevice), "H2D"));
-    for (int64_t i = 0; i < n; ++i) t32[i] = p->obs_camera[h->perm[i]];
-    TRYC(cuda_ok(cudaMemcpy(h->d_obs_camera, t32.data(), n * sizeof(uint32_t), cudaMemcpyHostToDevice), "H2D"));
-    for (int64_t i = 0; i < n; ++i) t32[i] = p->obs_point[h->perm[i]];
-    TRYC(cuda_ok(cudaMemcpy(h->d_obs_point, t32.data(), n * sizeof(uint32_t), cudaMemcpyHostToDevice), "H2D"));
+    for (int64_t i = 0; i < n; ++i) c32[i] = p->obs_camera[h->perm[i]];
+    TRYC(cuda_ok(cudaMemcpy(h->d_obs_camera, c32.data(), n * sizeof(uint32_t), cudaMemcpyHostToDevice), "H2D"));
+    for (int64_t i = 0; i < n; ++i) p32[i] = p->obs_point[h->perm[i]];
+    TRYC(cuda_ok(cudaMemcpy(h->d_obs_point, p32.data(), n * sizeof(uint32_t), cudaMemcpyHostToDevice), "H2D"));
+    for (int k = 0; k < 2; ++k) {
+      std::vector<uint32_t> order;
+      std::vector<int> off, win;
+      build_runs(h->pb.cams, n, c32.data(), cell.data(), k == 0 ? t32.data() : p32.data(), order, off, win);
+      RunsDev& r = h->runs[k];
+      uint32_t* d_order = nullptr;
+      int *d_off = nullptr, *d_win = nullptr;
+      TRYC(dev_alloc(h, &d_order, n));
+      TRYC(dev_alloc(h, &d_off, off.size()));
+      TRYC(dev_alloc(h, &d_win, win.size()));
+      r.order = d_order;
+      r.off = d_off;
+      r.win = d_win;
+      r.n_runs = static_cast<int>(win.size());
+      TRYC(cuda_ok(cudaMemcpy(d_order, order.data(), n * sizeof(uint32_t), cudaMemcpyHostToDevice), "H2D"));
+      TRYC(cuda_ok(cudaMemcpy(d_off, off.data(), off.size() * sizeof(int), cudaMemcpyHostToDevice), "H2D"));
+      TRYC(cuda_ok(cudaMemcpy(d_win, win.data(), win.size() * sizeof(int), cudaMemcpyHostToDevice), "H2D"));
+    }
     for (int64_t i = 0; i < n; ++i) {
       txy[2 * i] = p->obs_xy[2 * h->perm[i]];
       txy[2 * i + 1] = p->obs_xy[2 * h->perm[i] + 1];
@@ -2214,6 +2283,32 @@
   CUDA_TRY(h, cudaGetLastError());
   CUDA_TRY(h, cudaMemcpyAsync(rot, h->d_rot, 9 * sizeof(double) * h->n_cameras, cudaMemcpyDeviceToHost, h->stream));
   CUDA_TRY(h, cudaStreamSynchronize(h->stream));
+  return 0;
+}
+
+int b200ba_debug_window_runs(const b200ba_problem* p, int32_t pose_rows, uint32_t* order, int32_t* run_off,
+                             int32_t* run_win, int32_t* n_runs) {
+  if (!p || !order || !run_off || !run_win || !n_runs) {
+    g_create_error = "NULL argument";
+    return 2;
+  }
+  if (int rc = check_problem(p)) return rc;
+  CamDev cams[kMaxCameras];
+  for (int c = 0; c < p->n_cameras; ++c) fill_camdev(p->cameras[c], &cams[c]);
+  const int64_t n = p->n_obs;
+  std::vector<uint32_t> perm, cell, cam(n), ent(n);
+  cell_major_order(p, cams, perm, cell);
+  for (int64_t i = 0; i < n; ++i) {
+    cam[i] = p->obs_camera[perm[i]];
+    ent[i] = pose_rows ? p->obs_imageset[perm[i]] : p->obs_point[perm[i]];
+  }
+  std::vector<uint32_t> ord;
+  std::vector<int> off, win;
+  build_runs(cams, n, cam.data(), cell.data(), ent.data(), ord, off, win);
+  for (int64_t i = 0; i < n; ++i) order[i] = perm[ord[i]];
+  std::copy(off.begin(), off.end(), run_off);
+  std::copy(win.begin(), win.end(), run_win);
+  *n_runs = static_cast<int32_t>(win.size());
   return 0;
 }
 
diff --git a/camera_calibration_b200/csrc/ba_kernels.cu b/camera_calibration_b200/csrc/ba_kernels.cu
--- a/camera_calibration_b200/csrc/ba_kernels.cu
+++ b/camera_calibration_b200/csrc/ba_kernels.cu
@@ -710,17 +710,7 @@
   for (int a = 0; a < 3; ++a) {
     const double wx_ = w * jpx[a], wy_ = w * jpy[a];
 #pragma unroll
-    for (int b = a; b < 3; ++b) add_H(L, sys, gp + a, gp + b, wx_ * jpx[b] + wy_ * jpy[b]);
-#pragma unroll
     for (int b = 0; b < 6; ++b) add_H(L, sys, gp + a, go + b, wx_ * jox[b] + wy_ * joy[b]);
-    add_b(L, sys, gp + a, wx_ * rx + wy_ * ry);
-  }
-#pragma unroll
-  for (int a = 0; a < 6; ++a) {
-    const double wx_ = w * jox[a], wy_ = w * joy[a];
-#pragma unroll
-    for (int b = a; b < 6; ++b) add_H(L, sys, go + a, go + b, wx_ * jox[b] + wy_ * joy[b]);
-    add_b(L, sys, go + a, wx_ * rx + wy_ * ry);
   }
   if (L.rig_in_state) {
     const int gr = L.g_rig + 6 * cam;
@@ -767,16 +757,11 @@
   double* sJx = smem;
   double* sJy = sJx + kCellTile * S;
   double* sR = sJy + kCellTile * S;
-  double* sPx = sR + 2 * kCellTile;
-  double* sPy = sPx + 9 * kCellTile;
   __shared__ double sObs[kCellTile * 16];
   __shared__ double sTan[96];
   __shared__ uint32_t sKey[kCellTile];
-  __shared__ int sPoint[kCellTile];
-  __shared__ int sIset[kCellTile];
   const int warp = threadIdx.x >> 5, lane = threadIdx.x & 31;
   constexpr int kWarps = kCellThreads / 32;
-  constexpr int kSlots = (kMaxK + 31) / 32;
 
   double acc[MAXPAIRS];
   double accb = 0;
@@ -813,12 +798,6 @@
       pj[q] = j;
     }
     accb = 0;
-    int gck[kSlots];
-#pragma unroll
-    for (int s = 0; s < kSlots; ++s) {
-      const int kk = lane + 32 * s;
-      gck[s] = (kk < K) ? (L.g_intr + intr_col(c, cell, kk) - L.nbd) : -1;
-    }
     bool run_done = false;
     while (!run_done && pos < end) {
       const int tile_n = static_cast<int>(min(static_cast<int64_t>(kCellTile), end - pos));
@@ -847,28 +826,17 @@
           for (int q = 0; q < 6; ++q) so[9 + q] = out.cjac[static_cast<int64_t>(6 + q) * n + o];
           sR[2 * lane] = sw * rx;
           sR[2 * lane + 1] = sw * ry;
-          sPoint[lane] = static_cast<int>(pb.obs_point[o]);
-          sIset[lane] = static_cast<int>(pb.obs_imageset[o]);
         }
-        if (warp == 1 && lane < run_n) {
+        if (rigE && warp == 1 && lane < run_n) {
           const int64_t o = pos + lane;
           const double rx = out.residual[o], ry = out.residual[n + o];
           const double sw = sqrt(huber_weight_sq(huber, rx * rx + ry * ry));
           double jp[2][3], jo[2][6], jr[2][6];
           compact_small_blocks(pb, L, st, out, o, jp, jo, jr);
 #pragma unroll
-          for (int q = 0; q < 3; ++q) {
-            sPx[lane * 9 + q] = sw * jp[0][q];
-            sPy[lane * 9 + q] = sw * jp[1][q];
-          }
-#pragma unroll
           for (int q = 0; q < 6; ++q) {
-            sPx[lane * 9 + 3 + q] = sw * jo[0][q];
-            sPy[lane * 9 + 3 + q] = sw * jo[1][q];
-            if (rigE) {
-              sJx[lane * S + q] = sw * jr[0][q];
-              sJy[lane * S + q] = sw * jr[1][q];
-            }
+            sJx[lane * S + q] = sw * jr[0][q];
+            sJy[lane * S + q] = sw * jr[1][q];
           }
         }
         if (threadIdx.x >= 64 && threadIdx.x < 64 + 96 && K > 0) {
@@ -895,35 +863,12 @@
           sJx[lane * S + e] = sw * out.jac[(2 * static_cast<int64_t>(col)) * n + o];
           sJy[lane * S + e] = sw * out.jac[(2 * static_cast<int64_t>(col) + 1) * n + o];
         }
-        for (int r9 = warp; r9 < 9; r9 += kWarps) {
-          const int col = (r9 < 3) ? (L.jc_point + r9) : (L.jc_pose + (r9 - 3));
-          sPx[lane * 9 + r9] = sw * out.jac[(2 * static_cast<int64_t>(col)) * n + o];
-          sPy[lane * 9 + r9] = sw * out.jac[(2 * static_cast<int64_t>(col) + 1) * n + o];
-        }
         if (warp == 0) {
           sR[2 * lane] = sw * rx;
           sR[2 * lane + 1] = sw * ry;
-          sPoint[lane] = static_cast<int>(pb.obs_point[o]);
-          sIset[lane] = static_cast<int>(pb.obs_imageset[o]);
         }
       }
       __syncthreads();
-      if (K > 0) {
-        for (int q = warp; q < run_n * 9; q += kWarps) {
-          const int t = q / 9, r9 = q - 9 * t;
-          const double px = sPx[t * 9 + r9], py = sPy[t * 9 + r9];
-          const int grow = (r9 < 3) ? (L.g_point + 3 * sPoint[t] + r9) : (L.g_pose + 6 * sIset[t] + (r9 - 3));
-          double* rowp = (grow < L.nbd) ? (sys.B + static_cast<int64_t>(grow) * L.nd)
-                                        : (sys.C + static_cast<int64_t>(grow - L.nbd) * L.nd);
-          const double* jx = sJx + t * S + rigE;
-          const double* jy = sJy + t * S + rigE;
-#pragma unroll
-          for (int s = 0; s < kSlots; ++s) {
-            const int kk = lane + 32 * s;
-            if (kk < K) atomicAdd(rowp + gck[s], fma(px, jx[kk], py * jy[kk]));
-          }
-        }
-      }
 #pragma unroll
       for (int q = 0; q < MAXPAIRS; ++q) {
         if (threadIdx.x + q * kCellThreads < npairs) {
@@ -966,7 +911,7 @@
   if (Emax == 0) return;
   const int npairs = Emax * (Emax + 1) / 2;
   const int per_thread = (npairs + kCellThreads - 1) / kCellThreads;
-  const size_t smem = (2 * static_cast<size_t>(kCellTile) * (Emax | 1) + 2 * kCellTile + 18 * kCellTile) * sizeof(double);
+  const size_t smem = (2 * static_cast<size_t>(kCellTile) * (Emax | 1) + 2 * kCellTile) * sizeof(double);
   const unsigned blocks = static_cast<unsigned>((pb.n_obs + kCellChunk - 1) / kCellChunk);
 #define B200BA_LAUNCH_CELLS(MP)                                                                              \
   do {                                                                                                       \
@@ -985,6 +930,203 @@
   else
     B200BA_LAUNCH_CELLS(15);
 #undef B200BA_LAUNCH_CELLS
+}
+
+constexpr int kRunTile = 32;
+
+template <int ROWS>
+__global__ void __launch_bounds__(32 * ROWS)
+    accumulate_runs_kernel(ProblemDev pb, Layout L, StateDev st, ObsOut out, SystemDev sys, double huber, RunsDev runs) {
+  extern __shared__ double smem[];
+  constexpr int kPairs = ROWS * (ROWS + 1) / 2;
+  constexpr int kSlots = (kMaxK + 31) / 32;
+  const int64_t n = pb.n_obs;
+  const int beg = runs.off[blockIdx.x], end = runs.off[blockIdx.x + 1];
+  const int64_t o0 = runs.order[beg];
+  const int cam = static_cast<int>(pb.obs_camera[o0]);
+  const int ent = static_cast<int>(ROWS == 6 ? pb.obs_imageset[o0] : pb.obs_point[o0]);
+  const int g0 = (ROWS == 6) ? (L.g_pose + 6 * ent) : (L.g_point + 3 * ent);
+  const CamDev& c = pb.cams[cam];
+  const int K = L.localize_only ? 0 : c.K;
+  const bool grid = c.gw > 0;
+  const int cpc = grid ? K / 16 : K;
+  const int Wc = grid ? kRunWindow + 3 : 1;
+  const int X0 = grid ? runs.win[blockIdx.x] % c.gw : 0, Y0 = grid ? runs.win[blockIdx.x] / c.gw : 0;
+  const int NW = Wc * Wc * cpc;
+  const int S = K | 1;
+  double* sAcc = smem;
+  double* sJx = sAcc + ROWS * NW;
+  double* sJy = sJx + kRunTile * S;
+  uint8_t* sTouched = reinterpret_cast<uint8_t*>(sJy + kRunTile * S);
+  __shared__ double sPx[kRunTile][ROWS], sPy[kRunTile][ROWS], sR[kRunTile][2];
+  __shared__ double sObs[kRunTile][15];
+  __shared__ uint32_t sO[kRunTile];
+  __shared__ int sCell[kRunTile];
+  __shared__ int sLoc[kRunTile];
+  const int warp = threadIdx.x >> 5, lane = threadIdx.x & 31;
+  for (int i = threadIdx.x; i < ROWS * NW; i += blockDim.x) sAcc[i] = 0.0;
+  for (int i = threadIdx.x; i < Wc * Wc; i += blockDim.x) sTouched[i] = 0;
+  const int row_g = g0 + warp;
+  double* rowp = (row_g < L.nbd) ? (sys.B + static_cast<int64_t>(row_g) * L.nd)
+                                 : (sys.C + static_cast<int64_t>(row_g - L.nbd) * L.nd);
+  double acc = 0.0;
+  int pa = 0, pb_ = 0;
+  if (threadIdx.x < kPairs) {
+    int p = threadIdx.x;
+    while (p >= ROWS - pa) {
+      p -= ROWS - pa;
+      ++pa;
+    }
+    pb_ = pa + p;
+  }
+  for (int base = beg; base < end; base += kRunTile) {
+    const int tile_n = min(kRunTile, end - base);
+    __syncthreads();
+    if (threadIdx.x < tile_n) {
+      const int t = threadIdx.x;
+      const int64_t o = runs.order[base + t];
+      sO[t] = static_cast<uint32_t>(o);
+      if (out.has_jac[o] != kJacValid) {
+        sLoc[t] = -2;
+      } else {
+        const double rx = out.residual[o], ry = out.residual[n + o];
+        const double sw = sqrt(huber_weight_sq(huber, rx * rx + ry * ry));
+        sR[t][0] = sw * rx;
+        sR[t][1] = sw * ry;
+        if (out.compact) {
+          double jp[2][3], jo[2][6], jr[2][6];
+          compact_small_blocks(pb, L, st, out, o, jp, jo, jr);
+#pragma unroll
+          for (int q = 0; q < ROWS; ++q) {
+            sPx[t][q] = sw * (ROWS == 6 ? jo[0][q] : jp[0][q % 3]);
+            sPy[t][q] = sw * (ROWS == 6 ? jo[1][q] : jp[1][q % 3]);
+          }
+          double wx[4], dwx[4], wy[4], dwy[4];
+          bspline_basis(out.cjac[12 * n + o], wx, dwx);
+          bspline_basis(out.cjac[13 * n + o], wy, dwy);
+          sObs[t][0] = sw;
+#pragma unroll
+          for (int q = 0; q < 4; ++q) {
+            sObs[t][1 + q] = wx[q];
+            sObs[t][5 + q] = wy[q];
+          }
+#pragma unroll
+          for (int q = 0; q < 6; ++q) sObs[t][9 + q] = out.cjac[static_cast<int64_t>(6 + q) * n + o];
+        } else {
+          const int jc = (ROWS == 6) ? L.jc_pose : L.jc_point;
+#pragma unroll
+          for (int q = 0; q < ROWS; ++q) {
+            sPx[t][q] = sw * out.jac[(2 * static_cast<int64_t>(jc + q)) * n + o];
+            sPy[t][q] = sw * out.jac[(2 * static_cast<int64_t>(jc + q) + 1) * n + o];
+          }
+          sObs[t][0] = sw;
+        }
+        int loc = 0, cell = 0;
+        if (grid) {
+          cell = out.cell[o];
+          const int cx = cell % c.gw - X0, cy = cell / c.gw - Y0;
+          loc = (cx >= 0 && cx < kRunWindow && cy >= 0 && cy < kRunWindow) ? cx + cy * Wc : -1;
+        }
+        sCell[t] = cell;
+        sLoc[t] = loc;
+        if (loc >= 0 && K > 0) {
+          if (grid) {
+#pragma unroll
+            for (int q = 0; q < 16; ++q) sTouched[loc + (q & 3) + (q >> 2) * Wc] = 1;
+          } else {
+            sTouched[0] = 1;
+          }
+        }
+      }
+    }
+    __syncthreads();
+    for (int p = threadIdx.x; p < tile_n * K; p += blockDim.x) {
+      const int t = p / K, k = p - t * K;
+      if (sLoc[t] == -2) continue;
+      const int64_t o = sO[t];
+      double jx, jy;
+      if (out.compact) {
+        const int cp = k >> 1;
+        const double* so = sObs[t];
+        const double wk = so[0] * so[1 + (cp & 3)] * so[5 + (cp >> 2)];
+        const d3 tk = ld3(st.tangents + c.tan_off +
+                          6 * (static_cast<int64_t>(sCell[t]) + (cp & 3) + static_cast<int64_t>(cp >> 2) * c.gw) + 3 * (k & 1));
+        jx = wk * (so[9] * tk.x + so[10] * tk.y + so[11] * tk.z);
+        jy = wk * (so[12] * tk.x + so[13] * tk.y + so[14] * tk.z);
+      } else {
+        jx = sObs[t][0] * out.jac[(2 * static_cast<int64_t>(L.jc_intr + k)) * n + o];
+        jy = sObs[t][0] * out.jac[(2 * static_cast<int64_t>(L.jc_intr + k) + 1) * n + o];
+      }
+      sJx[t * S + k] = jx;
+      sJy[t * S + k] = jy;
+    }
+    __syncthreads();
+    for (int t = 0; t < tile_n; ++t) {
+      const int loc = sLoc[t];
+      if (loc == -2) continue;
+      const double px = sPx[t][warp], py = sPy[t][warp];
+      const double* jx = sJx + t * S;
+      const double* jy = sJy + t * S;
+#pragma unroll
+      for (int s = 0; s < kSlots; ++s) {
+        const int k = lane + 32 * s;
+        if (k < K) {
+          const double v = fma(px, jx[k], py * jy[k]);
+          if (loc >= 0) {
+            const int cp = k / cpc, q = k - cp * cpc;
+            sAcc[warp * NW + (loc + (cp & 3) + (cp >> 2) * Wc) * cpc + q] += v;
+          } else {
+            atomicAdd(rowp + (L.g_intr + intr_col(c, sCell[t], k) - L.nbd), v);
+          }
+        }
+      }
+    }
+    if (threadIdx.x < kPairs + ROWS) {
+      const bool is_b = threadIdx.x >= kPairs;
+      const int a = is_b ? threadIdx.x - kPairs : pa;
+      for (int t = 0; t < tile_n; ++t) {
+        if (sLoc[t] == -2) continue;
+        const double bx = is_b ? sR[t][0] : sPx[t][pb_], by = is_b ? sR[t][1] : sPy[t][pb_];
+        acc = fma(sPx[t][a], bx, fma(sPy[t][a], by, acc));
+      }
+    }
+  }
+  __syncthreads();
+  for (int i = threadIdx.x; i < ROWS * NW; i += blockDim.x) {
+    const int r = i / NW, j = i - r * NW, cpl = j / cpc;
+    if (!sTouched[cpl]) continue;
+    const int q = j - cpl * cpc;
+    const int gcol = grid ? c.upd_off + cpc * ((X0 + cpl % Wc) + (Y0 + cpl / Wc) * c.gw) + q : c.upd_off + q;
+    const int gr = g0 + r;
+    double* rp = (gr < L.nbd) ? (sys.B + static_cast<int64_t>(gr) * L.nd) : (sys.C + static_cast<int64_t>(gr - L.nbd) * L.nd);
+    atomicAdd(rp + (L.g_intr + gcol - L.nbd), sAcc[i]);
+  }
+  if (threadIdx.x < kPairs)
+    add_H(L, sys, g0 + pa, g0 + pb_, acc);
+  else if (threadIdx.x < kPairs + ROWS)
+    add_b(L, sys, g0 + threadIdx.x - kPairs, acc);
+}
+
+void launch_accumulate_runs(const ProblemDev& pb, const Layout& L, const StateDev& st, const ObsOut& out,
+                            const SystemDev& sys, double huber, const RunsDev& runs, bool pose_rows, cudaStream_t s) {
+  if (runs.n_runs == 0) return;
+  int nw = 0, wc2 = 1;
+  for (int c = 0; c < L.n_cameras; ++c) {
+    const CamDev& cd = pb.cams[c];
+    const int K = L.localize_only ? 0 : cd.K;
+    const int wc = cd.gw > 0 ? kRunWindow + 3 : 1;
+    nw = std::max(nw, cd.gw > 0 ? wc * wc * (K / 16) : K);
+    wc2 = std::max(wc2, wc * wc);
+  }
+  const int rows = pose_rows ? 6 : 3;
+  const size_t smem = (static_cast<size_t>(rows) * nw + 2 * static_cast<size_t>(kRunTile) * (L.Kmax | 1)) * sizeof(double) + wc2;
+  if (pose_rows) {
+    cudaFuncSetAttribute(accumulate_runs_kernel<6>, cudaFuncAttributeMaxDynamicSharedMemorySize, static_cast<int>(smem));
+    accumulate_runs_kernel<6><<<runs.n_runs, 6 * 32, smem, s>>>(pb, L, st, out, sys, huber, runs);
+  } else {
+    cudaFuncSetAttribute(accumulate_runs_kernel<3>, cudaFuncAttributeMaxDynamicSharedMemorySize, static_cast<int>(smem));
+    accumulate_runs_kernel<3><<<runs.n_runs, 3 * 32, smem, s>>>(pb, L, st, out, sys, huber, runs);
+  }
 }
 
 template <int BS>
diff --git a/camera_calibration_b200/csrc/ba_kernels.h b/camera_calibration_b200/csrc/ba_kernels.h
--- a/camera_calibration_b200/csrc/ba_kernels.h
+++ b/camera_calibration_b200/csrc/ba_kernels.h
@@ -23,6 +23,8 @@
                                const SystemDev& sys, double huber, cudaStream_t s);
 void launch_accumulate_cells(const ProblemDev& pb, const Layout& L, const StateDev& st, const ObsOut& out,
                              const SystemDev& sys, double huber, cudaStream_t s);
+void launch_accumulate_runs(const ProblemDev& pb, const Layout& L, const StateDev& st, const ObsOut& out,
+                            const SystemDev& sys, double huber, const RunsDev& runs, bool pose_rows, cudaStream_t s);
 void launch_schur_blocks(int bs, int n_blocks, const double* Dblk, const double* bp, double lambda, double* Linv,
                          double* v, int* fail, cudaStream_t s);
 void launch_schur_scale_rows(int bs, int n_blocks, int nd, const double* B, const double* Linv, double* W,
diff --git a/include/b200ba.h b/include/b200ba.h
--- a/include/b200ba.h
+++ b/include/b200ba.h
@@ -362,6 +362,9 @@
 #define B200BA_LM_REJECTED_COST 2
 #define B200BA_LM_REFUSED_PIVOT 3
 B200BA_API int32_t b200ba_debug_lm_events(const b200ba_handle* h, int32_t* codes, int32_t cap);
+#define B200BA_RUN_WINDOW 8
+B200BA_API int b200ba_debug_window_runs(const b200ba_problem* problem, int32_t pose_rows, uint32_t* order,
+                                        int32_t* run_off, int32_t* run_win, int32_t* n_runs);
 
 #ifdef __cplusplus
 }
```

Result: faster. 23.78, median of 6 (+1.7%).
